# alevar/tiebrush

Hardware: AMD Instinct MI355X
Metric: input alignment records/sec collapsed (tiebrush) + bases/sec covered (tiecov) (higher is better)
Workload: dtype int64; 1 GPU; c3: 64 synthetic sorted BAMs x 5000000 100bp reads per GPU, --clip collapse + tiecov -c -j of the result; records_per_gpu=320000000, groups_out=25086541, parallelism=files-per-rank x1, ranks_seen=1, resident=SoA in HBM before the timed region, contexts=3

## Files before the change

### include/tbk.h

```cpp
#ifndef TBK_H_
#define TBK_H_

#include <stddef.h>
#include <stdint.h>

#ifdef __cplusplus
extern "C" {
#endif

#define TBK_ABI_VERSION 9

typedef struct tbk_ctx tbk_ctx;

typedef enum tbk_status {
  TBK_OK = 0,
  TBK_EINVAL = -1,
  TBK_ENOMEM = -2,
  TBK_EHIP = -3,
  TBK_E2BIG = -4,
  TBK_EUNSUPPORTED = -5,
  TBK_EUNSORTED = -6,
  TBK_EFATALOP = -7,
  TBK_ECOLLISION = -8,
  TBK_ENODEVICE = -9
// ... 7 lines not shown
} tbk_strategy;

typedef enum tbk_mem {
  TBK_MEM_HOST = 0,
  TBK_MEM_DEVICE = 1,
  TBK_MEM_KEPT = 2
} tbk_mem;

#define TBK_NH_ABSENT INT32_MIN

typedef struct tbk_collapse_opts {
  int32_t strategy;
  int32_t max_nh;
  int32_t min_qual;
  uint32_t flags_mask;
  uint8_t keep_supplementary;
  uint8_t keep_secondary;
  uint8_t keep_unmapped;
  uint8_t collapse_same;
  uint8_t store_frac;
  uint8_t defer_yd;
  uint8_t keep_results;
  uint8_t reserved[1];
} tbk_collapse_opts;

typedef struct tbk_soa_in {
  int32_t mem;
  uint32_t n_files;
  uint32_t n_records;
  uint32_t n_cigar_ops;
  const uint32_t* file_off;
  const uint8_t* tbmerged;
  const int32_t* tid;
  const int32_t* pos;
  const uint16_t* flag;
  const uint8_t* mapq;
  const uint8_t* strand;
  const int32_t* nh;
  const uint32_t* cig_off;
  const uint32_t* cig;
  const double* yc_in;
  const int64_t* yx_in;
  const int64_t* yd_in;
  const uint32_t* md_off;
  const uint8_t* md;
  const uint8_t* md_has;
  const uint64_t* qname_hash;
  const uint64_t* prio_hi;
  const uint64_t* prio_lo;
  const uint32_t* qname_off;
  const uint8_t* qname;
} tbk_soa_in;

typedef struct tbk_groups_out {
  int32_t mem;
  uint32_t cap_groups;
  uint32_t* rep;
  double* yc;
  int64_t* yx;
  int32_t* yd;
  int32_t* g_start;
  int32_t* g_end;
  int32_t* rec_group;
  int32_t* rep_effend;
  uint64_t* g_key;
  uint32_t n_groups;
  uint32_t n_passed;
} tbk_groups_out;

typedef struct tbk_cov_in {
  int32_t mem;
  uint32_t n_records;
  uint32_t n_cigar_ops;
  const int32_t* tid;
  const int32_t* pos;
  const uint16_t* flag;
  const uint32_t* cig_off;
  const uint32_t* cig;
  const double* yc;
  const uint8_t* strand;
  const int64_t* yx;
} tbk_cov_in;

typedef struct tbk_cov_out {
  int32_t mem;
  uint32_t cap_intervals;
  int32_t* iv_tid;
  int32_t* iv_start;
  int32_t* iv_end;
  double* iv_val;
  uint32_t cap_junctions;
  int32_t* j_tid;
  int32_t* j_start;
  int32_t* j_end;
  uint8_t* j_strand;
  double* j_val;
  uint32_t n_intervals;
  uint32_t n_junctions;
  uint64_t n_bases;
  uint64_t span_bases;
} tbk_cov_out;

typedef struct tbk_sample_out {
  int32_t mem;
  uint32_t cap_intervals;
  int32_t* iv_tid;
  int32_t* iv_start;
  int32_t* iv_end;
  int64_t* iv_count;
  float* iv_heat;
  uint32_t n_intervals;
} tbk_sample_out;

typedef struct tbk_kernel_time {
  const char* name;
  float ms;
  uint32_t launches;
} tbk_kernel_time;

int tbk_abi_version(void);
int tbk_create(int device_ordinal, tbk_ctx** out);
void tbk_destroy(tbk_ctx* ctx);
const char* tbk_strerror(int status);
const char* tbk_last_error(const tbk_ctx* ctx);

#define TBK_STREAM_DEFAULT ((void*)1)
int tbk_set_stream(tbk_ctx* ctx, void* hip_stream);
void* tbk_get_stream(tbk_ctx* ctx);
int tbk_set_profiling(tbk_ctx* ctx, int enabled);
int tbk_set_debug(tbk_ctx* ctx, const char* spec);
int tbk_kernel_times(tbk_ctx* ctx, tbk_kernel_time* out, int cap);

int tbk_host_alloc(size_t bytes, void** out);
void tbk_host_free(void* p);

void tbk_collapse_opts_default(tbk_collapse_opts* o);
int tbk_collapse_tile(tbk_ctx* ctx, const tbk_collapse_opts* opts, const tbk_soa_in* in, tbk_groups_out* out);
int tbk_collapse_finish_yd(tbk_ctx* ctx);
int tbk_warmup(tbk_ctx* ctx);
enum { TBK_ROUTE_NONE = 0, TBK_ROUTE_RAW_WINDOW = 1, TBK_ROUTE_COMPACTED_WINDOW = 2, TBK_ROUTE_SORT = 3 };
typedef struct tbk_collapse_route {
  int32_t form;
  int32_t reseeds;
  uint8_t raw_handed_back;
  uint8_t big_bucket;
  uint8_t wg_stats;
  uint8_t reserved;
  uint32_t nw, nw_live;
  uint32_t ovf1, ovf2;
} tbk_collapse_route;
int tbk_last_route(const tbk_ctx* ctx, tbk_collapse_route* out);
int tbk_coverage_tile(tbk_ctx* ctx, const tbk_cov_in* in, tbk_cov_out* out);
int tbk_sample_tile(tbk_ctx* ctx, const tbk_cov_in* in, int32_t num_samples, tbk_sample_out* out);

int tbk_groups_to_cov_in(tbk_ctx* ctx, const tbk_soa_in* in, const tbk_groups_out* groups, tbk_cov_in* view);


int tbk_bgzf_inflate(tbk_ctx* ctx, const uint8_t* comp, uint64_t comp_bytes, uint8_t* out, uint64_t out_cap, uint64_t* out_bytes, int mem);

int tbk_bam_decode(tbk_ctx* ctx, uint32_t n_files, const uint8_t* const* comp, const uint64_t* comp_bytes, const uint8_t* tbmerged,
                   int want_md, int want_names, tbk_soa_in* tile, uint32_t* file_off_out);
int tbk_bam_records(tbk_ctx* ctx, const uint32_t* idx, uint32_t n, int idx_mem, uint8_t* out, uint64_t out_cap, uint64_t* out_off);
void tbk_bam_release(tbk_ctx* ctx);
int tbk_tile_join(tbk_ctx* ctx, const tbk_soa_in* dev_part, const tbk_soa_in* host_part, tbk_soa_in* out, uint32_t* file_off_out,
                  uint8_t* tbmerged_out);
int tbk_reserve_tile(tbk_ctx* ctx, uint64_t n_records, uint64_t n_cigar_ops);


int tbk_bgzf_deflate(tbk_ctx* ctx, const uint8_t* src, uint64_t n, int src_mem, const uint64_t* cuts, uint32_t n_members, uint8_t* out,
                     uint64_t out_cap, uint64_t* out_bytes);

typedef struct tbk_enc_in {
  int32_t mem;
  uint32_t n;
  const uint32_t* rep;
  const double* yc;
  const int64_t* yx;
  const int32_t* yd;
  uint32_t n_dev;
  uint32_t n_host;
  const uint8_t* host_blob;
  const uint64_t* host_off;
  const uint32_t* host_slot;
  uint32_t first;
  tbk_ctx* from;
} tbk_enc_in;
int tbk_bam_encode(tbk_ctx* ctx, const tbk_enc_in* in, uint8_t* out, uint64_t out_cap, uint64_t* out_bytes, uint64_t* payload_bytes);
typedef struct tbk_ix_opts {
  uint32_t n_ref;
  uint32_t reserved;
  const uint32_t* ref_len;
  uint64_t* rec_vbeg;
} tbk_ix_opts;
typedef struct tbk_ix_chunk {
  int32_t tid;
  uint32_t bin;
  uint64_t beg, end;
} tbk_ix_chunk;
typedef struct tbk_ix_ref {
  int32_t tid;
  uint32_t reserved;
  uint64_t n_records;
  uint64_t first, last;
} tbk_ix_ref;
typedef struct tbk_ix_part {
  uint32_t n_chunks;
  uint32_t n_refs;
  uint64_t n_lin;
  uint64_t lin_first;
  const tbk_ix_chunk* chunks;
  const uint64_t* lin;
  const tbk_ix_ref* refs;
} tbk_ix_part;
int tbk_bam_encode_indexed(tbk_ctx* ctx, const tbk_enc_in* in, uint8_t* out, uint64_t out_cap, uint64_t* out_bytes, uint64_t* payload_bytes,
                           const tbk_ix_opts* ix, tbk_ix_part* part);
int tbk_kept_results(tbk_ctx* ctx, uint32_t first, uint32_t n, uint32_t* rep, double* yc, int64_t* yx, int32_t* yd);

typedef struct tbk_packed_in {
  uint32_t n_files;
  uint32_t n_records;
  uint32_t n_cigar_ops;
  uint32_t n_tid_runs;
  const uint32_t* file_off;
  const uint32_t* tid_run_end;
  const int32_t* tid_run_tid;
  const int32_t* pos;
  const uint32_t* meta;
  const uint8_t* ncig;
  const uint32_t* cig;
  uint32_t n_nh_esc, n_ncig_esc;
  const uint32_t* nh_esc_idx;
  const int32_t* nh_esc_val;
  const uint32_t* ncig_esc_idx;
  const uint32_t* ncig_esc_val;
} tbk_packed_in;
int tbk_unpack_tile(tbk_ctx* ctx, const tbk_packed_in* in, tbk_soa_in* tile);


int tbk_shard_prepare(tbk_ctx* ctx, const tbk_collapse_opts* opts, const tbk_soa_in* in, int64_t* key, int64_t* emax, int32_t* effend,
                      uint8_t* pass);
int tbk_shard_probe_max(tbk_ctx* ctx, const uint32_t* file_off, uint32_t n_files, const int64_t* key, const int64_t* emax,
                        const int64_t* cuts, uint32_t n_cuts, int64_t* m_out);
int tbk_shard_probe_next(tbk_ctx* ctx, const uint32_t* file_off, uint32_t n_files, const int64_t* key, const int64_t* m, uint32_t n_cuts,
                         int64_t* nxt_out);
#define TBK_SHARD_ROW 6
int tbk_shard_pack(tbk_ctx* ctx, const tbk_soa_in* in, const int64_t* key, const uint8_t* pass, const int32_t* effend, const int64_t* cuts,
                   uint32_t world, int32_t* rows, uint32_t* cig_out, int64_t* src_idx, int64_t* tab);
int tbk_shard_unpack(tbk_ctx* ctx, const int32_t* rows, uint32_t n2, const uint32_t* file_off2, uint32_t K, int32_t* tid, int32_t* pos,
                     uint16_t* flag, uint8_t* mapq, uint8_t* strand, int32_t* nh, uint32_t* cig_off, int64_t* prio_hi, int64_t* prio_lo);


int tbk_partial_keys(tbk_ctx* ctx, const tbk_soa_in* in, const tbk_groups_out* g, int64_t* key, int64_t* emax, uint32_t* not_packable);
#define TBK_PARTIAL_ROW 12
int tbk_partial_pack(tbk_ctx* ctx, const tbk_collapse_opts* opts, const tbk_soa_in* in, const tbk_groups_out* g, const int64_t* key,
                     const int64_t* cuts, uint32_t world, uint32_t first_fidx, int32_t* rows, uint32_t* cig_out, int64_t* tab);
#define TBK_PARTIAL_BUNDLES 15
#define TBK_PARTIAL_CAND (2 + 2 * TBK_PARTIAL_BUNDLES)
#define TBK_PARTIAL_META (64 + 4)
int tbk_partial_stage_keys(tbk_ctx* ctx, const tbk_soa_in* in, const tbk_groups_out* g, int64_t* key, int64_t* emax, uint32_t first_fidx, int64_t carry,
                           int64_t* meta);
int tbk_partial_stage_cands(tbk_ctx* ctx, const int64_t* key, const int64_t* emax, uint32_t n_groups, const int64_t* allmeta, uint32_t world,
                            int64_t* targets, int64_t* cands);
int tbk_partial_stage_pack(tbk_ctx* ctx, const tbk_collapse_opts* opts, const tbk_soa_in* in, const tbk_groups_out* g, const int64_t* key,
                           const int64_t* mymeta, const int64_t* allcands, const int64_t* targets, uint32_t world, uint32_t first_fidx, int64_t* cuts,
                           int32_t* rows, uint32_t* cig_out, int64_t* tabx);
int tbk_partial_pack_md(tbk_ctx* ctx, const tbk_soa_in* in, const tbk_groups_out* g, const int64_t* tab, uint32_t world, int32_t* rows, uint8_t* md_out,
                        int64_t* md_tab);
int tbk_partial_unpack_md(tbk_ctx* ctx, const int32_t* rows, uint32_t n2, uint32_t* md_off, uint8_t* md_has);
int tbk_partial_unpack(tbk_ctx* ctx, const int32_t* rows, uint32_t n2, int32_t* tid, int32_t* pos, uint16_t* flag, uint8_t* mapq,
                       uint8_t* strand, int32_t* nh, uint32_t* cig_off, double* yc_in, int64_t* yx_in, int64_t* yd_in, int64_t* prio_hi,
                       int64_t* prio_lo);
int tbk_partial_reduce(tbk_ctx* ctx, const tbk_collapse_opts* opts, const int32_t* rows, uint32_t n2, const uint32_t* run_off,
                       uint32_t n_runs, const uint32_t* cig, tbk_groups_out* out, tbk_cov_in* view);
int tbk_partial_reduce_md(tbk_ctx* ctx, const tbk_collapse_opts* opts, const int32_t* rows, uint32_t n2, const uint32_t* run_off, uint32_t n_runs,
                          const uint32_t* cig, const uint8_t* md, tbk_groups_out* out, tbk_cov_in* view);

typedef enum tbk_track_kind { TBK_TRACK_COV = 0, TBK_TRACK_JUNC = 1, TBK_TRACK_SAMPLE = 2 } tbk_track_kind;
typedef struct tbk_track_rows {
  int32_t mem;
  int32_t kind;
  uint32_t n;
  uint32_t reserved;
  const int32_t* tid;
  const int32_t* start;
  const int32_t* end;
  const double* val;
  const uint8_t* strand;
  const int64_t* count;
  const float* heat;
  int64_t first_junc;
} tbk_track_rows;
typedef int (*tbk_track_sink)(void* user, const char* bytes, uint64_t n);
int tbk_track_names(tbk_ctx* ctx, uint32_t n_names, const uint64_t* off, const char* bytes);
int tbk_format_track(tbk_ctx* ctx, const tbk_track_rows* rows, tbk_track_sink sink, void* user, uint64_t* out_bytes);


int tbk_bam_decode_spans(tbk_ctx* ctx, uint32_t n_spans, const uint8_t* const* comp, const uint64_t* comp_bytes, const uint32_t* first_uoff,
                         const uint32_t* last_uoff, int32_t n_ref, tbk_soa_in* tile, uint32_t* span_off_out, const uint8_t** tag_seen_out);

int tbk_region_view(tbk_ctx* ctx, const tbk_soa_in* tile, const uint8_t* tag_seen, int32_t tid, int64_t beg, int64_t end, tbk_cov_in* view,
                    uint32_t* n_kept);

int tbk_cov_clip(tbk_ctx* ctx, tbk_cov_out* rows, int32_t tid, int64_t beg, int64_t end);
int tbk_sample_clip(tbk_ctx* ctx, tbk_sample_out* rows, int32_t tid, int64_t beg, int64_t end);


// ... 26 lines not shown
```

### tiebrush_amd/_lib.py

```python
from __future__ import annotations

import ctypes as C
import os

_HERE = os.path.dirname(os.path.abspath(__file__))
LIB_PATH = os.path.join(_HERE, "_build", "libtbk.so")

_P = C.c_void_p

TBK_MEM_HOST, TBK_MEM_DEVICE, TBK_MEM_KEPT = 0, 1, 2
PARTIAL_BUNDLES = 15
PARTIAL_CAND = 2 + 2 * PARTIAL_BUNDLES
PARTIAL_META = 64 + 4
STRAT = {"cigar": 0, "full": 1, "clip": 2, "exon": 3}
STATUS = {0: "TBK_OK", -1: "TBK_EINVAL", -2: "TBK_ENOMEM", -3: "TBK_EHIP", -4: "TBK_E2BIG", -5: "TBK_EUNSUPPORTED",
          -6: "TBK_EUNSORTED", -7: "TBK_EFATALOP", -8: "TBK_ECOLLISION", -9: "TBK_ENODEVICE"}

SYMBOLS = ["tbk_abi_version", "tbk_create", "tbk_destroy", "tbk_strerror", "tbk_last_error", "tbk_set_stream",
           "tbk_get_stream", "tbk_set_profiling", "tbk_set_debug", "tbk_kernel_times", "tbk_host_alloc", "tbk_host_free",
           "tbk_collapse_opts_default", "tbk_collapse_tile", "tbk_collapse_finish_yd", "tbk_coverage_tile", "tbk_sample_tile",
           "tbk_groups_to_cov_in", "tbk_bgzf_inflate", "tbk_bam_decode", "tbk_bam_records", "tbk_bam_release", "tbk_shard_prepare", "tbk_shard_probe_max", "tbk_shard_probe_next",
           "tbk_shard_pack", "tbk_shard_unpack", "tbk_partial_keys", "tbk_partial_pack", "tbk_partial_unpack", "tbk_partial_reduce", "tbk_unpack_tile", "tbk_tile_join", "tbk_reserve_tile", "tbk_bgzf_deflate", "tbk_bam_encode", "tbk_kept_results", "tbk_warmup", "tbk_partial_stage_keys", "tbk_partial_stage_cands", "tbk_partial_stage_pack",
           "tbk_partial_pack_md", "tbk_partial_unpack_md", "tbk_partial_reduce_md", "tbk_track_names", "tbk_format_track", "tbk_bam_encode_indexed",
           "tbk_bam_decode_spans", "tbk_region_view", "tbk_cov_clip", "tbk_sample_clip", "tbk_bam_decode_file_spans", "tbk_tile_region", "tbk_last_route",
           "tbk_regions_view", "tbk_cov_clip_regions", "tbk_sample_clip_regions", "tbk_tile_regions"]


class CollapseOpts(C.Structure):
    _fields_ = [("strategy", C.c_int32), ("max_nh", C.c_int32), ("min_qual", C.c_int32), ("flags_mask", C.c_uint32),
                ("keep_supplementary", C.c_uint8), ("keep_secondary", C.c_uint8), ("keep_unmapped", C.c_uint8),
                ("collapse_same", C.c_uint8), ("store_frac", C.c_uint8), ("defer_yd", C.c_uint8), ("keep_results", C.c_uint8), ("reserved", C.c_uint8 * 1)]


class CollapseRoute(C.Structure):
    _fields_ = [("form", C.c_int32), ("reseeds", C.c_int32), ("raw_handed_back", C.c_uint8), ("big_bucket", C.c_uint8),
                ("wg_stats", C.c_uint8), ("reserved", C.c_uint8), ("nw", C.c_uint32), ("nw_live", C.c_uint32), ("ovf1", C.c_uint32),
                ("ovf2", C.c_uint32)]


ROUTE_FORMS = {0: "none", 1: "raw", 2: "compacted", 3: "sort"}


class SoaIn(C.Structure):
    _fields_ = [("mem", C.c_int32), ("n_files", C.c_uint32), ("n_records", C.c_uint32), ("n_cigar_ops", C.c_uint32),
                ("file_off", _P), ("tbmerged", _P), ("tid", _P), ("pos", _P), ("flag", _P), ("mapq", _P),
                ("strand", _P), ("nh", _P), ("cig_off", _P), ("cig", _P), ("yc_in", _P), ("yx_in", _P), ("yd_in", _P),
                ("md_off", _P), ("md", _P), ("md_has", _P), ("qname_hash", _P), ("prio_hi", _P), ("prio_lo", _P),
                ("qname_off", _P), ("qname", _P)]


class PackedIn(C.Structure):
    _fields_ = [("n_files", C.c_uint32), ("n_records", C.c_uint32), ("n_cigar_ops", C.c_uint32), ("n_tid_runs", C.c_uint32), ("file_off", _P),
                ("tid_run_end", _P), ("tid_run_tid", _P), ("pos", _P), ("meta", _P), ("ncig", _P), ("cig", _P), ("n_nh_esc", C.c_uint32),
                ("n_ncig_esc", C.c_uint32), ("nh_esc_idx", _P), ("nh_esc_val", _P), ("ncig_esc_idx", _P), ("ncig_esc_val", _P)]


class GroupsOut(C.Structure):
    _fields_ = [("mem", C.c_int32), ("cap_groups", C.c_uint32), ("rep", _P), ("yc", _P), ("yx", _P), ("yd", _P),
                ("g_start", _P), ("g_end", _P), ("rec_group", _P), ("rep_effend", _P), ("g_key", _P), ("n_groups", C.c_uint32),
                ("n_passed", C.c_uint32)]


class CovIn(C.Structure):
    _fields_ = [("mem", C.c_int32), ("n_records", C.c_uint32), ("n_cigar_ops", C.c_uint32), ("tid", _P), ("pos", _P),
                ("flag", _P), ("cig_off", _P), ("cig", _P), ("yc", _P), ("strand", _P), ("yx", _P)]


class CovOut(C.Structure):
    _fields_ = [("mem", C.c_int32), ("cap_intervals", C.c_uint32), ("iv_tid", _P), ("iv_start", _P), ("iv_end", _P),
                ("iv_val", _P), ("cap_junctions", C.c_uint32), ("j_tid", _P), ("j_start", _P), ("j_end", _P),
                ("j_strand", _P), ("j_val", _P), ("n_intervals", C.c_uint32), ("n_junctions", C.c_uint32),
                ("n_bases", C.c_uint64), ("span_bases", C.c_uint64)]


class SampleOut(C.Structure):
    _fields_ = [("mem", C.c_int32), ("cap_intervals", C.c_uint32), ("iv_tid", _P), ("iv_start", _P), ("iv_end", _P),
                ("iv_count", _P), ("iv_heat", _P), ("n_intervals", C.c_uint32)]


class EncIn(C.Structure):
    _fields_ = [("mem", C.c_int32), ("n", C.c_uint32), ("rep", _P), ("yc", _P), ("yx", _P), ("yd", _P), ("n_dev", C.c_uint32), ("n_host", C.c_uint32),
                ("host_blob", _P), ("host_off", _P), ("host_slot", _P), ("first", C.c_uint32), ("from_ctx", _P)]


class IxOpts(C.Structure):
    _fields_ = [("n_ref", C.c_uint32), ("reserved", C.c_uint32), ("ref_len", _P), ("rec_vbeg", _P)]


class IxChunk(C.Structure):
    _fields_ = [("tid", C.c_int32), ("bin", C.c_uint32), ("beg", C.c_uint64), ("end", C.c_uint64)]


class IxRef(C.Structure):
    _fields_ = [("tid", C.c_int32), ("reserved", C.c_uint32), ("n_records", C.c_uint64), ("first", C.c_uint64), ("last", C.c_uint64)]


class IxPart(C.Structure):
    _fields_ = [("n_chunks", C.c_uint32), ("n_refs", C.c_uint32), ("n_lin", C.c_uint64), ("lin_first", C.c_uint64), ("chunks", _P), ("lin", _P), ("refs", _P)]


class Regions(C.Structure):
    _fields_ = [("n", C.c_uint32), ("tid", _P), ("beg", _P), ("end", _P)]


TRACK = {"cov": 0, "junc": 1, "sample": 2}


class TrackRows(C.Structure):
    _fields_ = [("mem", C.c_int32), ("kind", C.c_int32), ("n", C.c_uint32), ("reserved", C.c_uint32), ("tid", _P), ("start", _P), ("end", _P),
                ("val", _P), ("strand", _P), ("count", _P), ("heat", _P), ("first_junc", C.c_int64)]


TRACK_SINK = C.CFUNCTYPE(C.c_int, _P, _P, C.c_uint64)


class KernelTime(C.Structure):
    _fields_ = [("name", C.c_char_p), ("ms", C.c_float), ("launches", C.c_uint32)]


_lib = None


def load():
    global _lib
    if _lib is not None:
        return _lib
    if not os.path.exists(LIB_PATH):
        raise ImportError("%s not found: build it with `python -c 'import __graft_entry__ as g; g.build()'` "
                          "(hipcc --offload-arch=gfx950); there is no CPU fallback" % LIB_PATH)
    try:
        import torch
    except ImportError:
        pass
    L = C.CDLL(LIB_PATH)
    L.tbk_abi_version.restype = C.c_int
    L.tbk_create.argtypes = [C.c_int, C.POINTER(_P)]
    L.tbk_create.restype = C.c_int
    L.tbk_destroy.argtypes = [_P]
    L.tbk_destroy.restype = None
    L.tbk_strerror.argtypes = [C.c_int]
    L.tbk_strerror.restype = C.c_char_p
    L.tbk_last_error.argtypes = [_P]
    L.tbk_last_error.restype = C.c_char_p
    L.tbk_set_stream.argtypes = [_P, _P]
    L.tbk_get_stream.argtypes = [_P]
    L.tbk_get_stream.restype = _P
    L.tbk_set_profiling.argtypes = [_P, C.c_int]
    L.tbk_set_debug.argtypes = [_P, C.c_char_p]
    L.tbk_last_route.argtypes = [_P, C.POINTER(CollapseRoute)]
    L.tbk_last_route.restype = C.c_int
    L.tbk_kernel_times.argtypes = [_P, C.POINTER(KernelTime), C.c_int]
    L.tbk_host_alloc.argtypes = [C.c_size_t, C.POINTER(_P)]
    L.tbk_host_free.argtypes = [_P]
    L.tbk_host_free.restype = None
    L.tbk_collapse_opts_default.argtypes = [C.POINTER(CollapseOpts)]
    L.tbk_collapse_opts_default.restype = None
    L.tbk_collapse_tile.argtypes = [_P, C.POINTER(CollapseOpts), C.POINTER(SoaIn), C.POINTER(GroupsOut)]
    L.tbk_collapse_finish_yd.argtypes = [_P]
    L.tbk_coverage_tile.argtypes = [_P, C.POINTER(CovIn), C.POINTER(CovOut)]
    L.tbk_sample_tile.argtypes = [_P, C.POINTER(CovIn), C.c_int32, C.POINTER(SampleOut)]
    L.tbk_groups_to_cov_in.argtypes = [_P, C.POINTER(SoaIn), C.POINTER(GroupsOut), C.POINTER(CovIn)]
    L.tbk_bgzf_inflate.argtypes = [_P, _P, C.c_uint64, _P, C.c_uint64, C.POINTER(C.c_uint64), C.c_int]
    L.tbk_bam_decode.argtypes = [_P, C.c_uint32, _P, _P, _P, C.c_int, C.c_int, C.POINTER(SoaIn), _P]
    L.tbk_bam_records.argtypes = [_P, _P, C.c_uint32, C.c_int, _P, C.c_uint64, _P]
    L.tbk_bam_release.argtypes = [_P]
    L.tbk_bam_release.restype = None
    L.tbk_shard_prepare.argtypes = [_P, C.POINTER(CollapseOpts), C.POINTER(SoaIn), _P, _P, _P, _P]
    L.tbk_shard_probe_max.argtypes = [_P, _P, C.c_uint32, _P, _P, _P, C.c_uint32, _P]
    L.tbk_shard_probe_next.argtypes = [_P, _P, C.c_uint32, _P, _P, C.c_uint32, _P]
    L.tbk_shard_pack.argtypes = [_P, C.POINTER(SoaIn), _P, _P, _P, _P, C.c_uint32, _P, _P, _P, _P]
    L.tbk_shard_unpack.argtypes = [_P, _P, C.c_uint32, _P, C.c_uint32, _P, _P, _P, _P, _P, _P, _P, _P, _P]
    L.tbk_partial_keys.argtypes = [_P, C.POINTER(SoaIn), C.POINTER(GroupsOut), _P, _P, C.POINTER(C.c_uint32)]
    L.tbk_partial_pack.argtypes = [_P, C.POINTER(CollapseOpts), C.POINTER(SoaIn), C.POINTER(GroupsOut), _P, _P, C.c_uint32, C.c_uint32, _P, _P, _P]
    L.tbk_partial_reduce.argtypes = [_P, C.POINTER(CollapseOpts), _P, C.c_uint32, _P, C.c_uint32, _P, C.POINTER(GroupsOut), C.POINTER(CovIn)]
    L.tbk_partial_unpack.argtypes = [_P, _P, C.c_uint32] + [_P] * 12
    L.tbk_tile_join.argtypes = [_P, C.POINTER(SoaIn), C.POINTER(SoaIn), C.POINTER(SoaIn), C.POINTER(C.c_uint32), C.POINTER(C.c_uint8)]
    L.tbk_tile_join.restype = C.c_int
    L.tbk_reserve_tile.argtypes = [_P, C.c_uint64, C.c_uint64]
    L.tbk_reserve_tile.restype = C.c_int
    L.tbk_unpack_tile.argtypes = [_P, C.POINTER(PackedIn), C.POINTER(SoaIn)]
    L.tbk_partial_stage_keys.argtypes = [_P, C.POINTER(SoaIn), C.POINTER(GroupsOut), _P, _P, C.c_uint32, C.c_int64, _P]
    L.tbk_partial_stage_cands.argtypes = [_P, _P, _P, C.c_uint32, _P, C.c_uint32, _P, _P]
    L.tbk_partial_stage_pack.argtypes = [_P, C.POINTER(CollapseOpts), C.POINTER(SoaIn), C.POINTER(GroupsOut), _P, _P, _P, _P, C.c_uint32, C.c_uint32, _P, _P, _P, _P]
    L.tbk_partial_pack_md.argtypes = [_P, C.POINTER(SoaIn), C.POINTER(GroupsOut), _P, C.c_uint32, _P, _P, _P]
    L.tbk_partial_unpack_md.argtypes = [_P, _P, C.c_uint32, _P, _P]
    L.tbk_partial_reduce_md.argtypes = [_P, C.POINTER(CollapseOpts), _P, C.c_uint32, _P, C.c_uint32, _P, _P, C.POINTER(GroupsOut), C.POINTER(CovIn)]
    L.tbk_bgzf_deflate.argtypes = [_P, _P, C.c_uint64, C.c_int, _P, C.c_uint32, _P, C.c_uint64, C.POINTER(C.c_uint64)]
    L.tbk_bgzf_deflate.restype = C.c_int
    L.tbk_bam_encode.argtypes = [_P, C.POINTER(EncIn), _P, C.c_uint64, C.POINTER(C.c_uint64), C.POINTER(C.c_uint64)]
    L.tbk_bam_encode.restype = C.c_int
    L.tbk_bam_encode_indexed.argtypes = [_P, C.POINTER(EncIn), _P, C.c_uint64, C.POINTER(C.c_uint64), C.POINTER(C.c_uint64), C.POINTER(IxOpts), C.POINTER(IxPart)]
    L.tbk_bam_encode_indexed.restype = C.c_int
    L.tbk_kept_results.argtypes = [_P, C.c_uint32, C.c_uint32, _P, _P, _P, _P]
    L.tbk_kept_results.restype = C.c_int
    L.tbk_warmup.argtypes = [_P]
    L.tbk_warmup.restype = C.c_int
    L.tbk_track_names.argtypes = [_P, C.c_uint32, _P, _P]
    L.tbk_track_names.restype = C.c_int
    L.tbk_format_track.argtypes = [_P, C.POINTER(TrackRows), TRACK_SINK, _P, C.POINTER(C.c_uint64)]
    L.tbk_format_track.restype = C.c_int
    L.tbk_bam_decode_spans.argtypes = [_P, C.c_uint32, _P, _P, _P, _P, C.c_int32, C.POINTER(SoaIn), _P, C.POINTER(_P)]
    L.tbk_bam_decode_spans.restype = C.c_int
    L.tbk_region_view.argtypes = [_P, C.POINTER(SoaIn), _P, C.c_int32, C.c_int64, C.c_int64, C.POINTER(CovIn), C.POINTER(C.c_uint32)]
    L.tbk_region_view.restype = C.c_int
    L.tbk_cov_clip.argtypes = [_P, C.POINTER(CovOut), C.c_int32, C.c_int64, C.c_int64]
    L.tbk_cov_clip.restype = C.c_int
    L.tbk_sample_clip.argtypes = [_P, C.POINTER(SampleOut), C.c_int32, C.c_int64, C.c_int64]
    L.tbk_sample_clip.restype = C.c_int
    L.tbk_bam_decode_file_spans.argtypes = [_P, C.c_uint32, _P, _P, _P, _P, _P, C.c_int32, _P, C.c_int, C.c_int, C.POINTER(SoaIn), _P]
    L.tbk_bam_decode_file_spans.restype = C.c_int
    L.tbk_tile_region.argtypes = [_P, C.POINTER(SoaIn), C.c_int32, C.c_int64, C.c_int64, C.POINTER(SoaIn), _P, C.POINTER(C.c_uint32)]
    L.tbk_tile_region.restype = C.c_int
    L.tbk_regions_view.argtypes = [_P, C.POINTER(SoaIn), _P, C.POINTER(Regions), C.POINTER(CovIn), C.POINTER(C.c_uint32)]
    L.tbk_regions_view.restype = C.c_int
    L.tbk_cov_clip_regions.argtypes = [_P, C.POINTER(CovOut), C.POINTER(Regions)]
    L.tbk_cov_clip_regions.restype = C.c_int
    L.tbk_sample_clip_regions.argtypes = [_P, C.POINTER(SampleOut), C.POINTER(Regions)]
    L.tbk_sample_clip_regions.restype = C.c_int
    L.tbk_tile_regions.argtypes = [_P, C.POINTER(SoaIn), C.POINTER(Regions), C.POINTER(SoaIn), _P, C.POINTER(C.c_uint32)]
    L.tbk_tile_regions.restype = C.c_int
    _lib = L
    return L


HOST_LIB_PATH = os.environ.get("TBK_HOST_LIB") or os.path.join(_HERE, "_build", "libtbh.so")
HOST_SYMBOLS = ["tbh_abi_version", "tbh_last_error", "tbh_tag_deflate_part", "tbh_write_bam_parts", "tbh_is_tiebrush", "tbh_bai_index_file", "tbh_bai_reg2bin",
                "tbh_csi_index_file", "tbh_csi_depth", "tbh_csi_reg2bin", "tbh_index_query",
                "tbh_regions_from_bed", "tbh_index_query_regions"]
_host = None


def load_host():
    global _host
    if _host is not None:
        return _host
    if not os.path.exists(HOST_LIB_PATH):
        raise ImportError("%s not found: build it with `python -c 'import __graft_entry__ as g; g.build()'`" % HOST_LIB_PATH)
    H = C.CDLL(HOST_LIB_PATH)
    H.tbh_abi_version.restype = C.c_int
    H.tbh_last_error.restype = C.c_char_p
    H.tbh_tag_deflate_part.argtypes = [_P, _P, _P, C.c_uint32, _P, _P, _P, C.c_int, C.c_int, C.c_char_p]
    H.tbh_tag_deflate_part.restype = C.c_int
    H.tbh_write_bam_parts.argtypes = [C.c_char_p, C.c_char_p, C.c_int, C.POINTER(C.c_char_p), C.c_int, C.POINTER(C.c_char_p), C.c_int,
                                      C.POINTER(C.c_char_p), C.c_int]
    H.tbh_write_bam_parts.restype = C.c_int
    H.tbh_is_tiebrush.argtypes = [C.c_char_p]
    H.tbh_is_tiebrush.restype = C.c_int
    H.tbh_bai_index_file.argtypes = [C.c_char_p, C.c_char_p]
    H.tbh_bai_index_file.restype = C.c_int
    H.tbh_bai_reg2bin.argtypes = [C.c_int64, C.c_int64]
    H.tbh_bai_reg2bin.restype = C.c_uint32
    H.tbh_csi_index_file.argtypes = [C.c_char_p, C.c_char_p]
    H.tbh_csi_index_file.restype = C.c_int
    H.tbh_csi_depth.argtypes = [C.c_uint64]
    H.tbh_csi_depth.restype = C.c_int
    H.tbh_csi_reg2bin.argtypes = [C.c_int64, C.c_int64, C.c_int]
    H.tbh_csi_reg2bin.restype = C.c_uint32
    H.tbh_index_query.argtypes = [C.c_char_p, C.c_char_p, C.c_int32, C.c_int64, C.c_int64, _P, _P, C.c_uint64]
    H.tbh_index_query.restype = C.c_int64
    H.tbh_regions_from_bed.argtypes = [C.c_char_p, C.c_char_p, _P, _P, _P, C.c_uint64]
    H.tbh_regions_from_bed.restype = C.c_int64
    H.tbh_index_query_regions.argtypes = [C.c_char_p, C.c_char_p, C.c_uint32, _P, _P, _P, _P, _P, C.c_uint64]
    H.tbh_index_query_regions.restype = C.c_int64
    _host = H
    return H


class TbkError(RuntimeError):
    def __init__(self, status, detail=""):
        self.status = status
        super().__init__("%s (%d) %s" % (STATUS.get(status, "?"), status, detail))
```

### tiebrush_amd/api.py

```python
from __future__ import annotations

import contextlib
import os
import ctypes as C
from dataclasses import replace

import numpy as np

from . import _lib
from ._lib import TbkError
from .soa import CovInput, SoATile


def _torch():
    import torch
    return torch


def _is_torch(a):
    return a is not None and type(a).__module__.startswith("torch")


def _addr(a, dtype, keep, n=None):
    if a is None:
        return None
    if _is_torch(a):
        torch = _torch()
        want = {np.int32: torch.int32, np.uint32: torch.int32, np.uint16: torch.int16, np.uint8: torch.uint8,
                np.float64: torch.float64, np.int64: torch.int64, np.uint64: torch.int64, np.float32: torch.float32}[dtype]
        if a.dtype != want and a.element_size() != np.dtype(dtype).itemsize:
            raise TypeError("tensor dtype %s does not match %s" % (a.dtype, dtype))
        if not a.is_contiguous():
            raise ValueError("tensor must be contiguous")
        if n is not None and a.numel() < n:
            raise ValueError("tensor too small: %d < %d" % (a.numel(), n))
        keep.append(a)
        return a.data_ptr()
    b = np.ascontiguousarray(a, dtype=dtype)
    if n is not None and b.size < n:
        raise ValueError("array too small: %d < %d" % (b.size, n))
    keep.append(b)
    return b.ctypes.data


def to_device(obj, device="cuda:0"):
    torch = _torch()

    def mv(a, dt):
        if a is None:
            return None
        b = np.ascontiguousarray(a, dtype=dt)
        sd = {np.uint32: np.int32, np.uint16: np.int16, np.uint64: np.int64}.get(dt, dt)
        return torch.from_numpy(b.view(sd)).to(device)

    if isinstance(obj, SoATile):
        r = replace(obj, tid=mv(obj.tid, np.int32), pos=mv(obj.pos, np.int32), flag=mv(obj.flag, np.uint16),
                       mapq=mv(obj.mapq, np.uint8), strand=mv(obj.strand, np.uint8), nh=mv(obj.nh, np.int32),
                       cig_off=mv(obj.cig_off, np.uint32), cig=mv(obj.cig, np.uint32), yc_in=mv(obj.yc_in, np.float64),
                       yx_in=mv(obj.yx_in, np.int64), yd_in=mv(obj.yd_in, np.int64), md_off=mv(obj.md_off, np.uint32),
                       md=mv(obj.md, np.uint8), md_has=mv(obj.md_has, np.uint8),
                       qname_hash=mv(obj.qname_hash, np.uint64), qn_off=mv(obj.qn_off, np.uint32), qn=mv(obj.qn, np.uint8),
                       prio_hi=mv(obj.prio_hi, np.uint64), prio_lo=mv(obj.prio_lo, np.uint64))
        torch.cuda.synchronize()
        return r
    if isinstance(obj, CovInput):
        r = replace(obj, tid=mv(obj.tid, np.int32), pos=mv(obj.pos, np.int32), flag=mv(obj.flag, np.uint16),
                       cig_off=mv(obj.cig_off, np.uint32), cig=mv(obj.cig, np.uint32), yc=mv(obj.yc, np.float64),
                       strand=mv(obj.strand, np.uint8), yx=mv(obj.yx, np.int64))
        torch.cuda.synchronize()
        return r
    raise TypeError(type(obj))


def _numel(a):
    return int(a.numel()) if _is_torch(a) else int(np.asarray(a).size)


class DeviceTile:

    def __init__(self, struct, n_files, keep):
        self.struct, self.n_files, self._keep = struct, n_files, keep
        self.n_records = int(struct.n_records)


class DeviceCovView:

    def __init__(self, struct, n_records, n_cigar_ops):
        self.struct = struct
        self.n_records = n_records
        self.n_cigar_ops = n_cigar_ops


class _FollowDebug:

    def __init__(self, lib, ctx):
        self._lib, self._ctx = lib, ctx

    def __getattr__(self, name):
        self._ctx._follow_debug()
        return getattr(self._lib, name)


class Context:
    def __init__(self, device: int = 0):
        lib = _lib.load()
        h = C.c_void_p()
        self._debug_spec = os.environ.get("TBK_DEBUG", "")
        rc = lib.tbk_create(int(device), C.byref(h))
        if rc != 0:
            raise TbkError(rc, "tbk_create(device=%d)" % device)
        self._lib = lib
        self.L = _FollowDebug(lib, self)
        self.h = h
        self.device = device
        self._on_torch_stream = False

    def _follow_debug(self):
        spec = os.environ.get("TBK_DEBUG", "")
        if spec != self._debug_spec and getattr(self, "h", None):
            self._debug_spec = spec
            self._lib.tbk_set_debug(self.h, spec.encode())

    def set_debug(self, spec: str):
        self._debug_spec = os.environ.get("TBK_DEBUG", "")
        self._check(self._lib.tbk_set_debug(self.h, spec.encode()), "tbk_set_debug")

    def close(self):
        if getattr(self, "h", None):
            self._lib.tbk_destroy(self.h)
            self.h = None

    def __del__(self):
        try:
            self.close()
        except Exception:
            pass

    def _check(self, rc, what):
        if rc != 0:
            raise TbkError(rc, "%s: %s" % (what, (self.L.tbk_last_error(self.h) or b"").decode()))

    def use_torch_stream(self):
        s = _torch().cuda.current_stream(self.device).cuda_stream
        self._check(self.L.tbk_set_stream(self.h, C.c_void_p(s if s else 1)), "tbk_set_stream")
        self._on_torch_stream = True

    def _order_after_torch(self, dev):
        if dev and not self._on_torch_stream:
            _torch().cuda.current_stream(self.device).synchronize()

    def last_message(self) -> str:
        return (self.L.tbk_last_error(self.h) or b"").decode()

    def collapse_route(self) -> dict:
        r = _lib.CollapseRoute()
        self._check(self._lib.tbk_last_route(self.h, C.byref(r)), "tbk_last_route")
        d = dict(form=_lib.ROUTE_FORMS[int(r.form)], reseeds=int(r.reseeds), raw_handed_back=bool(r.raw_handed_back),
                 big_bucket=bool(r.big_bucket))
        if r.wg_stats:
            d.update(nw=int(r.nw), nw_live=int(r.nw_live), ovf1=int(r.ovf1), ovf2=int(r.ovf2))
        return d

    def stream_ptr(self):
        return self.L.tbk_get_stream(self.h)

    def set_profiling(self, on: bool):
        self._check(self.L.tbk_set_profiling(self.h, 1 if on else 0), "tbk_set_profiling")

    def kernel_times(self):
        arr = (_lib.KernelTime * 128)()
        n = self.L.tbk_kernel_times(self.h, arr, 128)
        return {arr[i].name.decode(): (float(arr[i].ms), int(arr[i].launches)) for i in range(min(n, 128))}

    def _alloc(self, device_mode, n, dtype):
        n = max(int(n), 1)
        if device_mode:
            torch = _torch()
            td = {np.int32: torch.int32, np.uint32: torch.int32, np.uint8: torch.uint8, np.float64: torch.float64,
                  np.int64: torch.int64, np.uint64: torch.int64, np.float32: torch.float32}[dtype]
            return torch.empty(n, dtype=td, device="cuda:%d" % self.device)
        return np.empty(n, dtype=dtype)

    @staticmethod
    def _trim(a, n, dtype):
        if _is_torch(a):
            return a[:n]
        return a[:n].view(dtype) if a.dtype != dtype else a[:n]

    def make_opts(self, strategy="cigar", max_nh=2**31 - 1, min_qual=-1, keep_supplementary=False,
                  keep_secondary=False, keep_unmapped=False, collapse_same=False, store_frac=False, flags_mask=0,
                  defer_yd=False, keep_results=False):
        o = _lib.CollapseOpts()
        self.L.tbk_collapse_opts_default(C.byref(o))
        o.strategy = _lib.STRAT[strategy] if isinstance(strategy, str) else int(strategy)
        o.max_nh, o.min_qual, o.flags_mask = int(max_nh), int(min_qual), int(flags_mask)
        o.keep_supplementary, o.keep_secondary = int(keep_supplementary), int(keep_secondary)
        o.keep_unmapped, o.collapse_same, o.store_frac = int(keep_unmapped), int(collapse_same), int(store_frac)
        o.defer_yd = int(defer_yd)
        o.keep_results = int(keep_results)
        return o

    def finish_yd(self):
        self._check(self.L.tbk_collapse_finish_yd(self.h), "tbk_collapse_finish_yd")

    def unpack_tile(self, pt) -> DeviceTile:
        keep = []

        def addr(a, dt):
            if _is_torch(a):
                keep.append(a)
                return a.data_ptr() if a.numel() else None
            b = np.ascontiguousarray(a, dtype=dt)
            keep.append(b)
            return b.ctypes.data if b.size else None

        fo = np.ascontiguousarray(pt.file_off, dtype=np.uint32)
        re_, rt = np.ascontiguousarray(pt.tid_run_end, np.uint32), np.ascontiguousarray(pt.tid_run_tid, np.int32)
        keep += [fo, re_, rt]
        p = _lib.PackedIn(pt.n_files, _numel(pt.pos), _numel(pt.cig), len(re_), fo.ctypes.data, re_.ctypes.data, rt.ctypes.data, addr(pt.pos, np.int32),
                          addr(pt.meta, np.uint32), addr(pt.ncig, np.uint8), addr(pt.cig, np.uint32), _numel(pt.nh_esc_idx), _numel(pt.ncig_esc_idx),
                          addr(pt.nh_esc_idx, np.uint32), addr(pt.nh_esc_val, np.int32), addr(pt.ncig_esc_idx, np.uint32),
                          addr(pt.ncig_esc_val, np.uint32))
        s = _lib.SoaIn()
        self._check(self.L.tbk_unpack_tile(self.h, C.byref(p), C.byref(s)), "tbk_unpack_tile")
        return DeviceTile(s, pt.n_files, keep)

    def _soa_struct(self, tile: SoATile, keep):
        if isinstance(tile, DeviceTile):
            keep.append(tile)
            return tile.struct, True, tile.n_records
        dev = _is_torch(tile.tid)
        n = _numel(tile.tid)
        nc = _numel(tile.cig)
        fo = np.ascontiguousarray(tile.file_off, dtype=np.uint32)
        tb = np.ascontiguousarray(tile.tbmerged, dtype=np.uint8)
        keep += [fo, tb]
        s = _lib.SoaIn(
            _lib.TBK_MEM_DEVICE if dev else _lib.TBK_MEM_HOST, tile.n_files, n, nc, fo.ctypes.data, tb.ctypes.data,
            _addr(tile.tid, np.int32, keep, n), _addr(tile.pos, np.int32, keep, n), _addr(tile.flag, np.uint16, keep, n),
            _addr(tile.mapq, np.uint8, keep, n), _addr(tile.strand, np.uint8, keep, n), _addr(tile.nh, np.int32, keep, n),
            _addr(tile.cig_off, np.uint32, keep, n + 1), _addr(tile.cig, np.uint32, keep, nc),
            _addr(tile.yc_in, np.float64, keep, n), _addr(tile.yx_in, np.int64, keep, n),
            _addr(tile.yd_in, np.int64, keep, n), _addr(tile.md_off, np.uint32, keep, n + 1),
            _addr(tile.md, np.uint8, keep), _addr(tile.md_has, np.uint8, keep, n),
            _addr(tile.qname_hash, np.uint64, keep, n), _addr(tile.prio_hi, np.uint64, keep, n),
            _addr(tile.prio_lo, np.uint64, keep, n), _addr(tile.qn_off, np.uint32, keep, n + 1), _addr(tile.qn, np.uint8, keep))
        return s, dev, n

    def collapse(self, tile: SoATile, opts=None, want_coords=True, want_rec_group=False, want_effend=False, out=None,
                 raw=False, want_key=None, cap_groups=None, **kw):
        o = opts if opts is not None else self.make_opts(**kw)
        keep = []
        s, dev, n = self._soa_struct(tile, keep)
        self._order_after_torch(dev)
        cap = max(n if cap_groups is None else min(int(cap_groups), n), 1)
        bufs = out if out is not None else {}
        if bufs.get("_cap_groups", 0) > cap:
            cap = bufs["_cap_groups"]
        res = self._collapse_once(o, s, dev, n, cap, bufs, keep, want_coords, want_rec_group, want_effend, want_key, raw)
        if isinstance(res, int):
            bufs["_cap_groups"] = cap = min(n, res + res // 16 + 1)
            res = self._collapse_once(o, s, dev, n, cap, bufs, keep, want_coords, want_rec_group, want_effend, want_key, raw)
            assert not isinstance(res, int)
        return res

    def _collapse_once(self, o, s, dev, n, cap, bufs, keep, want_coords, want_rec_group, want_effend, want_key, raw):

        def buf(name, count, dt, wanted=True):
            if not wanted:
                return None
            if name not in bufs or _numel(bufs[name]) < count:
                bufs[name] = self._alloc(dev, count, dt)
            return bufs[name]

        rep, yc = buf("rep", cap, np.uint32), buf("yc", cap, np.float64)
        yx, yd = buf("yx", cap, np.int64), buf("yd", cap, np.int32)
        gs, ge = buf("g_start", cap, np.int32, want_coords), buf("g_end", cap, np.int32, want_coords)
        rg = buf("rec_group", max(n, 1), np.int32, want_rec_group)
        re_ = buf("rep_effend", cap, np.int32, want_effend)
        want_key = bool(dev) if want_key is None else want_key
        gk = buf("g_key", 2 * cap, np.uint64, want_key)
        g = _lib.GroupsOut(s.mem, cap, _addr(rep, np.uint32, keep), _addr(yc, np.float64, keep),
                           _addr(yx, np.int64, keep), _addr(yd, np.int32, keep), _addr(gs, np.int32, keep),
                           _addr(ge, np.int32, keep), _addr(rg, np.int32, keep), _addr(re_, np.int32, keep),
                           _addr(gk, np.uint64, keep), 0, 0)
        rc = self.L.tbk_collapse_tile(self.h, C.byref(o), C.byref(s), C.byref(g))
        if rc == -4 and int(g.n_groups) > cap:
            return int(g.n_groups)
        self._check(rc, "tbk_collapse_tile")
        m = int(g.n_groups)
        res = dict(n_groups=m, n_passed=int(g.n_passed), _bufs=bufs, _struct=g, _soa=s, _keep=keep)
        if raw:
            return res
        res.update(rep=self._trim(rep, m, np.uint32), yc=yc[:m], yx=yx[:m], yd=yd[:m])
        if want_coords:
            res.update(g_start=gs[:m], g_end=ge[:m])
        if want_rec_group:
            res["rec_group"] = rg[:n]
        if want_effend:
            res["rep_effend"] = re_[:m]
        if want_key:
            res["g_key"] = gk[:2 * m]
        return res

    def groups_to_cov_in(self, collapse_result) -> DeviceCovView:
        v = _lib.CovIn()
        self._order_after_torch(True)
        self._check(self.L.tbk_groups_to_cov_in(self.h, C.byref(collapse_result["_soa"]),
                                                C.byref(collapse_result["_struct"]), C.byref(v)),
                    "tbk_groups_to_cov_in")
        return DeviceCovView(v, int(v.n_records), int(v.n_cigar_ops))

    def bgzf_inflate(self, comp: bytes) -> bytes:
        src = np.frombuffer(comp, dtype=np.uint8)
        need = C.c_uint64(0)
        out = np.empty(max(1, 4 * len(src) + 65536), dtype=np.uint8)
        rc = self.L.tbk_bgzf_inflate(self.h, src.ctypes.data, len(src), out.ctypes.data, out.size, C.byref(need), _lib.TBK_MEM_HOST)
        if rc == -4:
            out = np.empty(int(need.value), dtype=np.uint8)
            rc = self.L.tbk_bgzf_inflate(self.h, src.ctypes.data, len(src), out.ctypes.data, out.size, C.byref(need), _lib.TBK_MEM_HOST)
        self._check(rc, "tbk_bgzf_inflate")
        return out[:int(need.value)].tobytes()

    def bgzf_deflate(self, payload: bytes, cuts=None) -> bytes:
        src = np.frombuffer(payload, dtype=np.uint8)
# ... 698 lines not shown
```

### tiebrush_amd/csrc/cb_tiles.hpp

```cpp
#pragma once
#include "dev_common.hpp"
#include "scan_op.hpp"

struct CbAgg {
  int32_t first_tid, last_tid;
  int32_t mx;
  uint32_t whole;
};
struct CbOp {
  __device__ __forceinline__ CbAgg operator()(const CbAgg& a, const CbAgg& b) const {
    if (b.last_tid == INT32_MIN) return a;
    if (a.last_tid == INT32_MIN) return b;
    CbAgg r;
    r.first_tid = a.first_tid;
    r.last_tid = b.last_tid;
    const bool joins = b.whole && b.first_tid == a.last_tid;
    r.mx = joins ? (a.mx > b.mx ? a.mx : b.mx) : b.mx;
    r.whole = joins ? a.whole : 0u;
    return r;
  }
};
constexpr uint32_t CB_NT = 256, CB_ROWS = 4, CB_TILE = CB_NT * 4 * CB_ROWS;
template <class T, class Op>
__device__ __forceinline__ T wave_incl_scan_op(T v, Op op) {
#pragma unroll
  for (int d = 1; d < 64; d <<= 1) {
    const T o = shfl_up_t(v, d);
    if ((int)lane_id() >= d) v = op(o, v);
  }
  return v;
}
__device__ __forceinline__ void cb_put(uint64_t* p, uint64_t v) { __hip_atomic_store(p, v, __ATOMIC_RELAXED, __HIP_MEMORY_SCOPE_AGENT); }
__device__ __forceinline__ uint64_t cb_get(const uint64_t* p) { return __hip_atomic_load(p, __ATOMIC_RELAXED, __HIP_MEMORY_SCOPE_AGENT); }
__device__ __forceinline__ uint4 cb_get4(const uint4* p) {
  const uint64_t a = cb_get(reinterpret_cast<const uint64_t*>(p)), b = cb_get(reinterpret_cast<const uint64_t*>(p) + 1);
  return make_uint4((uint32_t)a, (uint32_t)(a >> 32), (uint32_t)b, (uint32_t)(b >> 32));
}
__device__ __forceinline__ bool cb_last_block(uint32_t* __restrict__ done) {
  __shared__ uint32_t s_last;
  if (threadIdx.x == 0) {
    __builtin_amdgcn_s_waitcnt(TBK_WAIT_VMCNT0);
    __asm__ volatile("" ::: "memory");
    s_last = atomicAdd(done, 1u) == gridDim.x - 1u ? 1u : 0u;
  }
  __syncthreads();
  return s_last != 0u;
}
template <uint32_t NT>
__device__ __forceinline__ void cb_spine_block(uint4* __restrict__ part, uint32_t ntiles, CbAgg* wl ) {
  const CbOp op{};
  const CbAgg none{0, INT32_MIN, INT32_MIN, 1u};
  auto un = [](const uint4& v) { return CbAgg{(int32_t)v.x, (int32_t)v.y, (int32_t)v.z, v.w}; };
  auto pk = [](const CbAgg& a) { return make_uint4((uint32_t)a.first_tid, (uint32_t)a.last_tid, (uint32_t)a.mx, a.whole); };
  const uint4 none4 = pk(none);
  const uint32_t per = (ntiles + NT - 1u) / NT, i0 = threadIdx.x * per, i1 = i0 + per < ntiles ? i0 + per : ntiles;
  CbAgg a = none;
  for (uint32_t q0 = i0; q0 < i1; q0 += 8u) {
    uint4 v8[8];
#pragma unroll
    for (uint32_t u = 0; u < 8u; ++u) v8[u] = q0 + u < i1 ? cb_get4(part + q0 + u) : none4;
#pragma unroll
    for (uint32_t u = 0; u < 8u; ++u) a = op(a, un(v8[u]));
  }
  const CbAgg inc = wave_incl_scan_op(a, op);
  if (lane_id() == 63) wl[threadIdx.x >> 6] = inc;
  CbAgg run = shfl_up_t(inc, 1);
  __syncthreads();
  {
    CbAgg acc = none;
    const uint32_t wv = threadIdx.x >> 6;
    for (uint32_t q = 0; q < wv; ++q) acc = op(acc, wl[q]);
    run = lane_id() == 0 ? acc : op(acc, run);
  }
  for (uint32_t q0 = i0; q0 < i1; q0 += 8u) {
    uint4 v8[8];
#pragma unroll
    for (uint32_t u = 0; u < 8u; ++u) v8[u] = q0 + u < i1 ? cb_get4(part + q0 + u) : none4;
#pragma unroll
    for (uint32_t u = 0; u < 8u; ++u) {
      if (q0 + u < i1) part[q0 + u] = pk(run);
      run = op(run, un(v8[u]));
    }
  }
}
```

### tiebrush_amd/csrc/collapse.hip

```cpp
#include <stdlib.h>

#include <chrono>

#include "cb_tiles.hpp"
#include "dev_common.hpp"
#include "rx_w64.hpp"
#include "scan_op.hpp"
#include "strategy.hpp"
#include "tbk_internal.h"
#include "wgroup.h"

namespace {

struct EffKey {
  uint32_t khi_h, khi_l;
  int32_t kend;
  uint32_t flag_cnt;
};
struct EffOp {
  __device__ __forceinline__ EffKey operator()(const EffKey& a, const EffKey& b) const {
    uint64_t ak = ((uint64_t)a.khi_h << 32) | a.khi_l, bk = ((uint64_t)b.khi_h << 32) | b.khi_l;
    bool take_b = (b.flag_cnt >> 31) || bk > ak || (bk == ak && b.kend > a.kend);
    EffKey r;
    r.khi_h = take_b ? b.khi_h : a.khi_h;
// ... 2301 lines not shown
      out->n_passed = m;
      if (m == 0) return 0;
      m_hi = m;
    }
    bool runs_now = use_runs && (lean || m >= runs_min);
    for (;;) {
      if (runs_now)
        TBK_TRY(tbk_sort_runs(ctx, &s2, m_hi, run_off, I.k, ctx->d_err, (uint32_t*)(sc + 12)));
      else
        TBK_TRY(tbk_radix_sort128(ctx, &s2, m));
      TBK_LAUNCH(ctx, "col_heads", col_heads_k, cdiv(m_hi, B), B, 0, I, O.strategy, sc + 0, m_hi, s2.hi, s2.lo, s2.val, fidx, flags,
                 ghead, ctx->d_err);
      TBK_TRY(tbk_exscan_u32(ctx, ghead, gex, m_hi, sc + 1));
      if (lean) break;
      TBK_TRY(tbk_sync_err(ctx, &eb));
      if (runs_now && (eb & TBK_DERR_BIGBUCKET)) {
        std::swap(s2.hi, s2.hi2);
        std::swap(s2.lo, s2.lo2);
        std::swap(s2.val, s2.val2);
        TBK_HIP(hipMemsetAsync(ctx->d_err, 0, sizeof(uint32_t), ctx->stream));
        runs_now = false;
        continue;
      }
      break;
    }
    if (!lean) {
      if (eb & TBK_DERR_COLLISION) {
        ++attempt;
        continue;
      }
      if (eb) return tbk_derr_to_status(ctx, eb);
      ng = (uint32_t)ctx->h_scalars[1];
      if (ng > out->cap_groups) {
        out->n_groups = ng;
        return TBK_E2BIG;
      }
      ng_hi = ng;
    }
    const uint64_t *pm = sc + 0, *png = sc + 1;
    G.yc = ws_alloc<double>(ctx, ng_hi);
    G.ns = ws_alloc<uint32_t>(ctx, ng_hi);
    G.yxin = ws_alloc<long long>(ctx, ng_hi);
    G.ydin = ws_alloc<long long>(ctx, ng_hi);
    G.rep = ws_alloc<unsigned long long>(ctx, ng_hi);
    G.first = ws_alloc<uint32_t>(ctx, ng_hi);
    G.tie = ws_alloc<uint8_t>(ctx, ng_hi);
    g_yd = ws_alloc<int32_t>(ctx, ng_hi);
    gperm = ws_alloc<uint32_t>(ctx, ng_hi);
    ginv = ws_alloc<uint32_t>(ctx, ng_hi);
    if (!ginv) return TBK_ENOMEM;
    TBK_LAUNCH(ctx, "col_init_groups", col_init_groups_k, cdiv(ng_hi, B), B, 0, png, G, g_yd);
    TBK_LAUNCH(ctx, "col_reduce", col_reduce_k, cdiv(m_hi, B), B, 0, I, O, pm, s2.val, flags, gex, fidx, effend, G, sgid, ctx->d_err);
    if (I.prio_hi && I.prio_lo) TBK_LAUNCH(ctx, "col_rep_prio", col_rep_prio_k, cdiv(ng_hi, B), B, 0, I, png, pm, s2.val, G);
    if (O.collapse_same) TBK_LAUNCH(ctx, "col_same", col_same_k, cdiv(m_hi, B), B, 0, I, O, pm, s2.val, flags, sgid, fidx, G);
    TBK_LAUNCH(ctx, "col_tie_sort", col_tie_sort_k, cdiv(ng_hi, B), B, 0, I, O.strategy, png, s2.val, G, gperm, ginv);

    if (O.store_frac || any_tbm) {
      TBK_TRY(tbk_sync_err(ctx, &eb));
      const bool need_ordered = O.store_frac || (eb & TBK_DERR_FRACTIONAL);
      eb &= ~TBK_DERR_FRACTIONAL;
      if (eb) return tbk_derr_to_status(ctx, eb);
      if (need_ordered) {
        TBK_HIP(hipMemsetAsync(ctx->d_err, 0, sizeof(uint32_t), ctx->stream));
        SortBufs ob;
        ob.hi = ws_alloc<uint64_t>(ctx, m);
        ob.lo = ws_alloc<uint64_t>(ctx, m);
        ob.val = ws_alloc<uint32_t>(ctx, m);
        ob.hi2 = ws_alloc<uint64_t>(ctx, m);
        ob.lo2 = ws_alloc<uint64_t>(ctx, m);
        ob.val2 = ws_alloc<uint32_t>(ctx, m);
        uint8_t* fh_by_rec = ws_alloc<uint8_t>(ctx, n);
        if (!ob.val2 || !fh_by_rec) return TBK_ENOMEM;
        TBK_LAUNCH(ctx, "ord_fill", ord_fill_k, cdiv(m, B), B, 0, m, s2.val, sgid, effend, I.prio_hi, flags, ob.hi, ob.lo, ob.val, fh_by_rec);
        TBK_TRY(tbk_radix_sort128(ctx, &ob, m));
        TBK_LAUNCH(ctx, "ord_sum", ord_sum_k, cdiv(ng, 64), 64, 0, I, O, ng, m, ob.val, fidx, fh_by_rec, G);
      }
    }
    TBK_LAUNCH(ctx, "col_write", col_write_k<false>, cdiv(ng_hi, B), B, 0, png, gperm, G, s2.hi, s2.lo, out->cap_groups, out->rep, out->yc,
               out->yx, out->g_start, out->g_end, effend, out->rep_effend, out->g_key, O.strategy);
    if (out->rec_group) TBK_LAUNCH(ctx, "col_recgroup", col_recgroup_k, cdiv(m_hi, B), B, 0, pm, s2.val, sgid, ginv, out->rec_group);
    TBK_TRY(tbk_sync_err(ctx, &eb));
    if (lean) {
      if (eb & TBK_DERR_BIGBUCKET) {
        use_runs = false;
        lean = false;
        continue;
      }
      if (eb & TBK_DERR_COLLISION) {
        ++attempt;
        continue;
      }
      m = (uint32_t)ctx->h_scalars[0];
      ng = (uint32_t)ctx->h_scalars[1];
      out->n_passed = m;
    }
    if (eb & ~TBK_DERR_FRACTIONAL) return tbk_derr_to_status(ctx, eb);
    sb = s2;
    route.form = TBK_ROUTE_SORT;
    if (attempt > 0) {
      char b[96];
      snprintf(b, sizeof(b), "info: key-hash collision, reseeded %d time(s)", attempt);
      ctx->last_error = b;
    }
    break;
  }
  out->n_groups = ng;
  if (m == 0) return 0;
  if (ng > out->cap_groups) return TBK_E2BIG;
  TBK_TRY(tbk_check_launch(ctx, "collapse"));
  YdJob* job = new YdJob();
  job->I = I;
  job->m = m;
  job->ng = ng;
  job->cap = out->cap_groups;
  if (win_done) {
    job->win = true;
    job->np = win_out.np;
    job->pfile = win_out.pfile;
    job->pgrp = win_out.pgrp;
    job->gpoff = win_out.gpoff;
    job->gfmask = win_out.gfmask;
  }
  job->val = sb.val;
  job->flags = flags;
  job->fidx = fidx;
  job->sgid = sgid;
  job->ginv = ginv;
  job->gperm = gperm;
  job->G = G;
  job->shi = win_done ? win_out.ghi : sb.hi;
  job->slo = win_done ? win_out.glo : sb.lo;
  job->g_yd = g_yd;
  job->out_yd = out->yd;
  ctx->yd_job = job;
  return 0;
}

namespace {
__global__ void g2c_count_k(uint32_t ng, const uint32_t* __restrict__ rep, const uint32_t* __restrict__ cig_off, uint32_t* __restrict__ cnt,
                            uint32_t* __restrict__ cfirst) {
  uint32_t o = blockIdx.x * blockDim.x + threadIdx.x;
  if (o >= ng) return;
  const uint32_t c0 = cig_off[rep[o]];
  cnt[o] = cig_off[rep[o] + 1] - c0;
  cfirst[o] = c0;
}
__device__ __forceinline__ uint32_t g2c_key_ops(uint64_t k1) {
  const uint32_t shape = (uint32_t)k1;
  return shape == 0x80000000u ? 1u : ((shape >> 30) == 3u ? 3u : 0u);
}
__global__ __launch_bounds__(CB_NT) void g2c_count_key_k(uint32_t ng, const uint64_t* __restrict__ key, const uint32_t* __restrict__ rep,
                                                         const uint32_t* __restrict__ cig_off, const uint32_t* __restrict__ cig,
                                                         uint32_t* __restrict__ cnt, uint32_t* __restrict__ cfirst, uint4* __restrict__ part,
                                                         unsigned long long* __restrict__ tsum, uint32_t* __restrict__ done,
                                                         unsigned long long* __restrict__ total) {
  constexpr uint32_t NWV = CB_NT / 64;
  __shared__ CbAgg wl[CB_ROWS * NWV];
  __shared__ unsigned long long wsum[CB_ROWS * NWV];
  const CbOp op{};
  const CbAgg none{0, INT32_MIN, INT32_MIN, 1u};
  for (uint32_t r = 0; r < CB_ROWS; ++r) {
    const uint64_t i = (uint64_t)blockIdx.x * CB_TILE + ((uint64_t)r * CB_NT + threadIdx.x) * 4u;
    CbAgg a = none;
    uint32_t n4[4] = {0u, 0u, 0u, 0u};
#pragma unroll
    for (int e = 0; e < 4; ++e) {
      if (i + e < ng) {
        const uint32_t o = (uint32_t)(i + e);
        const uint64_t k0 = key[2 * (size_t)o], k1 = key[2 * (size_t)o + 1];
        const int32_t tidv = (int32_t)(uint32_t)(k0 >> 33) - 1, posv = (int32_t)(uint32_t)((k0 >> 2) & 0x7FFFFFFFull) - 1;
        uint32_t n = g2c_key_ops(k1);
        int l = (int)(uint32_t)(k1 >> 32);
        if (n == 0) {
          const uint32_t rp = rep[o];
          const uint32_t c0 = cig_off[rp];
          n = cig_off[rp + 1] - c0;
          cfirst[o] = c0;
          int nex = 0;
          l = walk_exons(posv, cig + c0, n, [](int, int) {}, &nex);
        }
        n4[e] = n;
        a = op(a, CbAgg{tidv, tidv, posv + l, 1u});
      }
    }
    if (i + 3 < ng) {
      *reinterpret_cast<uint4*>(cnt + i) = make_uint4(n4[0], n4[1], n4[2], n4[3]);
    } else {
#pragma unroll
      for (int e = 0; e < 4; ++e)
        if (i + e < ng) cnt[i + e] = n4[e];
    }
    a = wave_incl_scan_op(a, op);
    const unsigned long long sum = wave_sum((unsigned long long)n4[0] + n4[1] + n4[2] + n4[3]);
    if (lane_id() == 63) {
      wl[r * NWV + (threadIdx.x >> 6)] = a;
      wsum[r * NWV + (threadIdx.x >> 6)] = sum;
    }
  }
  __syncthreads();
  if (threadIdx.x == 0) {
    CbAgg run = none;
    unsigned long long sum = 0;
#pragma unroll
    for (uint32_t q = 0; q < CB_ROWS * NWV; ++q) {
      run = op(run, wl[q]);
      sum += wsum[q];
    }
    uint64_t* o = reinterpret_cast<uint64_t*>(part + blockIdx.x);
    cb_put(o, (uint64_t)(uint32_t)run.first_tid | ((uint64_t)(uint32_t)run.last_tid << 32));
    cb_put(o + 1, (uint64_t)(uint32_t)run.mx | ((uint64_t)run.whole << 32));
    cb_put(reinterpret_cast<uint64_t*>(tsum + blockIdx.x), sum);
  }
  if (!cb_last_block(done)) return;
  const uint32_t ntiles = gridDim.x;
  cb_spine_block<CB_NT>(part, ntiles, wl);
  const uint32_t per = (ntiles + CB_NT - 1u) / CB_NT;
  const uint32_t i0 = threadIdx.x * per < ntiles ? threadIdx.x * per : ntiles, i1 = i0 + per < ntiles ? i0 + per : ntiles;
  unsigned long long mine = 0;
  for (uint32_t q = i0; q < i1; ++q) mine += cb_get(reinterpret_cast<const uint64_t*>(tsum + q));
  unsigned long long tot;
  unsigned long long run = block_excl_sum<unsigned long long, CB_NT>(mine, wsum, &tot);
  for (uint32_t q = i0; q < i1; ++q) {
    const unsigned long long v = cb_get(reinterpret_cast<const uint64_t*>(tsum + q));
    tsum[q] = run;
    run += v;
  }
  if (threadIdx.x == 0) *total = tot;
}
struct G2cPrep {
  int32_t *start, *end, *yi;
  uint32_t *jcnt, *ridx;
  unsigned long long* sums;
};
__global__ __launch_bounds__(256) void g2c_gather_key_k(uint32_t ng, const uint64_t* __restrict__ key, const double* __restrict__ yc,
                                                        const int64_t* __restrict__ yx, const uint32_t* __restrict__ cfirst,
                                                        const uint32_t* __restrict__ cnt, const uint32_t* __restrict__ cig,
                                                        const unsigned long long* __restrict__ tbase, const uint4* __restrict__ part,
                                                        uint32_t ntiles, uint32_t total, int32_t* __restrict__ o_tid,
                                                        int32_t* __restrict__ o_pos, uint8_t* __restrict__ o_strand, double* __restrict__ o_yc,
                                                        int64_t* __restrict__ o_yx, uint32_t* __restrict__ o_cig_off, uint32_t* __restrict__ o_cig,
                                                        uint4* __restrict__ o_part, G2cPrep P) {
  constexpr uint32_t NROW = CB_TILE / 256u;
  __shared__ uint32_t s_w[NROW * 4u];
  for (uint32_t q = blockIdx.x * 256u + threadIdx.x; q < ntiles; q += gridDim.x * 256u) o_part[q] = part[q];
  unsigned long long mb = 0, ay = 0, nji = 0;
  uint32_t eb = 0;
  for (uint32_t tile = blockIdx.x; tile < ntiles; tile += gridDim.x) {
  const uint32_t o0 = tile * CB_TILE;
  for (uint32_t j = 0; j < NROW; ++j) {
    const uint32_t o = o0 + j * 256u + threadIdx.x;
    const uint32_t s = wave_sum(o < ng ? cnt[o] : 0u);
    if (lane_id() == 0) s_w[j * 4u + (threadIdx.x >> 6)] = s;
  }
  __syncthreads();
  if (threadIdx.x < 64u) {
    const uint32_t v = s_w[threadIdx.x];
    s_w[threadIdx.x] = wave_incl_sum(v) - v;
  }
  __syncthreads();
  const uint32_t base = (uint32_t)tbase[tile];
  for (uint32_t j = 0; j < NROW; ++j) {
    const uint32_t o = o0 + j * 256u + threadIdx.x;
    const uint32_t cn = o < ng ? cnt[o] : 0u;
    const uint32_t d = base + s_w[j * 4u + (threadIdx.x >> 6)] + wave_incl_sum(cn) - cn;
    if (o >= ng) continue;
    const uint64_t k0 = key[2 * (size_t)o], k1 = key[2 * (size_t)o + 1];
    const int32_t tidv = (int32_t)(uint32_t)(k0 >> 33) - 1, posv = (int32_t)(uint32_t)((k0 >> 2) & 0x7FFFFFFFull) - 1;
    o_tid[o] = tidv;
    o_pos[o] = posv;
    const uint32_t sc = (uint32_t)k0 & 3u;
    o_strand[o] = sc == 0u ? (uint8_t)'+' : (sc == 1u ? (uint8_t)'-' : (uint8_t)'.');
    const double y0 = (double)(float)yc[o];
    o_yc[o] = y0;
    o_yx[o] = yx[o];
    o_cig_off[o] = d;
    if (o + 1 == ng) o_cig_off[ng] = total;
    const uint32_t shape = (uint32_t)k1, span = (uint32_t)(k1 >> 32);
    int l, nex = 0;
    if (shape == 0x80000000u) {
      o_cig[d] = (span << 4) | C_M;
      l = (int)span;
      nex = 1;
      mb += span;
    } else if ((shape >> 30) == 3u) {
      const uint32_t a = (shape >> 20) & 0x3FFu, g = shape & 0xFFFFFu;
      o_cig[d] = (a << 4) | C_M;
      o_cig[d + 1] = (g << 4) | C_N;
      o_cig[d + 2] = ((span - a - g) << 4) | C_M;
      l = (int)span;
      nex = 2;
      mb += span - g;
    } else {
      const uint32_t c0 = cfirst[o], n = cn;
      l = walk_exons(posv, cig + c0, n, [](int, int) {}, &nex);
      for (uint32_t k = 0; k < n; ++k) {
        const uint32_t w = cig[c0 + k];
        o_cig[d + k] = w;
        const uint32_t op = cig_op(w);
        if (op == C_M)
          mb += cig_len(w);
        else if (op != C_I && op != C_D && op != C_N && op != C_S)
          eb |= TBK_DERR_FATALOP;
      }
      if (n >= 256) eb |= TBK_DERR_NCIGAR;
    }
    double y = y0;
    if (!(y == rint(y)) || !(fabs(y) < 1073741824.0)) {
      eb |= TBK_DERR_FRACTIONAL;
      y = 0.0;
    } else {
      ay += (unsigned long long)fabs(y);
    }
    P.ridx[o] = o;
    P.yi[o] = (int32_t)y;
    P.start[o] = posv + 1;
    P.end[o] = posv + l;
    P.jcnt[o] = (uint32_t)(nex - 1);
    nji += (unsigned long long)(nex - 1);
  }
  __syncthreads();
  }
  __shared__ unsigned long long red_mb[4], red_ay[4], red_nj[4];
  __shared__ uint32_t red_e[4];
  mb = wave_sum(mb);
  ay = wave_sum(ay);
  nji = wave_sum(nji);
#pragma unroll
  for (int dd = 32; dd >= 1; dd >>= 1) eb |= __shfl_xor(eb, dd, 64);
  if (lane_id() == 0) {
    red_mb[threadIdx.x >> 6] = mb;
    red_ay[threadIdx.x >> 6] = ay;
    red_nj[threadIdx.x >> 6] = nji;
    red_e[threadIdx.x >> 6] = eb;
  }
  __syncthreads();
  if (threadIdx.x == 0) {
    for (int q = 1; q < 4; ++q) {
      mb += red_mb[q];
      ay += red_ay[q];
      nji += red_nj[q];
      eb |= red_e[q];
    }
    if (mb) atomicAdd(&P.sums[0], mb);
    if (ay) atomicAdd(&P.sums[1], ay);
    if (eb) atomicOr(&P.sums[2], (unsigned long long)eb);
    if (nji) atomicAdd(&P.sums[3], nji);
  }
}
__global__ void g2c_gather_k(uint32_t ng, const uint32_t* __restrict__ rep, const double* __restrict__ yc, const int64_t* __restrict__ yx,
                             const int32_t* __restrict__ tid, const int32_t* __restrict__ pos, const uint8_t* __restrict__ strand,
                             const uint32_t* __restrict__ cfirst, const uint32_t* __restrict__ cnt, const uint32_t* __restrict__ cig,
                             const uint32_t* __restrict__ ooff, uint32_t total, int32_t* __restrict__ o_tid, int32_t* __restrict__ o_pos,
                             uint8_t* __restrict__ o_strand, double* __restrict__ o_yc, int64_t* __restrict__ o_yx,
                             uint32_t* __restrict__ o_cig_off, uint32_t* __restrict__ o_cig) {
  uint32_t o = blockIdx.x * blockDim.x + threadIdx.x;
  if (o >= ng) return;
  uint32_t r = rep[o];
  o_tid[o] = tid[r];
  o_pos[o] = pos[r];
  o_strand[o] = strand[r];
  o_yc[o] = (double)(float)yc[o];
  o_yx[o] = yx[o];
  uint32_t d = ooff[o];
  o_cig_off[o] = d;
  if (o + 1 == ng) o_cig_off[ng] = total;
  const uint32_t c0 = cfirst[o], n = cnt[o];
  for (uint32_t k = 0; k < n; ++k) o_cig[d + k] = cig[c0 + k];
}
}

extern "C" int tbk_groups_to_cov_in(tbk_ctx* ctx, const tbk_soa_in* in, const tbk_groups_out* g, tbk_cov_in* view) {
  if (!ctx || !in || !g || !view) return TBK_EINVAL;
  if (in->mem != TBK_MEM_DEVICE || g->mem != TBK_MEM_DEVICE) return TBK_EINVAL;
  TBK_HIP(hipSetDevice(ctx->device));
  const uint32_t ng = g->n_groups;
  memset(view, 0, sizeof(*view));
  view->mem = TBK_MEM_DEVICE;
  tbk_prof_begin_call(ctx);
  struct ProfEnd {
    tbk_ctx* c;
    ~ProfEnd() { tbk_prof_end_call(c); }
  } prof_end{ctx};
  if (ng == 0) return 0;
  TBK_TRY(tbk_ws_reserve(ctx, (size_t)ng * 24 + ((size_t)1 << 20)));
  return tbk_cov_view_build(ctx, in->tid, in->pos, in->strand, in->cig_off, in->cig, g->rep, g->yc, g->yx, ng, view, g->g_key);
}

int tbk_cov_view_build(tbk_ctx* ctx, const int32_t* r_tid, const int32_t* r_pos, const uint8_t* r_strand, const uint32_t* r_cig_off,
                       const uint32_t* r_cig, const uint32_t* g_rep, const double* g_yc, const int64_t* g_yx, uint32_t ng, tbk_cov_in* view,
                       const uint64_t* g_key) {
  memset(view, 0, sizeof(*view));
  view->mem = TBK_MEM_DEVICE;
  ctx->view_prep.valid = false;
  if (ng == 0) return 0;
  uint32_t* cnt = ws_alloc<uint32_t>(ctx, ng);
  uint32_t* cfirst = ws_alloc<uint32_t>(ctx, ng);
  if (!cnt || !cfirst) return TBK_ENOMEM;
  const uint32_t B = 256;
  static_assert(CB_NT == 256 && CB_TILE % 256 == 0 && CB_TILE / 256 * 4 == 64, "g2c_gather_key_k: rows of 256 groups, 64 wave sums per tile");
  const uint32_t ntiles = cdiv(ng, CB_TILE);
  uint32_t* ooff = nullptr;
  uint4* part = nullptr;
  unsigned long long* tbase = nullptr;
  if (g_key) {
    part = ws_alloc<uint4>(ctx, ntiles);
    tbase = ws_alloc<unsigned long long>(ctx, ntiles);
    if (!part || !tbase) return TBK_ENOMEM;
    uint32_t* done = (uint32_t*)(ctx->d_scalars + 21);
    TBK_HIP(hipMemsetAsync(done, 0, sizeof(uint64_t), ctx->stream));
    TBK_LAUNCH(ctx, "g2c_count", g2c_count_key_k, ntiles, CB_NT, 0, ng, g_key, g_rep, r_cig_off, r_cig, cnt, cfirst, part, tbase, done,
               (unsigned long long*)(ctx->d_scalars + 20));
  } else {
    ooff = ws_alloc<uint32_t>(ctx, ng);
    if (!ooff) return TBK_ENOMEM;
    TBK_LAUNCH(ctx, "g2c_count", g2c_count_k, cdiv(ng, B), B, 0, ng, g_rep, r_cig_off, cnt, cfirst);
    TBK_TRY(tbk_exscan_u32(ctx, cnt, ooff, ng, ctx->d_scalars + 20));
  }
  TBK_HIP(hipMemcpyAsync(ctx->h_scalars + 20, ctx->d_scalars + 20, sizeof(uint64_t), hipMemcpyDeviceToHost, ctx->stream));
  TBK_HIP(hipStreamSynchronize(ctx->stream));
  const uint64_t total = ctx->h_scalars[20];
  if (total >= (1ull << 32)) return TBK_E2BIG;
  auto al = [](size_t x) { return (x + 255) & ~(size_t)255; };
  size_t need = al((size_t)ng * 4) * 2 + al(ng) + al((size_t)ng * 8) * 2 + al((size_t)(ng + 1) * 4) + al((size_t)total * 4 + 4) +
                (g_key ? al((size_t)ng * 4) * 5 + al((size_t)ntiles * sizeof(uint4)) : 0);
  if (need > ctx->d_view_cap) {
    if (ctx->d_view) (void)hipFree(ctx->d_view);
    ctx->d_view = nullptr;
    ctx->d_view_cap = 0;
    size_t cap = need + need / 4;
    TBK_HIP(hipMalloc((void**)&ctx->d_view, cap));
    ctx->d_view_cap = cap;
  }
  char* p = ctx->d_view;
  auto take = [&](size_t bytes) {
    char* r = p;
    p += al(bytes);
    return r;
  };
  int32_t* o_tid = (int32_t*)take((size_t)ng * 4);
  int32_t* o_pos = (int32_t*)take((size_t)ng * 4);
  uint8_t* o_strand = (uint8_t*)take(ng);
  double* o_yc = (double*)take((size_t)ng * 8);
  int64_t* o_yx = (int64_t*)take((size_t)ng * 8);
  uint32_t* o_cig_off = (uint32_t*)take((size_t)(ng + 1) * 4);
  uint32_t* o_cig = (uint32_t*)take((size_t)total * 4 + 4);
  G2cPrep P{};
  uint4* o_part = nullptr;
  if (g_key) {
    P.start = (int32_t*)take((size_t)ng * 4);
    P.end = (int32_t*)take((size_t)ng * 4);
    P.yi = (int32_t*)take((size_t)ng * 4);
    P.jcnt = (uint32_t*)take((size_t)ng * 4);
    P.ridx = (uint32_t*)take((size_t)ng * 4);
    o_part = (uint4*)take((size_t)ntiles * sizeof(uint4));
    P.sums = (unsigned long long*)(ctx->d_scalars + 24);
    TBK_HIP(hipMemsetAsync(P.sums, 0, 4 * sizeof(uint64_t), ctx->stream));
    TBK_LAUNCH(ctx, "g2c_gather", g2c_gather_key_k, ntiles, B, 0, ng, g_key, g_yc, g_yx, cfirst, cnt, r_cig, tbase, part, ntiles, (uint32_t)total,
               o_tid, o_pos, o_strand, o_yc, o_yx, o_cig_off, o_cig, o_part, P);
    TBK_HIP(hipMemcpyAsync(ctx->h_scalars + 24, ctx->d_scalars + 24, 4 * sizeof(uint64_t), hipMemcpyDeviceToHost, ctx->stream));
  } else
    TBK_LAUNCH(ctx, "g2c_gather", g2c_gather_k, cdiv(ng, B), B, 0, ng, g_rep, g_yc, g_yx, r_tid, r_pos, r_strand, cfirst, cnt, r_cig, ooff,
               (uint32_t)total, o_tid, o_pos, o_strand, o_yc, o_yx, o_cig_off, o_cig);
  TBK_HIP(hipStreamSynchronize(ctx->stream));
  TBK_TRY(tbk_check_launch(ctx, "groups_to_cov_in"));
  view->n_records = ng;
  view->n_cigar_ops = (uint32_t)total;
  view->tid = o_tid;
  view->pos = o_pos;
  view->flag = nullptr;
  view->cig_off = o_cig_off;
  view->cig = o_cig;
  view->yc = o_yc;
  view->strand = o_strand;
  view->yx = o_yx;
  if (g_key) {
    auto& V = ctx->view_prep;
    V.cig = o_cig;
    V.n = ng;
    V.start = P.start;
    V.end = P.end;
    V.yi = P.yi;
    V.jcnt = P.jcnt;
    V.ridx = P.ridx;
    V.agg = o_part;
    V.agg_tiles = ntiles;
    V.n_bases = ctx->h_scalars[24];
    V.sum_abs = ctx->h_scalars[25];
    V.err = (uint32_t)ctx->h_scalars[26];
    V.n_junc = ctx->h_scalars[27];
    V.valid = true;
  }
  return 0;
}
```

### tiebrush_amd/csrc/cov.hip

```cpp
#include <thread>

#include "cb_tiles.hpp"
#include "dev_common.hpp"
#include "scan_op.hpp"
#include "tbk_internal.h"

namespace {

constexpr int COV_W = 8192;
constexpr int COV_NT = 256;
constexpr int COV_PER = COV_W / COV_NT;

struct SegMax {
  int32_t mx;
  uint32_t flag;
};
struct SegMaxOp {
  __device__ __forceinline__ SegMax operator()(const SegMax& a, const SegMax& b) const {
    SegMax r;
    r.mx = b.flag ? b.mx : (a.mx > b.mx ? a.mx : b.mx);
    r.flag = a.flag | b.flag;
    return r;
  }
};
// ... 549 lines not shown
}

__device__ __forceinline__ bool cp_kept(const uint64_t* sp, const double* sv, uint32_t q) {
  if (!(sp[q] >> 63)) return true;
  return q > 0 && sv[q] != sv[q - 1];
}


constexpr uint32_t IV_NT = 256, IV_ROWS = 8, IV_TILE = IV_NT * IV_ROWS;
__device__ __forceinline__ bool iv_emits(const uint64_t* __restrict__ sp, const double* __restrict__ sv, uint32_t q) {
  return cp_kept(sp, sv, q) && sv[q] != 0.0;
}
__global__ __launch_bounds__(IV_NT) void iv_count_k(uint32_t ncp, const uint64_t* __restrict__ sp, const double* __restrict__ sv, uint32_t* __restrict__ cnt) {
  __shared__ uint32_t sm[IV_NT / 64];
  uint32_t n = 0;
#pragma unroll
  for (uint32_t r = 0; r < IV_ROWS; ++r) {
    const uint64_t q = (uint64_t)blockIdx.x * IV_TILE + (uint64_t)r * IV_NT + threadIdx.x;
    n += q < ncp && iv_emits(sp, sv, (uint32_t)q) ? 1u : 0u;
  }
  n = wave_sum(n);
  if (lane_id() == 0) sm[threadIdx.x >> 6] = n;
  __syncthreads();
  if (threadIdx.x == 0) cnt[blockIdx.x] = sm[0] + sm[1] + sm[2] + sm[3];
}
__global__ __launch_bounds__(IV_NT) void iv_emit_k(uint32_t ncp, uint64_t S, uint32_t nb, CovArrays A, const uint64_t* __restrict__ sp,
                                                   const double* __restrict__ sv, const uint32_t* __restrict__ off, const uint32_t* __restrict__ tile_b,
                                                   uint32_t cap, int32_t* __restrict__ iv_tid, int32_t* __restrict__ iv_start, int32_t* __restrict__ iv_end,
                                                   double* __restrict__ iv_val) {
  __shared__ uint32_t sm[8];
  uint32_t run = off[blockIdx.x];
#pragma unroll 1
  for (uint32_t r = 0; r < IV_ROWS; ++r) {
    const uint64_t q64 = (uint64_t)blockIdx.x * IV_TILE + (uint64_t)r * IV_NT + threadIdx.x;
    const uint32_t q = (uint32_t)q64;
    const bool e = q64 < ncp && iv_emits(sp, sv, q);
    uint32_t tot;
    const uint32_t o = run + block_excl_sum<uint32_t, IV_NT>(e ? 1u : 0u, sm, &tot);
    run += tot;
    if (!e || o >= cap) continue;
    uint32_t nx = q + 1;
    while (nx < ncp && !cp_kept(sp, sv, nx)) ++nx;
    const uint64_t endp = nx < ncp ? (sp[nx] & ~(1ull << 63)) : S;
    const uint64_t p = sp[q] & ~(1ull << 63);
    const uint32_t tl = (uint32_t)(p / COV_W);
    uint32_t lo = tile_b[tl], hi = tile_b[tl + 1] + 1u;
    if (hi > nb) hi = nb;
    while (hi - lo > 1) {
      const uint32_t mid = lo + ((hi - lo) >> 1);
      if (A.b_off[mid] <= p)
        lo = mid;
      else
        hi = mid;
    }
    const int32_t s0 = A.b_start[lo] - 1 + (int32_t)(p - A.b_off[lo]);
    iv_tid[o] = A.b_tid[lo];
    iv_start[o] = s0;
    iv_end[o] = s0 + (int32_t)(endp - p);
    iv_val[o] = sv[q];
  }
}

__global__ void cov_tile_bundle_k(uint32_t ntiles, uint32_t nb, const uint64_t* __restrict__ b_off, uint32_t* __restrict__ tile_b) {
  const uint32_t t = blockIdx.x * blockDim.x + threadIdx.x;
  if (t > ntiles) return;
  const uint64_t p = (uint64_t)t * COV_W;
  uint32_t lo = 0, hi = nb;
  while (hi - lo > 1) {
    const uint32_t mid = lo + ((hi - lo) >> 1);
    if (b_off[mid] <= p)
      lo = mid;
    else
      hi = mid;
  }
  tile_b[t] = lo;
}

struct ClTiles {
  uint32_t* first;
  uint32_t* tb;
  uint32_t* cnt;
  uint32_t cap;
};
constexpr uint32_t CL_SC_NB = 3, CL_SC_S = 4, CL_SC_NSPILL = 5, CL_SC_NSL = 12, CL_SC_REFUSED = 13;

struct ClChunks {
  uint32_t *base, *cnt, *tbase;
  uint32_t* j;
  uint64_t* cs;
};
template <uint32_t NT>
__device__ __forceinline__ void cl_scan_block(uint32_t nt, const uint32_t* __restrict__ hcnt, const long long* __restrict__ xsum,
                                              uint32_t* __restrict__ hbase, long long* __restrict__ xbase, uint32_t* sh ,
                                              long long* sx ) {
  const uint32_t per = (nt + NT - 1u) / NT, i0 = threadIdx.x * per, i1 = i0 + per < nt ? i0 + per : nt;
  uint32_t h = 0;
  long long x = 0;
  for (uint32_t q0 = i0; q0 < i1; q0 += 8u) {
    uint32_t h8[8];
    long long x8[8];
#pragma unroll
    for (uint32_t u = 0; u < 8u; ++u) {
      h8[u] = q0 + u < i1 ? __hip_atomic_load(hcnt + q0 + u, __ATOMIC_RELAXED, __HIP_MEMORY_SCOPE_AGENT) : 0u;
      x8[u] = q0 + u < i1 ? __hip_atomic_load(xsum + q0 + u, __ATOMIC_RELAXED, __HIP_MEMORY_SCOPE_AGENT) : 0ll;
    }
#pragma unroll
    for (uint32_t u = 0; u < 8u; ++u) {
      h += h8[u];
      x += x8[u];
    }
  }
  uint32_t hi_ = h;
  long long xi_ = x;
#pragma unroll
  for (int d = 1; d < 64; d <<= 1) {
    const uint32_t oh = __shfl_up(hi_, d, 64);
    const long long ox = __shfl_up(xi_, d, 64);
    if ((int)lane_id() >= d) {
      hi_ += oh;
      xi_ += ox;
    }
  }
  if (lane_id() == 63) {
    sh[threadIdx.x >> 6] = hi_;
    sx[threadIdx.x >> 6] = xi_;
  }
  __syncthreads();
  uint32_t rh = hi_ - h;
  long long rx = xi_ - x;
  for (uint32_t q = 0; q < (threadIdx.x >> 6); ++q) {
    rh += sh[q];
    rx += sx[q];
  }
  for (uint32_t q0 = i0; q0 < i1; q0 += 8u) {
    uint32_t h8[8];
    long long x8[8];
#pragma unroll
    for (uint32_t u = 0; u < 8u; ++u) {
      h8[u] = q0 + u < i1 ? __hip_atomic_load(hcnt + q0 + u, __ATOMIC_RELAXED, __HIP_MEMORY_SCOPE_AGENT) : 0u;
      x8[u] = q0 + u < i1 ? __hip_atomic_load(xsum + q0 + u, __ATOMIC_RELAXED, __HIP_MEMORY_SCOPE_AGENT) : 0ll;
    }
#pragma unroll
    for (uint32_t u = 0; u < 8u; ++u) {
      if (q0 + u < i1) {
        hbase[q0 + u] = rh;
        xbase[q0 + u] = rx;
      }
      rh += h8[u];
      rx += x8[u];
    }
  }
}

template <bool EMIT>
__global__ __launch_bounds__(CB_NT) void cl_heads_k(uint32_t m, CovArrays A, const uint4* __restrict__ part ,
                                                    uint32_t* __restrict__ hcnt, long long* __restrict__ xsum, const uint32_t* __restrict__ hbase,
                                                    const long long* __restrict__ xbase, const uint32_t* __restrict__ cig_off,
                                                    const uint32_t* __restrict__ cig, ClTiles T, ClChunks L, uint64_t* __restrict__ sc,
                                                    uint32_t* __restrict__ err, uint32_t* __restrict__ done, uint32_t* __restrict__ hbase_out,
                                                    long long* __restrict__ xbase_out) {
  constexpr uint32_t NWV = CB_NT / 64;
  __shared__ CbAgg wl[CB_ROWS * NWV];
  __shared__ uint32_t smu[CB_ROWS * NWV];
  __shared__ long long smx[CB_ROWS * NWV];
  __shared__ uint32_t lcnt[EMIT ? COV_SW : 1];
  __shared__ uint16_t l_j[EMIT ? CB_TILE : 1];
  __shared__ uint32_t l_cs[EMIT ? CB_TILE : 1];
  __shared__ uint32_t s_tbase, s_nsl, s_np, s_slbase;
  __shared__ uint64_t s_cs0, s_cs1;
  const CbOp op{};
  const CbAgg none{0, INT32_MIN, INT32_MIN, 1u};
  auto un = [](const uint4& v) { return CbAgg{(int32_t)v.x, (int32_t)v.y, (int32_t)v.z, v.w}; };
  const uint32_t wv = threadIdx.x >> 6;
  uint32_t heads_tile = 0;
  long long x_tile = 0;
  bool bad = false, refused = false;
  if (EMIT) {
    if (threadIdx.x < COV_SW) lcnt[threadIdx.x] = 0;
    if (threadIdx.x == 0) s_nsl = s_np = 0;
  }
  int32_t t4[CB_ROWS][4], s4[CB_ROWS][4], e4[CB_ROWS][4];
#pragma unroll
  for (uint32_t r = 0; r < CB_ROWS; ++r) {
    const uint64_t i = (uint64_t)blockIdx.x * CB_TILE + ((uint64_t)r * CB_NT + threadIdx.x) * 4u;
    cb_load4(A.tid, i, m, 0, t4[r]);
    cb_load4(A.start, i, m, 0, s4[r]);
    cb_load4(A.end, i, m, 0, e4[r]);
  }
  const CbAgg run0 = un(part[blockIdx.x]);
  const uint32_t hrun0 = EMIT ? hbase[blockIdx.x] : 0u;
  const long long xrun0 = EMIT ? xbase[blockIdx.x] : 0ll;
  CbAgg ex[CB_ROWS];
#pragma unroll
  for (uint32_t r = 0; r < CB_ROWS; ++r) {
    const uint64_t i = (uint64_t)blockIdx.x * CB_TILE + ((uint64_t)r * CB_NT + threadIdx.x) * 4u;
    CbAgg a = none;
#pragma unroll
    for (int e = 0; e < 4; ++e)
      if (i + e < m) a = op(a, CbAgg{t4[r][e], t4[r][e], e4[r][e], 1u});
    const CbAgg inc = wave_incl_scan_op(a, op);
    if (lane_id() == 63) wl[r * NWV + wv] = inc;
    ex[r] = shfl_up_t(inc, 1);
  }
  __syncthreads();
  {
    CbAgg acc = run0;
#pragma unroll
    for (uint32_t q = 0; q < CB_ROWS * NWV; ++q) {
      if (q % NWV == wv) ex[q / NWV] = lane_id() == 0 ? acc : op(acc, ex[q / NWV]);
      acc = op(acc, wl[q]);
    }
  }
  uint32_t hdn[CB_ROWS];
  uint32_t hinc[CB_ROWS];
  long long xs[CB_ROWS], xinc[CB_ROWS];
#pragma unroll
  for (uint32_t r = 0; r < CB_ROWS; ++r) {
    const uint64_t i = (uint64_t)blockIdx.x * CB_TILE + ((uint64_t)r * CB_NT + threadIdx.x) * 4u;
    uint32_t hd = 0, nh = 0;
    xs[r] = 0;
    CbAgg w = ex[r];
#pragma unroll
    for (int e = 0; e < 4; ++e) {
      if (i + e < m) {
        const bool first = w.last_tid == INT32_MIN;
        const bool head = first || t4[r][e] != w.last_tid || s4[r][e] > w.mx;
        if (head) {
          xs[r] += (long long)s4[r][e] - 1ll - (first ? 0ll : (long long)w.mx);
          hd |= 1u << e;
          ++nh;
        }
        w = op(w, CbAgg{t4[r][e], t4[r][e], e4[r][e], 1u});
      }
    }
    hdn[r] = hd | (nh << 4);
    uint32_t hi_ = nh;
    long long xi_ = xs[r];
#pragma unroll
    for (int d = 1; d < 64; d <<= 1) {
      const uint32_t oh = __shfl_up(hi_, d, 64);
      const long long ox = __shfl_up(xi_, d, 64);
      if ((int)lane_id() >= d) {
        hi_ += oh;
        xi_ += ox;
      }
    }
    if (lane_id() == 63) {
      smu[r * NWV + wv] = hi_;
      smx[r * NWV + wv] = xi_;
    }
    hinc[r] = hi_;
    xinc[r] = xi_;
  }
  __syncthreads();
  uint32_t bf[CB_ROWS];
  long long cf[CB_ROWS];
  {
    uint32_t ah = 0;
    long long ax = 0;
#pragma unroll
    for (uint32_t q = 0; q < CB_ROWS * NWV; ++q) {
      if (q % NWV == wv) {
        bf[q / NWV] = hrun0 + ah + hinc[q / NWV] - (hdn[q / NWV] >> 4);
        cf[q / NWV] = xrun0 + ax + xinc[q / NWV] - xs[q / NWV];
      }
      ah += smu[q];
      ax += smx[q];
    }
    heads_tile = ah;
    x_tile = ax;
  }
  if (EMIT) {
    const uint32_t hd_all = (hdn[0] & 15u) | ((hdn[1] & 15u) << 4) | ((hdn[2] & 15u) << 8) | ((hdn[3] & 15u) << 12);
    static_assert(CB_ROWS == 4, "the row selects below");
#define CL_ROW(a, r) ((r) == 0 ? a[0] : (r) == 1 ? a[1] : (r) == 2 ? a[2] : a[3])
    const int32_t vt[CB_ROWS] = {ex[0].last_tid, ex[1].last_tid, ex[2].last_tid, ex[3].last_tid};
    const int32_t vm[CB_ROWS] = {ex[0].mx, ex[1].mx, ex[2].mx, ex[3].mx};
#pragma unroll 1
    for (uint32_t r = 0; r < CB_ROWS; ++r) {
      const uint64_t i = (uint64_t)blockIdx.x * CB_TILE + ((uint64_t)r * CB_NT + threadIdx.x) * 4u;
      int32_t rt[4], rs[4], re[4];
      cb_load4(A.tid, i, m, 0, rt);
      cb_load4(A.start, i, m, 0, rs);
      cb_load4(A.end, i, m, 0, re);
      const int32_t pst = i > 0 && i < m ? A.start[i - 1] : 0;
      const uint32_t hd = (hd_all >> (4u * r)) & 15u;
      long long C = CL_ROW(cf, r);
      uint32_t b = CL_ROW(bf, r);
      int32_t v_tid = CL_ROW(vt, r), v_mx = CL_ROW(vm, r);
      uint64_t prev_cs = i > 0 && i < m ? (uint64_t)((long long)pst - 1ll - C) : 0ull;
      uint64_t pk4 = 0;
#pragma unroll
      for (int e = 0; e < 4; ++e) {
        const uint64_t j = i + e;
        if (j < m) {
          const bool head = (hd >> e) & 1u;
          const bool run_head = v_tid == INT32_MIN || rt[e] != v_tid;
          const int32_t prev_start = e == 0 ? pst : rs[e - 1];
          if (!run_head && rs[e] < prev_start) bad = true;
          b += head ? 1u : 0u;
          if (head) C += (long long)rs[e] - 1ll - (v_tid == INT32_MIN ? 0ll : (long long)v_mx);
          const uint32_t bundle = b - 1u;
          const uint64_t cs = (uint64_t)((long long)rs[e] - 1ll - C);
          pk4 |= (uint64_t)((uint32_t)(cs % COV_W) | (head ? 0x8000u : 0u)) << (16 * e);
          if (head) {
            A.b_tid[bundle] = rt[e];
            A.b_start[bundle] = rs[e];
            A.b_off[bundle] = cs;
          }
          const uint64_t tl = cs / COV_W;
          if (r == 0 && threadIdx.x == 0 && e == 0) {
            s_tbase = (uint32_t)tl;
            s_cs0 = cs;
          }
          if (j + 1 == m || j + 1 == ((uint64_t)blockIdx.x + 1u) * CB_TILE) s_cs1 = cs;
          for (uint64_t tp = j ? prev_cs / COV_W + 1u : 0u; tp <= tl; ++tp) {
            if (tp >= T.cap) {
              refused = true;
              break;
            }
            T.first[tp] = (uint32_t)j;
            T.tb[tp] = bundle - ((head && cs > tp * COV_W) ? 1u : 0u);
          }
          v_mx = (!run_head && v_mx > re[e]) ? v_mx : re[e];
          v_tid = rt[e];
          if (j + 1 == m) {
            const uint64_t S = (uint64_t)((long long)v_mx - C);
            const uint64_t nt = (S + COV_W - 1) / COV_W;
            sc[CL_SC_NB] = (uint64_t)bundle + 1u;
            sc[CL_SC_S] = S;
            if (nt >= T.cap) {
              refused = true;
            } else {
              for (uint64_t u = tl + 1; u <= nt; ++u) {
                T.first[u] = m;
                T.tb[u] = bundle;
              }
            }
          }
          if ((uint32_t)(cs % COV_W) + (uint32_t)(re[e] - rs[e] + 1) > (uint32_t)COV_W) {
            const uint32_t k = atomicAdd(&s_nsl, 1u);
            l_j[k] = (uint16_t)(j - (uint64_t)blockIdx.x * CB_TILE);
            l_cs[k] = (uint32_t)cs;
          }
          prev_cs = cs;
        }
      }
      if (i + 3 < m) {
        *reinterpret_cast<uint64_t*>(A.pk + i) = pk4;
      } else {
        for (int e = 0; e < 4; ++e)
          if (i + e < m) A.pk[i + e] = (uint16_t)(pk4 >> (16 * e));
      }
    }
#undef CL_ROW
    __syncthreads();
  }
  if (!EMIT) {
    if (threadIdx.x == 0) {
      __hip_atomic_store(hcnt + blockIdx.x, heads_tile, __ATOMIC_RELAXED, __HIP_MEMORY_SCOPE_AGENT);
      __hip_atomic_store(xsum + blockIdx.x, x_tile, __ATOMIC_RELAXED, __HIP_MEMORY_SCOPE_AGENT);
    }
    if (cb_last_block(done)) cl_scan_block<CB_NT>(gridDim.x, hcnt, xsum, hbase_out, xbase_out, smu, smx);
  }
  if (EMIT) {
    const uint32_t nsl = s_nsl, tbase = s_tbase;
    const uint64_t cs0 = s_cs0;
    if (s_cs1 - cs0 >= (1ull << 32)) refused = true;
    auto full_cs = [&](uint32_t k) { return cs0 + (uint64_t)(uint32_t)(l_cs[k] - (uint32_t)cs0); };
    if (nsl) {
      if (threadIdx.x == 0) s_slbase = (uint32_t)atomicAdd((unsigned long long*)&sc[CL_SC_NSL], (unsigned long long)nsl);
      uint32_t np = 0;
      for (uint32_t k = threadIdx.x; k < nsl; k += CB_NT) {
        const uint32_t ri = A.ridx[(uint64_t)blockIdx.x * CB_TILE + l_j[k]];
        const uint32_t c0 = cig_off[ri];
        for_each_spill_piece(full_cs(k), cig + c0, cig_off[ri + 1] - c0, [&](uint32_t t, uint32_t, uint32_t) {
          ++np;
          if (t >= T.cap)
            refused = true;
          else if (t - tbase < COV_SW)
            atomicAdd(&lcnt[t - tbase], 1u);
// ... 596 lines not shown
  if (threadIdx.x == 0) ucnt[h] = run;
  __syncthreads();
  }
}
__global__ void jh_write_k(uint32_t nblk, const uint32_t* __restrict__ ucnt, const uint32_t* __restrict__ uoff, const uint32_t* __restrict__ off,
                           const uint64_t* __restrict__ hi2, const uint64_t* __restrict__ lo2, const double* __restrict__ pv2, uint32_t cap,
                           int32_t* __restrict__ j_tid, int32_t* __restrict__ j_start, int32_t* __restrict__ j_end, uint8_t* __restrict__ j_strand,
                           double* __restrict__ j_val) {
  const uint32_t h = (blockIdx.x * blockDim.x + threadIdx.x) >> 6;
  if (h >= nblk) return;
  const uint32_t n = ucnt[h], o0 = uoff[h], b0 = off[h];
  for (uint32_t u = lane_id(); u < n; u += 64) {
    const uint32_t o = o0 + u;
    if (o >= cap) break;
    const uint64_t kh = hi2[b0 + u], kl = lo2[b0 + u];
    const int32_t start = (int32_t)(uint32_t)(kh & 0xFFFFFFFFu);
    j_tid[o] = (int32_t)(uint32_t)(kh >> 32);
    j_start[o] = start - 1;
    j_end[o] = start + (int32_t)(uint32_t)(kl >> 8) - 1;
    j_strand[o] = (uint8_t)(kl & 0xFFu);
    j_val[o] = pv2[b0 + u];
  }
}

}

namespace {
__global__ void sample_convert_k(uint32_t n, const double* __restrict__ v, float denom, int64_t* __restrict__ cnt, float* __restrict__ heat) {
  uint32_t i = blockIdx.x * blockDim.x + threadIdx.x;
  if (i >= n) return;
  unsigned long long c = (unsigned long long)v[i];
  cnt[i] = (int64_t)c;
  const float mint = 0.1f, maxt = 1.5f;
  const float mult = (maxt - mint);
  heat[i] = ((float)c / denom) * mult + mint;
}
}

constexpr uint32_t COV_SIDE_MIN = 1u << 16;
static int junc_branch(tbk_ctx* ctx, uint32_t m, const CovArrays& A, const tbk_cov_in* in, const uint32_t* jcnt, tbk_cov_out* out,
                       bool integral, uint64_t nj_known, uint32_t* nj_out, uint32_t* nju_out) {
  const uint32_t B = 256;
  uint64_t* sc = ctx->d_scalars;
  *nj_out = *nju_out = 0;
  const bool agg = integral && !ctx->dbg.no_junc_agg;
  uint32_t* joff = nullptr;
  uint32_t nj;
  if (agg && nj_known != ~0ull) {
    if (nj_known >= (1ull << 32)) return TBK_E2BIG;
    nj = (uint32_t)nj_known;
  } else {
    joff = ws_alloc<uint32_t>(ctx, m);
    if (!joff) return TBK_ENOMEM;
    TBK_TRY(tbk_exscan_u32(ctx, jcnt, joff, m, sc + 7));
    TBK_HIP(hipMemcpyAsync(ctx->h_scalars + 7, sc + 7, sizeof(uint64_t), hipMemcpyDeviceToHost, ctx->stream));
    TBK_HIP(hipStreamSynchronize(ctx->stream));
    nj = (uint32_t)ctx->h_scalars[7];
  }
  *nj_out = nj;
  if (!nj) return 0;
  SortBufs sb;
  sb.hi = ws_alloc<uint64_t>(ctx, nj);
  sb.lo = ws_alloc<uint64_t>(ctx, nj);
  sb.val = ws_alloc<uint32_t>(ctx, nj);
  sb.hi2 = ws_alloc<uint64_t>(ctx, nj);
  sb.lo2 = ws_alloc<uint64_t>(ctx, nj);
  sb.val2 = ws_alloc<uint32_t>(ctx, nj);
  uint32_t* head = ws_alloc<uint32_t>(ctx, nj);
  uint32_t* hoff = ws_alloc<uint32_t>(ctx, nj);
  if (!hoff) return TBK_ENOMEM;
  uint32_t ns = nj;
  double* pv = nullptr;
  if (agg) {
    pv = ws_alloc<double>(ctx, nj);
    if (!pv) return TBK_ENOMEM;
    TBK_HIP(hipMemsetAsync(sc + 11, 0, 3 * sizeof(uint64_t), ctx->stream));
    TBK_LAUNCH(ctx, "junc_agg", junc_agg_k, cdiv(m, JA_REC), 256, 0, m, A, in->tid, in->pos, in->cig_off, in->cig, in->strand, in->yc, jcnt, sb.hi, sb.lo,
               pv, (unsigned long long*)(sc + 11));
    if (!ctx->dbg.junc_radix) {
      const uint32_t nblk = cdiv(m, JH_REC);
      uint64_t* bkey = ws_alloc<uint64_t>(ctx, nblk);
      uint32_t* hcnt = ws_alloc<uint32_t>(ctx, (size_t)nblk * 2);
      uint32_t* hoff2 = ws_alloc<uint32_t>(ctx, nblk);
      uint32_t* ucnt = ws_alloc<uint32_t>(ctx, nblk);
      uint32_t* uoff = ws_alloc<uint32_t>(ctx, nblk);
      double* pv2 = ws_alloc<double>(ctx, nj);
      if (!bkey || !hcnt || !hoff2 || !ucnt || !uoff || !pv2) return TBK_ENOMEM;
      uint32_t* hfill = hcnt + nblk;
      TBK_HIP(hipMemsetAsync(hcnt, 0, (size_t)nblk * 2 * 4, ctx->stream));
      TBK_LAUNCH(ctx, "junc_home", jh_blockkey_k, cdiv(nblk, B), B, 0, nblk, A, in->tid, in->pos, bkey);
      TBK_LAUNCH(ctx, "junc_home", jh_home_k, cdiv(nj, B), B, 0, (const unsigned long long*)(sc + 11), nj, sb.hi, nblk, bkey, head , hcnt);
      TBK_TRY(tbk_exscan_u32(ctx, hcnt, hoff2, nblk, nullptr));
      TBK_LAUNCH(ctx, "junc_home", jh_scatter_k, cdiv(nj, B), B, 0, (const unsigned long long*)(sc + 11), nj, sb.hi, sb.lo, pv, head, hoff2, hfill, sb.hi2,
                 sb.lo2, pv2);
      uint32_t jh_cap = JH_CAP;
      if (ctx->dbg.jh_cap && ctx->dbg.jh_cap < JH_CAP) jh_cap = ctx->dbg.jh_cap;
      uint32_t* big = hoff;
      TBK_LAUNCH(ctx, "junc_sort", jh_sort_k, cdiv((uint64_t)nblk * 64, B), B, 0, nblk, hcnt, hoff2, sb.hi2, sb.lo2, pv2, ucnt, big, sc + 13);
      TBK_LAUNCH(ctx, "junc_sort", jh_sort_big_k, 512, 256, 0, big, sc + 13, hcnt, hoff2, sb.hi2, sb.lo2, pv2, ucnt, sc + 12, jh_cap);
      TBK_TRY(tbk_exscan_u32(ctx, ucnt, uoff, nblk, sc + 9));
      TBK_LAUNCH(ctx, "junc_write", jh_write_k, cdiv((uint64_t)nblk * 64, B), B, 0, nblk, ucnt, uoff, hoff2, sb.hi2, sb.lo2, pv2, out->cap_junctions, out->j_tid,
                 out->j_start, out->j_end, out->j_strand, out->j_val);
      TBK_HIP(hipMemcpyAsync(ctx->h_scalars + 9, sc + 9, 4 * sizeof(uint64_t), hipMemcpyDeviceToHost, ctx->stream));
      TBK_HIP(hipStreamSynchronize(ctx->stream));
      if (!ctx->h_scalars[12]) {
        *nju_out = (uint32_t)ctx->h_scalars[9];
        return tbk_check_launch(ctx, "junctions");
      }
      ns = (uint32_t)ctx->h_scalars[11];
    } else {
      TBK_HIP(hipMemcpyAsync(ctx->h_scalars + 11, sc + 11, sizeof(uint64_t), hipMemcpyDeviceToHost, ctx->stream));
      TBK_HIP(hipStreamSynchronize(ctx->stream));
      ns = (uint32_t)ctx->h_scalars[11];
    }
    TBK_LAUNCH(ctx, "junc_iota", junc_iota_k, cdiv(ns, B), B, 0, ns, sb.val);
  } else {
    TBK_LAUNCH(ctx, "junc_fill", junc_fill_k, cdiv(m, B), B, 0, m, A, in->tid, in->pos, in->cig_off, in->cig, in->strand, joff, sb.hi, sb.lo, sb.val);
  }
  TBK_TRY(tbk_radix_sort128(ctx, &sb, ns));
  TBK_LAUNCH(ctx, "junc_head", junc_head_k, cdiv(ns, B), B, 0, ns, sb.hi, sb.lo, head);
  TBK_TRY(tbk_exscan_u32(ctx, head, hoff, ns, sc + 9));
  if (integral) {
    TBK_LAUNCH(ctx, "junc_head_write", junc_head_write_k, cdiv(ns, B), B, 0, ns, sb.hi, sb.lo, head, hoff, out->cap_junctions, out->j_tid,
               out->j_start, out->j_end, out->j_strand, out->j_val);
    if (agg)
      TBK_LAUNCH(ctx, "junc_sum", junc_sum_k<true>, cdiv(ns, B), B, 0, ns, A, sb.val, head, hoff, pv, out->cap_junctions, out->j_val);
    else
      TBK_LAUNCH(ctx, "junc_sum", junc_sum_k<false>, cdiv(ns, B), B, 0, ns, A, sb.val, head, hoff, in->yc, out->cap_junctions, out->j_val);
  } else {
    TBK_LAUNCH(ctx, "junc_write", junc_write_k, cdiv(nj, B), B, 0, nj, A, sb.hi, sb.lo, sb.val, head, hoff, in->yc, out->cap_junctions,
               out->j_tid, out->j_start, out->j_end, out->j_strand, out->j_val);
  }
  TBK_HIP(hipMemcpyAsync(ctx->h_scalars + 9, sc + 9, sizeof(uint64_t), hipMemcpyDeviceToHost, ctx->stream));
  TBK_HIP(hipStreamSynchronize(ctx->stream));
  *nju_out = (uint32_t)ctx->h_scalars[9];
  return tbk_check_launch(ctx, "junctions");
}

struct JuncSide {
  TbkWorker* w = nullptr;
  bool th = false;
  int rc = 0;
  int join() {
    if (th) {
      w->wait();
      th = false;
    }
    return rc;
  }
  ~JuncSide() { (void)join(); }
};

static int cov_intervals_lean(tbk_ctx* ctx, const tbk_cov_in* in, tbk_cov_out* out, CovArrays A, uint32_t m, bool all_valid, uint64_t sum_abs,
                              const uint4* pre_part) {
  const uint32_t B = 256;
  uint64_t* sc = ctx->d_scalars;
  const uint32_t cbt = cdiv(m, CB_TILE);
  uint4* own_part = pre_part ? nullptr : ws_alloc<uint4>(ctx, cbt);
  const uint4* cpart = pre_part ? pre_part : own_part;
  uint32_t* hcnt = ws_alloc<uint32_t>(ctx, cbt);
  uint32_t* hbase = ws_alloc<uint32_t>(ctx, cbt);
  long long* xsum = ws_alloc<long long>(ctx, cbt);
  long long* xbase = ws_alloc<long long>(ctx, cbt);
  ClChunks L;
  L.base = ws_alloc<uint32_t>(ctx, cbt);
  L.cnt = ws_alloc<uint32_t>(ctx, cbt);
  L.tbase = ws_alloc<uint32_t>(ctx, cbt);
  L.j = ws_alloc<uint32_t>(ctx, m);
  L.cs = ws_alloc<uint64_t>(ctx, m);
  ClTiles T;
  uint64_t cap64 = (uint64_t)m / 8u > (1ull << 20) ? (uint64_t)m / 8u : (1ull << 20);
  if (ctx->dbg.cov_tile_cap) cap64 = ctx->dbg.cov_tile_cap;
  T.cap = (uint32_t)cap64;
  T.first = ws_alloc<uint32_t>(ctx, (size_t)T.cap + 1);
  T.tb = ws_alloc<uint32_t>(ctx, (size_t)T.cap + 1);
  T.cnt = ws_alloc<uint32_t>(ctx, (size_t)T.cap + 1);
  if (!cpart || !hcnt || !hbase || !xsum || !xbase || !L.base || !L.cnt || !L.tbase || !L.j || !L.cs || !T.first || !T.tb || !T.cnt) return TBK_ENOMEM;
  TBK_HIP(hipMemsetAsync(T.cnt, 0, ((size_t)T.cap + 1) * 4, ctx->stream));
  uint32_t* done = (uint32_t*)(sc + 16);
  TBK_HIP(hipMemsetAsync(done, 0, sizeof(uint64_t), ctx->stream));
  if (!pre_part) TBK_LAUNCH(ctx, "cov_bundles", cb_agg_k, cbt, CB_NT, 0, m, A.tid, A.end, own_part, done);
  TBK_LAUNCH(ctx, "cov_bundles", cl_heads_k<false>, cbt, CB_NT, 0, m, A, cpart, hcnt, xsum, (const uint32_t*)nullptr, (const long long*)nullptr, in->cig_off,
             in->cig, T, L, sc, ctx->d_err, done + 1, hbase, xbase);
  TBK_LAUNCH(ctx, "cov_place", cl_heads_k<true>, cbt, CB_NT, 0, m, A, cpart, hcnt, xsum, hbase, xbase, in->cig_off, in->cig, T, L, sc, ctx->d_err,
             (uint32_t*)nullptr, (uint32_t*)nullptr, (long long*)nullptr);
  uint32_t eb = 0;
  TBK_TRY(tbk_sync_err(ctx, &eb));
  if (eb) return tbk_derr_to_status(ctx, eb);
  if (ctx->h_scalars[CL_SC_REFUSED]) return 1;
  const uint32_t nb = (uint32_t)ctx->h_scalars[CL_SC_NB];
  const uint64_t S = ctx->h_scalars[CL_SC_S], nspill = ctx->h_scalars[CL_SC_NSPILL];
  const uint32_t nsl = (uint32_t)ctx->h_scalars[CL_SC_NSL];
  out->span_bases = S;
  const uint32_t ntiles = (uint32_t)((S + COV_W - 1) / COV_W);
  if (nspill >= (1ull << 32)) return TBK_E2BIG;
  const uint64_t cp_cap64 = 2ull * ((uint64_t)in->n_cigar_ops + nspill) + nb + ntiles + 16;
  if (cp_cap64 >= (1ull << 32)) return TBK_E2BIG;
  const uint32_t cp_cap = (uint32_t)cp_cap64;
  uint32_t* tile_off = ws_alloc<uint32_t>(ctx, (size_t)ntiles + 1);
  uint32_t* tile_fill = ws_alloc<uint32_t>(ctx, (size_t)ntiles + 1);
  uint32_t* sp_seg = ws_alloc<uint32_t>(ctx, nspill + 1);
  uint32_t* sp_rec = ws_alloc<uint32_t>(ctx, nspill + 1);
  uint64_t* cp_pos = ws_alloc<uint64_t>(ctx, cp_cap);
  double* cp_val = ws_alloc<double>(ctx, cp_cap);
  uint32_t* tile_cp_base = ws_alloc<uint32_t>(ctx, ntiles);
  uint32_t* tile_cp_cnt = ws_alloc<uint32_t>(ctx, ntiles);
  uint32_t* icnt = ws_alloc<uint32_t>(ctx, ntiles);
  uint32_t* ioff = ws_alloc<uint32_t>(ctx, ntiles);
  ClTileOut O;
  O.ecnt = ws_alloc<uint32_t>(ctx, ntiles);
  O.fv = ws_alloc<double>(ctx, ntiles);
  O.lv = ws_alloc<double>(ctx, ntiles);
  uint32_t* cp_alloc = (uint32_t*)(sc + 10);
  if (!tile_off || !tile_fill || !sp_seg || !sp_rec || !cp_pos || !cp_val || !tile_cp_base || !tile_cp_cnt || !icnt || !ioff || !O.ecnt || !O.fv || !O.lv)
    return TBK_ENOMEM;
  TBK_TRY(tbk_exscan_u32(ctx, T.cnt, tile_off, ntiles + 1, nullptr));
  if (nsl) {
    TBK_HIP(hipMemsetAsync(tile_fill, 0, ((size_t)ntiles + 1) * 4, ctx->stream));
    TBK_LAUNCH(ctx, "cov_spill_fill", cl_spill_fill_k, cbt, B, 0, L, A, in->cig_off, in->cig, tile_off, tile_fill, sp_seg, sp_rec);
  }
#define COV_TILE_LAUNCH(ACC, ID)                                                                                                  \
  TBK_LAUNCH(ctx, "cov_tile", (cov_tile_k<ACC, ID, true>), ntiles, COVT_NT, 0, m, S, A, in->cig_off, in->cig, in->yc, T.first, tile_off, \
             sp_seg, sp_rec, cp_pos, cp_val, tile_cp_base, tile_cp_cnt, cp_alloc, cp_cap, ctx->d_err, O)
  const bool small = sum_abs < (1ull << 31);
  if (!ntiles) {
  } else if (small && all_valid)
    COV_TILE_LAUNCH(int32_t, true);
  else if (small)
    COV_TILE_LAUNCH(int32_t, false);
  else if (all_valid)
    COV_TILE_LAUNCH(long long, true);
  else
    COV_TILE_LAUNCH(long long, false);
#undef COV_TILE_LAUNCH
  if (ntiles) TBK_LAUNCH(ctx, "cov_iv_count", cl_iv_count_k, cdiv(ntiles, B), B, 0, ntiles, O, icnt);
  TBK_TRY(tbk_exscan_u32(ctx, icnt, ioff, ntiles, sc + 8));
  if (ntiles)
    TBK_LAUNCH(ctx, "cov_iv_write", cl_iv_emit_k, ntiles, 256, 0, ntiles, S, nb, A, cp_pos, cp_val, tile_cp_base, tile_cp_cnt, O, ioff, T.tb, out->cap_intervals,
               out->iv_tid, out->iv_start, out->iv_end, out->iv_val);
  return 0;
}

static int cov_run(tbk_ctx* ctx, const tbk_cov_in* in, tbk_cov_out* out, bool sample_mode) {
  const uint32_t n = in->n_records;
  const bool want_cov = out->cap_intervals > 0, want_j = out->cap_junctions > 0;
  out->n_intervals = out->n_junctions = 0;
  out->n_bases = 0;
  out->span_bases = 0;
  if (n == 0) return 0;
  const uint32_t B = 256;
  uint64_t* sc = ctx->d_scalars;
  TBK_HIP(hipMemsetAsync(sc, 0, 16 * sizeof(uint64_t), ctx->stream));

  uint32_t* valid = ws_alloc<uint32_t>(ctx, n);
  uint32_t* vpos = ws_alloc<uint32_t>(ctx, n);
  CovArrays A;
  A.ridx = ws_alloc<uint32_t>(ctx, n);
  A.start = ws_alloc<int32_t>(ctx, n);
  A.end = ws_alloc<int32_t>(ctx, n);
  A.tid = ws_alloc<int32_t>(ctx, n);
  A.bhead = ws_alloc<uint32_t>(ctx, n);
  A.bid = ws_alloc<uint32_t>(ctx, n);
  A.cs = ws_alloc<uint64_t>(ctx, n);
  A.pk = ws_alloc<uint16_t>(ctx, n);
  A.yi = ws_alloc<int32_t>(ctx, n);
  A.b_tid = ws_alloc<int32_t>(ctx, n);
  A.b_start = ws_alloc<int32_t>(ctx, n);
  A.b_end = ws_alloc<int32_t>(ctx, n);
  A.b_span = ws_alloc<uint32_t>(ctx, n);
  A.b_off = ws_alloc<uint64_t>(ctx, n + 1);
  uint32_t* jcnt = want_j ? ws_alloc<uint32_t>(ctx, n) : nullptr;
  if (!A.b_off || (want_j && !jcnt)) return TBK_ENOMEM;
  uint32_t nj = 0, nju = 0;
  JuncSide side;

  const bool all_valid = in->flag == nullptr;
  if (!all_valid) {
    TBK_LAUNCH(ctx, "cov_valid", cov_valid_k, cdiv(n, B), B, 0, in->flag, n, valid);
    TBK_TRY(tbk_exscan_u32(ctx, valid, vpos, n, sc + 2));
  }
  const auto& V = ctx->view_prep;
  const bool prepared = V.valid && all_valid && !sample_mode && in->mem == TBK_MEM_DEVICE && in->cig == V.cig && n == V.n &&
                        !ctx->dbg.cov_prep;
  uint32_t eb = 0;
  if (prepared) {
    A.ridx = V.ridx;
    A.start = V.start;
    A.end = V.end;
    A.tid = const_cast<int32_t*>(in->tid);
    A.yi = V.yi;
    if (want_j) jcnt = V.jcnt;
    eb = V.err;
    if (!want_cov) eb &= ~(uint32_t)(TBK_DERR_FATALOP | TBK_DERR_NCIGAR);
    ctx->h_scalars[0] = V.n_bases;
    ctx->h_scalars[1] = V.sum_abs;
  } else {
    TBK_LAUNCH(ctx, "cov_prep", cov_prep_k, (cdiv(n, B) < 4096u ? cdiv(n, B) : 4096u), B, 0, n, all_valid ? (const uint32_t*)nullptr : valid, vpos, in->tid, in->pos, in->cig_off, in->cig,
               sample_mode ? (const double*)nullptr : in->yc, want_cov ? 1 : 0, A, jcnt, sc, ctx->d_err);
    TBK_TRY(tbk_sync_err(ctx, &eb));
  }
  const bool fractional = (eb & TBK_DERR_FRACTIONAL) != 0;
  eb &= ~TBK_DERR_FRACTIONAL;
  if (eb) return tbk_derr_to_status(ctx, eb);
  if (fractional && !prepared) TBK_HIP(hipMemsetAsync(ctx->d_err, 0, sizeof(uint32_t), ctx->stream));
  const uint32_t m = all_valid ? n : (uint32_t)ctx->h_scalars[2];
  out->n_bases = ctx->h_scalars[0];
  const uint64_t sum_abs = ctx->h_scalars[1];
  const bool integral = !fractional && !sample_mode && sum_abs < (1ull << 52);
  const uint64_t nj_known = prepared ? V.n_junc : (want_j ? ctx->h_scalars[14] : ~0ull);
  if (m == 0) return 0;
  if (want_j && want_cov && m >= COV_SIDE_MIN) {
    tbk_ctx* jc = tbk_side_ctx(ctx);
    if (jc) {
      const size_t hint = (size_t)m * 8 + (size_t)in->n_cigar_ops * 64 + ((size_t)4 << 20);
      if (!ctx->side_worker) ctx->side_worker = new TbkWorker();
      side.w = ctx->side_worker;
      side.th = true;
      side.w->post([&side, jc, hint, m, &A, in, jcnt, out, integral, nj_known, &nj, &nju]() {
        side.rc = tbk_side_begin(jc, hint);
        if (side.rc == 0) side.rc = junc_branch(jc, m, A, in, jcnt, out, integral, nj_known, &nj, &nju);
        tbk_side_end(jc);
      });
    }
  }

  bool lean_done = false;
  if (want_cov && !fractional && !sample_mode && !ctx->dbg.cov_legacy && !ctx->dbg.cov_bundle_scan) {
    const size_t ws_mark = ctx->ws_off;
    const uint4* pre_part = (prepared && V.agg && V.agg_tiles == cdiv(m, CB_TILE)) ? (const uint4*)V.agg : nullptr;
    const int lrc = cov_intervals_lean(ctx, in, out, A, m, all_valid, sum_abs, pre_part);
    if (lrc < 0) return lrc;
    lean_done = lrc == 0;
    if (!lean_done) {
      if (ctx->ws_overflow.empty()) ctx->ws_off = ws_mark;
      TBK_HIP(hipMemsetAsync(sc + 3, 0, 11 * sizeof(uint64_t), ctx->stream));
    }
  }
  if (!lean_done) {
  {
    if (ctx->dbg.cov_bundle_scan) {
      BundleLoad ld{A.tid, A.end};
      BundleAux ax{A.tid, A.start};
      BundleHead hd{};
      BundleStore st{A, m, sc + 3, ctx->d_err};
      SegMax ident{INT32_MIN, 0u};
      TBK_TRY((scan_two_run<4, SegMax, SegMaxOp, uint32_t, SoPlusU32, BundleLoad, BundleAux, BundleHead, BundleStore>(ctx, "cov_bundles", m, ld, ax, hd, st, SegMaxOp{}, ident,
                                                                                                          SoPlusU32{}, 0u)));
    } else {
      const uint32_t cbt = cdiv(m, CB_TILE);
      uint4* cpart = ws_alloc<uint4>(ctx, cbt);
      uint32_t* hcnt = ws_alloc<uint32_t>(ctx, cbt);
      uint32_t* hbase = ws_alloc<uint32_t>(ctx, cbt);
      if (!cpart || !hcnt || !hbase) return TBK_ENOMEM;
      uint32_t* done = (uint32_t*)(sc + 16);
      TBK_HIP(hipMemsetAsync(done, 0, sizeof(uint64_t), ctx->stream));
      TBK_LAUNCH(ctx, "cov_bundles", cb_agg_k, cbt, CB_NT, 0, m, A.tid, A.end, cpart, done);
      TBK_LAUNCH(ctx, "cov_bundles", cb_heads_k<false>, cbt, CB_NT, 0, m, A, cpart, hcnt, (const uint32_t*)nullptr, sc + 3, ctx->d_err);
      TBK_TRY(tbk_exscan_u32(ctx, hcnt, hbase, cbt, nullptr));
      TBK_LAUNCH(ctx, "cov_bundles", cb_heads_k<true>, cbt, CB_NT, 0, m, A, cpart, hcnt, hbase, sc + 3, ctx->d_err);
    }
  }
  TBK_TRY(tbk_sync_err(ctx, &eb));
  if (eb) return tbk_derr_to_status(ctx, eb);
  const uint32_t nb = (uint32_t)ctx->h_scalars[3];
  TBK_LAUNCH(ctx, "cov_bundle_span", cov_bundle_span_k, cdiv(nb, B), B, 0, nb, A);
  TBK_TRY(tbk_exscan_u32_u64(ctx, A.b_span, A.b_off, nb, sc + 4));
  TBK_HIP(hipMemcpyAsync(A.b_off + nb, sc + 4, sizeof(uint64_t), hipMemcpyDeviceToDevice, ctx->stream));
  TBK_HIP(hipMemcpyAsync(ctx->h_scalars, sc, 16 * sizeof(uint64_t), hipMemcpyDeviceToHost, ctx->stream));
  TBK_HIP(hipStreamSynchronize(ctx->stream));
  const uint64_t S = ctx->h_scalars[4];
  out->span_bases = S;
  const uint64_t ntiles64 = (S + COV_W - 1) / COV_W;
  if (ntiles64 >= (1ull << 31)) return TBK_E2BIG;
  const uint32_t ntiles = (uint32_t)ntiles64;

  if (want_cov) {
    uint32_t* tile_cnt = ws_alloc<uint32_t>(ctx, ntiles + 1);
    uint32_t* tile_off = ws_alloc<uint32_t>(ctx, ntiles + 1);
    uint32_t* tile_fill = ws_alloc<uint32_t>(ctx, ntiles + 1);
    uint32_t* tile_first = ws_alloc<uint32_t>(ctx, ntiles + 1);
    if (!tile_fill || !tile_first) return TBK_ENOMEM;
    TBK_HIP(hipMemsetAsync(tile_cnt, 0, (size_t)(ntiles + 1) * 4, ctx->stream));
    TBK_HIP(hipMemsetAsync(tile_fill, 0, (size_t)(ntiles + 1) * 4, ctx->stream));
    TBK_LAUNCH(ctx, "cov_cs_count", cov_cs_count_k, cdiv(m, B), B, 0, m, A, in->cig_off, in->cig, tile_cnt, tile_first, ntiles);
    TBK_TRY(tbk_exscan_u32(ctx, tile_cnt, tile_off, ntiles + 1, sc + 5));
    TBK_HIP(hipMemcpyAsync(ctx->h_scalars, sc, 16 * sizeof(uint64_t), hipMemcpyDeviceToHost, ctx->stream));
    TBK_HIP(hipStreamSynchronize(ctx->stream));
    const uint64_t nspill = ctx->h_scalars[5];
    if (nspill >= (1ull << 32)) return TBK_E2BIG;
    uint32_t* sp_seg = ws_alloc<uint32_t>(ctx, nspill + 1);
    uint32_t* sp_rec = ws_alloc<uint32_t>(ctx, nspill + 1);
    const uint64_t cp_cap64 = 2ull * ((uint64_t)in->n_cigar_ops + nspill) + nb + ntiles + 16;
    if (cp_cap64 >= (1ull << 32)) return TBK_E2BIG;
    const uint32_t cp_cap = (uint32_t)cp_cap64;
    uint64_t* cp_pos = ws_alloc<uint64_t>(ctx, cp_cap);
    double* cp_val = ws_alloc<double>(ctx, cp_cap);
    uint64_t* sp = ws_alloc<uint64_t>(ctx, cp_cap);
    double* sv = ws_alloc<double>(ctx, cp_cap);
    uint32_t* tile_cp_base = ws_alloc<uint32_t>(ctx, ntiles);
    uint32_t* tile_cp_cnt = ws_alloc<uint32_t>(ctx, ntiles);
    uint32_t* tile_cp_off = ws_alloc<uint32_t>(ctx, ntiles);
    uint32_t* cp_alloc = (uint32_t*)(sc + 10);
    if (!cp_pos || !cp_val || !sp || !sv || !tile_cp_off) return TBK_ENOMEM;
    if (nspill)
      TBK_LAUNCH(ctx, "cov_spill_fill", cov_spill_fill_k, cdiv(m, B), B, 0, m, A, in->cig_off, in->cig, tile_off, tile_fill,
                 sp_seg, sp_rec);
    if (!ntiles) {
    } else if (sample_mode) {
      TBK_LAUNCH(ctx, "sample_tile", (cov_tile_ordered_k<true>), ntiles, COV_NT, 0, m, S, A, in->cig_off, in->cig, in->yc, in->yx,
                 tile_first, tile_off, sp_seg, sp_rec, cp_pos, cp_val, tile_cp_base, tile_cp_cnt, cp_alloc, cp_cap, ctx->d_err);
    } else if (fractional) {
      TBK_LAUNCH(ctx, "cov_tile_ordered", (cov_tile_ordered_k<false>), ntiles, COV_NT, 0, m, S, A, in->cig_off, in->cig, in->yc,
                 in->yx, tile_first, tile_off, sp_seg, sp_rec, cp_pos, cp_val, tile_cp_base, tile_cp_cnt, cp_alloc, cp_cap, ctx->d_err);
    } else {
#define COV_TILE_LAUNCH(ACC, ID)                                                                                                   \
  TBK_LAUNCH(ctx, "cov_tile", (cov_tile_k<ACC, ID, false>), ntiles, COVT_NT, 0, m, S, A, in->cig_off, in->cig, in->yc, tile_first, tile_off, \
             sp_seg, sp_rec, cp_pos, cp_val, tile_cp_base, tile_cp_cnt, cp_alloc, cp_cap, ctx->d_err, ClTileOut{nullptr, nullptr, nullptr})
      const bool small = sum_abs < (1ull << 31);
      if (small && all_valid)
        COV_TILE_LAUNCH(int32_t, true);
      else if (small)
        COV_TILE_LAUNCH(int32_t, false);
      else if (all_valid)
        COV_TILE_LAUNCH(long long, true);
      else
        COV_TILE_LAUNCH(long long, false);
#undef COV_TILE_LAUNCH
    }
    TBK_TRY(tbk_exscan_u32(ctx, tile_cp_cnt, tile_cp_off, ntiles, sc + 6));
    if (ntiles)
      TBK_LAUNCH(ctx, "cov_cp_gather", cov_cp_gather_k, ntiles, 64, 0, ntiles, tile_cp_base, tile_cp_cnt, tile_cp_off, cp_pos, cp_val,
                 sp, sv);
    TBK_TRY(tbk_sync_err(ctx, &eb));
    if (eb) return tbk_derr_to_status(ctx, eb);
    const uint32_t ncp = (uint32_t)ctx->h_scalars[6];
    if (ncp) {
      const uint32_t ivt = cdiv(ncp, IV_TILE);
      uint32_t* icnt = ws_alloc<uint32_t>(ctx, ivt);
      uint32_t* ioff = ws_alloc<uint32_t>(ctx, ivt);
      uint32_t* tile_b = ws_alloc<uint32_t>(ctx, (size_t)ntiles + 2);
      if (!icnt || !ioff || !tile_b) return TBK_ENOMEM;
      TBK_LAUNCH(ctx, "cov_iv_write", cov_tile_bundle_k, cdiv(ntiles + 1, B), B, 0, ntiles, nb, A.b_off, tile_b);
      TBK_LAUNCH(ctx, "cov_iv_count", iv_count_k, ivt, IV_NT, 0, ncp, sp, sv, icnt);
      TBK_TRY(tbk_exscan_u32(ctx, icnt, ioff, ivt, sc + 8));
      TBK_LAUNCH(ctx, "cov_iv_write", iv_emit_k, ivt, IV_NT, 0, ncp, S, nb, A, sp, sv, ioff, tile_b, out->cap_intervals, out->iv_tid, out->iv_start,
                 out->iv_end, out->iv_val);
    }
  }

  }

  if (want_j && !side.th) TBK_TRY(junc_branch(ctx, m, A, in, jcnt, out, integral, nj_known, &nj, &nju));
  TBK_TRY(tbk_sync_err(ctx, &eb));
  if (eb) return tbk_derr_to_status(ctx, eb);
  TBK_TRY(tbk_check_launch(ctx, "coverage"));
  if (side.th) {
    const int jrc = side.join();
    ctx->side_times_pending = true;
    if (jrc != 0) {
      ctx->last_error = ctx->side_ctx->last_error;
      return jrc;
    }
  }
  if (want_cov) {
    out->n_intervals = (uint32_t)ctx->h_scalars[8];
    if (out->n_intervals > out->cap_intervals) return TBK_E2BIG;
  }
  if (want_j && nj) {
    out->n_junctions = nju;
    if (out->n_junctions > out->cap_junctions) return TBK_E2BIG;
  }
  return 0;
}

int tbk_coverage_device(tbk_ctx* ctx, const tbk_cov_in* in, tbk_cov_out* out) { return cov_run(ctx, in, out, false); }

int tbk_sample_device(tbk_ctx* ctx, const tbk_cov_in* in, int32_t num_samples, tbk_sample_out* out) {
  out->n_intervals = 0;
  if (out->cap_intervals == 0 || !out->iv_tid || !out->iv_start || !out->iv_end || !out->iv_count || !out->iv_heat) return TBK_EINVAL;
  tbk_cov_out co;
  memset(&co, 0, sizeof(co));
  co.mem = TBK_MEM_DEVICE;
  co.cap_intervals = out->cap_intervals;
// ... 15 lines not shown
```

### tiebrush_amd/csrc/tbk_api.hip

```cpp
#include <sys/mman.h>

#include <algorithm>
#include <chrono>
#include <mutex>
#include <vector>
#include <new>

#include "tbk_internal.h"

namespace {
std::mutex g_reg_m;
struct RegEntry {
  void* p;
  int users;
};
std::vector<RegEntry> g_reg;
}

static void release_registered(tbk_ctx* ctx) {
  if (ctx->registered.empty()) return;
  (void)hipStreamSynchronize(ctx->stream);
  const auto r0 = std::chrono::steady_clock::now();
  struct RP {
    tbk_ctx* c;
// ... 302 lines not shown
}
static int out_dalloc(tbk_ctx* ctx, const tbk_groups_out* out, size_t cap, size_t n, bool keep, tbk_groups_out* dout) {
  dout->mem = TBK_MEM_DEVICE;
  TBK_TRY(dalloc_if(ctx, keep || out->rep, cap, &dout->rep));
  TBK_TRY(dalloc_if(ctx, keep || out->yc, cap, &dout->yc));
  TBK_TRY(dalloc_if(ctx, keep || out->yx, cap, &dout->yx));
  TBK_TRY(dalloc_if(ctx, keep || out->yd, cap, &dout->yd));
  TBK_TRY(dalloc(ctx, out->g_start, cap, &dout->g_start));
  TBK_TRY(dalloc(ctx, out->g_end, cap, &dout->g_end));
  TBK_TRY(dalloc(ctx, out->rec_group, n, &dout->rec_group));
  TBK_TRY(dalloc(ctx, out->rep_effend, cap, &dout->rep_effend));
  TBK_TRY(dalloc(ctx, out->g_key, 2 * cap, &dout->g_key));
  return 0;
}
static int out_d2h(tbk_ctx* ctx, tbk_groups_out* out, const tbk_groups_out* dout, size_t n) {
  const size_t g = dout->n_groups;

  TBK_TRY(d2h(ctx, out->rep, dout->rep, g));
  TBK_TRY(d2h(ctx, out->yc, dout->yc, g));
  TBK_TRY(d2h(ctx, out->yx, dout->yx, g));
  TBK_TRY(d2h(ctx, out->yd, dout->yd, g));
  TBK_TRY(d2h(ctx, out->g_start, dout->g_start, g));
  TBK_TRY(d2h(ctx, out->g_end, dout->g_end, g));
  TBK_TRY(d2h(ctx, out->rec_group, dout->rec_group, n));
  TBK_TRY(d2h(ctx, out->rep_effend, dout->rep_effend, g));
  TBK_TRY(d2h(ctx, out->g_key, dout->g_key, 2 * g));
  TBK_HIP(hipStreamSynchronize(ctx->stream));
  return 0;
}
static int keep_results(tbk_ctx* ctx, const tbk_groups_out* d) {
  const size_t g = d->n_groups;
  auto al = [](size_t x) { return (x + 255) & ~(size_t)255; };
  const size_t need = 2 * al(g * 8) + 2 * al(g * 4) + 256;
  if (need > ctx->kept_cap) {
    if (ctx->kept) (void)hipFree(ctx->kept);
    ctx->kept = nullptr;
    ctx->kept_cap = 0;
    if (hipMalloc((void**)&ctx->kept, need + need / 8) != hipSuccess) {
      (void)hipGetLastError();
      ctx->last_error = "keep_results: hipMalloc failed";
      return TBK_ENOMEM;
    }
    ctx->kept_cap = need + need / 8;
  }
  char* p = ctx->kept;
  ctx->kept_yc = (double*)p, p += al(g * 8);
  ctx->kept_yx = (int64_t*)p, p += al(g * 8);
  ctx->kept_rep = (uint32_t*)p, p += al(g * 4);
  ctx->kept_yd = (int32_t*)p;
  if (g) {
    TBK_HIP(hipMemcpyAsync(ctx->kept_yc, d->yc, g * 8, hipMemcpyDeviceToDevice, ctx->stream));
    TBK_HIP(hipMemcpyAsync(ctx->kept_yx, d->yx, g * 8, hipMemcpyDeviceToDevice, ctx->stream));
    TBK_HIP(hipMemcpyAsync(ctx->kept_rep, d->rep, g * 4, hipMemcpyDeviceToDevice, ctx->stream));
    TBK_HIP(hipMemcpyAsync(ctx->kept_yd, d->yd, g * 4, hipMemcpyDeviceToDevice, ctx->stream));
  }
  ctx->kept_n = (uint32_t)g;
  return 0;
}

hipStream_t tbk_aux_stream(tbk_ctx* ctx) {
  if (!ctx->aux) {
    if (hipStreamCreateWithFlags(&ctx->aux, hipStreamNonBlocking) != hipSuccess) ctx->aux = nullptr;
    if (ctx->aux && hipEventCreateWithFlags(&ctx->aux_done, hipEventDisableTiming) != hipSuccess) {
      (void)hipStreamDestroy(ctx->aux);
      ctx->aux = nullptr;
    }
  }
  return ctx->aux;
}

tbk_ctx* tbk_side_ctx(tbk_ctx* ctx) {
  if (!ctx->side_ctx && tbk_create(ctx->device, &ctx->side_ctx) != 0) ctx->side_ctx = nullptr;
  if (ctx->side_ctx) {
    ctx->side_ctx->profiling = ctx->profiling;
    ctx->side_ctx->dbg = ctx->dbg;
  }
  return ctx->side_ctx;
}
int tbk_side_begin(tbk_ctx* side, size_t arena_hint) {
  if (hipSetDevice(side->device) != hipSuccess) return TBK_EHIP;
  tbk_prof_begin_call(side);
  return ws_begin_call(side, arena_hint);
}
void tbk_side_end(tbk_ctx* side) { tbk_prof_end_call(side); }

static void merge_side_times(tbk_ctx* ctx) {
  if (!ctx->side_times_pending || !ctx->side_ctx) return;
  ctx->side_times_pending = false;
  for (auto& t : ctx->side_ctx->last_times) {
    bool found = false;
    for (auto& u : ctx->last_times)
      if (strcmp(u.name, t.name) == 0) {
        u.ms += t.ms;
        u.launches += t.launches;
        found = true;
        break;
      }
    if (!found) ctx->last_times.push_back(t);
  }
}

static int yd_stage_on(tbk_ctx* run_on, void* job, size_t hint) {
  if (hipSetDevice(run_on->device) != hipSuccess) return TBK_EHIP;
  tbk_prof_begin_call(run_on);
  int rc = ws_begin_call(run_on, hint);
  if (rc == 0) rc = tbk_collapse_yd_run(run_on, job);
  tbk_prof_end_call(run_on);
  return rc;
}

static int finish_yd(tbk_ctx* ctx) {
  if (!ctx->yd_pending) return 0;
  ctx->yd_worker->wait();
  ctx->yd_pending = false;
  ctx->ws_base_off = 0;
  if (ctx->yd_ctx) {
    ctx->last_times = ctx->yd_ctx->last_times;
    if (ctx->yd_rc != 0) ctx->last_error = ctx->yd_ctx->last_error;
  }
  return ctx->yd_rc;
}

void tbk_debug_parse(const char* spec, TbkDebug* out) {
  *out = TbkDebug();
  if (!spec) return;
  std::string s(spec);
  size_t at = 0;
  while (at < s.size()) {
    size_t end = s.find(',', at);
    if (end == std::string::npos) end = s.size();
    const std::string kv = s.substr(at, end - at);
    at = end + 1;
    const size_t eq = kv.find('=');
    const std::string k = kv.substr(0, eq), v = eq == std::string::npos ? std::string("1") : kv.substr(eq + 1);
    const unsigned long long u = strtoull(v.c_str(), nullptr, 0);
    const bool on = v != "0";
    if (k == "path") out->path = v == "sort" ? 1 : (v == "window" ? 2 : 0);
    else if (k == "raw") out->raw = on ? 1 : 0;
    else if (k == "sort") out->sort = v == "radix" ? 1 : (v == "runs" ? 2 : 0);
    else if (k == "scan") out->scan = v == "lookback" ? 1 : (v == "3pass" ? 2 : 0);
    else if (k == "hash_mask") out->hash_mask = (uint32_t)u;
    else if (k == "qhash_mask") out->qhash_mask = u;
    else if (k == "yd_wave_min") out->yd_wave_min = (uint32_t)u;
    else if (k == "yd_bgrid") out->yd_bgrid = (uint32_t)u;
    else if (k == "yd_radix") out->yd_radix = on;
    else if (k == "yd_literal") out->yd_literal = on;
    else if (k == "yd_front") out->yd_front_split = v == "split";
    else if (k == "yd_own_arena") out->yd_own_arena = on;
    else if (k == "wg_stats") out->wg_stats = on;
    else if (k == "wg_og") out->wg_og = (uint32_t)u;
    else if (k == "wg_dense_verify") out->wg_dense_verify = on;
    else if (k == "wg_rank_merge") out->wg_rank_merge = on;
    else if (k == "wg_back") out->wg_back_split = v == "split";
    else if (k == "cov_legacy") out->cov_legacy = on;
    else if (k == "cov_bundle_scan") out->cov_bundle_scan = on;
    else if (k == "cov_prep") out->cov_prep = on;
    else if (k == "cov_tile_cap") out->cov_tile_cap = u;
    else if (k == "junc_radix") out->junc_radix = on;
    else if (k == "no_junc_agg") out->no_junc_agg = on;
    else if (k == "jh_cap") out->jh_cap = (uint32_t)u;
    else if (k == "index_chain") out->index_chain = on;
    else if (k == "no_register") out->no_register = on;
    else if (k == "phases") out->phases = on;
    else if (k == "no_bounce") out->no_bounce = on;
    else if (k == "fmt_slice") out->fmt_slice = u;
  }
}

extern "C" {

int tbk_abi_version(void) { return TBK_ABI_VERSION; }

int tbk_set_debug(tbk_ctx* ctx, const char* spec) {
  if (!ctx) return TBK_EINVAL;
  tbk_debug_parse(spec, &ctx->dbg);
  if (ctx->yd_ctx) ctx->yd_ctx->dbg = ctx->dbg;
  if (ctx->side_ctx) ctx->side_ctx->dbg = ctx->dbg;
  return 0;
}

const char* tbk_strerror(int s) {
  switch (s) {
    case TBK_OK: return "ok";
    case TBK_EINVAL: return "invalid argument";
    case TBK_ENOMEM: return "out of memory";
    case TBK_EHIP: return "HIP runtime error";
    case TBK_E2BIG: return "output capacity too small";
    case TBK_EUNSUPPORTED: return "option or input outside the supported/pinned semantics";
    case TBK_EUNSORTED: return "input not coordinate-sorted";
    case TBK_EFATALOP: return "unknown opcode (tiecov accepts only M/I/D/N/S)";
    case TBK_ECOLLISION: return "key hash collision survived all reseeds";
    case TBK_ENODEVICE: return "no usable gfx950 device";
  }
  return "unknown status";
}

int tbk_create(int device_ordinal, tbk_ctx** out) {
  if (!out) return TBK_EINVAL;
  *out = nullptr;
  int ndev = 0;
  if (hipGetDeviceCount(&ndev) != hipSuccess || ndev <= 0 || device_ordinal < 0 || device_ordinal >= ndev) return TBK_ENODEVICE;
  tbk_ctx* ctx = new (std::nothrow) tbk_ctx();
  if (!ctx) return TBK_ENOMEM;
  ctx->device = device_ordinal;
  tbk_debug_parse(getenv("TBK_DEBUG"), &ctx->dbg);
  bool ok = hipSetDevice(device_ordinal) == hipSuccess;
  hipDeviceProp_t prop;
  if (ok && hipGetDeviceProperties(&prop, device_ordinal) == hipSuccess) ctx->num_cu = prop.multiProcessorCount;
  ok = ok && hipStreamCreateWithFlags(&ctx->own_stream, hipStreamNonBlocking) == hipSuccess;
  ctx->stream = ctx->own_stream;
  ok = ok && hipMalloc((void**)&ctx->d_scalars, 64 * sizeof(uint64_t)) == hipSuccess;
  if (ok) ctx->d_err = (uint32_t*)(ctx->d_scalars + 15);
  ok = ok && hipHostMalloc((void**)&ctx->h_scalars, (64 + 4096) * sizeof(uint64_t), hipHostMallocDefault) == hipSuccess;
  if (!ok) {
    tbk_destroy(ctx);
    return TBK_EHIP;
  }
  *out = ctx;
  return 0;
}

int tbk_collapse_finish_yd(tbk_ctx* ctx) {
  if (!ctx) return TBK_EINVAL;
  return finish_yd(ctx);
}

void tbk_destroy(tbk_ctx* ctx) {
  if (!ctx) return;
  (void)finish_yd(ctx);
  tbk_bam_release(ctx);
  delete ctx->yd_worker;
  ctx->yd_worker = nullptr;
  delete ctx->side_worker;
  ctx->side_worker = nullptr;
  if (ctx->yd_ctx) {
    tbk_destroy(ctx->yd_ctx);
    ctx->yd_ctx = nullptr;
  }
  if (ctx->side_ctx) {
    tbk_destroy(ctx->side_ctx);
    ctx->side_ctx = nullptr;
  }
  (void)hipSetDevice(ctx->device);
  if (ctx->stream) (void)hipStreamSynchronize(ctx->stream);
  release_registered(ctx);
  for (auto& c : ctx->ws_overflow) (void)hipFree(c.first);
  for (auto e : ctx->ev_pool) (void)hipEventDestroy(e);
  if (ctx->ws && !ctx->ws_borrowed) (void)hipFree(ctx->ws);
  if (ctx->d_view) (void)hipFree(ctx->d_view);
  if (ctx->d_unpack) (void)hipFree(ctx->d_unpack);
  if (ctx->kept) (void)hipFree(ctx->kept);
  if (ctx->d_names) (void)hipFree(ctx->d_names);
  if (ctx->d_name_off) (void)hipFree(ctx->d_name_off);
  for (void* p : ctx->fmt_pin)
    if (p) (void)hipHostFree(p);
  if (ctx->bounce) (void)hipHostFree(ctx->bounce);
  tbk_enc_free(ctx);
  tbk_ix_free(ctx);
  tbk_stager_free(ctx);
  if (ctx->d_scalars) (void)hipFree(ctx->d_scalars);
  if (ctx->h_scalars) (void)hipHostFree(ctx->h_scalars);
  if (ctx->aux_done) (void)hipEventDestroy(ctx->aux_done);
  if (ctx->stage_ev) (void)hipEventDestroy(ctx->stage_ev);
  if (ctx->aux) (void)hipStreamDestroy(ctx->aux);
  if (ctx->own_stream) (void)hipStreamDestroy(ctx->own_stream);
  delete ctx;
}

int tbk_last_route(const tbk_ctx* ctx, tbk_collapse_route* out) {
  if (!ctx || !out) return TBK_EINVAL;
  *out = ctx->route;
  return 0;
}
const char* tbk_last_error(const tbk_ctx* ctx) { return ctx ? ctx->last_error.c_str() : ""; }

int tbk_set_stream(tbk_ctx* ctx, void* s) {
  if (!ctx) return TBK_EINVAL;
  ctx->stream = s == TBK_STREAM_DEFAULT ? (hipStream_t) nullptr : (s ? (hipStream_t)s : ctx->own_stream);
  return 0;
}
void* tbk_get_stream(tbk_ctx* ctx) { return ctx ? (void*)ctx->stream : nullptr; }

int tbk_set_profiling(tbk_ctx* ctx, int enabled) {
  if (!ctx) return TBK_EINVAL;
  ctx->profiling = enabled != 0;
  return 0;
}

int tbk_kernel_times(tbk_ctx* ctx, tbk_kernel_time* out, int cap) {
  if (!ctx) return TBK_EINVAL;
  int n = (int)ctx->last_times.size();
  for (int i = 0; i < n && i < cap; ++i) out[i] = ctx->last_times[i];
  return n;
}

namespace {
struct PinnedBlk {
  void* raw;
  size_t raw_bytes;
};
std::mutex g_pin_m;
std::vector<std::pair<void*, PinnedBlk>> g_pin;
constexpr size_t PIN_HUGE = (size_t)2 << 20;
}

int tbk_host_alloc(size_t bytes, void** out) {
// ... 376 lines not shown
```

### tiebrush_amd/csrc/tbk_internal.h

```cpp
#pragma once
#include <hip/hip_runtime.h>
#include <stdint.h>
#include <stdio.h>
#include <string.h>

#include <string>
#include <condition_variable>
#include <functional>
#include <mutex>
#include <thread>
#include <utility>
#include <vector>

#include "../../include/tbk.h"

enum : uint32_t {
  TBK_DERR_UNSORTED = 1u << 0,
  TBK_DERR_COLLISION = 1u << 1,
  TBK_DERR_FATALOP = 1u << 2,
  TBK_DERR_SPAN = 1u << 3,
  TBK_DERR_NCIGAR = 1u << 4,
  TBK_DERR_FRACTIONAL = 1u << 5,
  TBK_DERR_OVERFLOW = 1u << 6,
  TBK_DERR_INTERNAL = 1u << 7,
  TBK_DERR_BIGBUCKET = 1u << 8,
  TBK_DERR_RAWORDER = 1u << 9
};

struct KTime {
  const char* name;
  hipEvent_t a, b;
};

struct TbkWorker {
  std::thread th;
  std::mutex m;
  std::condition_variable cv;
  std::function<void()> job;
  bool busy = false, quit = false, started = false;
  void post(std::function<void()> j) {
    {
      std::lock_guard<std::mutex> lk(m);
      if (!started) {
        started = true;
        th = std::thread([this]() {
          std::unique_lock<std::mutex> lk2(m);
          for (;;) {
            cv.wait(lk2, [&] { return quit || (bool)job; });
            if (quit) return;
            std::function<void()> run = std::move(job);
            job = nullptr;
            lk2.unlock();
            run();
            lk2.lock();
            busy = false;
            cv.notify_all();
          }
        });
      }
      job = std::move(j);
      busy = true;
    }
    cv.notify_all();
  }
  void wait() {
    std::unique_lock<std::mutex> lk(m);
    cv.wait(lk, [&] { return !busy; });
  }
  ~TbkWorker() {
    {
      std::lock_guard<std::mutex> lk(m);
      quit = true;
    }
    cv.notify_all();
    if (th.joinable()) th.join();
  }
};

struct TbkDebug {
  int path = 0;
  int raw = -1;
  int sort = 0;
  int scan = 0;
  uint32_t hash_mask = 0xFFFFFFFFu;
  uint64_t qhash_mask = ~0ull;
  uint32_t yd_wave_min = 0;
  uint32_t yd_bgrid = 0;
  bool yd_radix = false;
  bool yd_literal = false;
  bool yd_front_split = false;
  bool yd_own_arena = false;
  uint32_t wg_og = 0;
  bool wg_stats = false;
  bool wg_dense_verify = false, wg_rank_merge = false;
  bool wg_back_split = false;
  bool cov_legacy = false, cov_bundle_scan = false, cov_prep = false, junc_radix = false, no_junc_agg = false;
  uint64_t cov_tile_cap = 0;
  uint32_t jh_cap = 0;
  bool index_chain = false;
  bool no_register = false;
  bool no_bounce = false;
  bool phases = false;
  uint64_t fmt_slice = 0;
};
void tbk_debug_parse(const char* spec, TbkDebug* out);

struct tbk_ctx {
  int device = 0;
  TbkDebug dbg;
  hipStream_t own_stream = nullptr;
  hipStream_t stream = nullptr;
  hipStream_t aux = nullptr;
  hipEvent_t aux_done = nullptr;
  char* ws = nullptr;
  size_t ws_cap = 0, ws_off = 0;
  size_t ws_top = 0;
  bool ws_top_mode = false;
  bool ws_borrowed = false;
  std::vector<std::pair<char*, size_t>> ws_overflow;
  size_t ws_over_used = 0;
  uint32_t* d_err = nullptr;
  uint64_t* d_scalars = nullptr;
  uint64_t* h_scalars = nullptr;
  hipEvent_t stage_ev = nullptr;
  char* d_view = nullptr;
  size_t d_view_cap = 0;
  struct ViewPrep {
    bool valid = false;
    const void* cig = nullptr;
    uint32_t n = 0;
    int32_t *start = nullptr, *end = nullptr, *yi = nullptr;
    uint32_t *jcnt = nullptr, *ridx = nullptr;
    const void* agg = nullptr;
    uint32_t agg_tiles = 0;
    uint64_t n_bases = 0, sum_abs = 0, n_junc = 0;
    uint32_t err = 0;
  } view_prep;
  bool profiling = false;
  std::vector<KTime> ktimes;
  std::vector<hipEvent_t> ev_pool;
  size_t ev_used = 0;
  std::vector<tbk_kernel_time> last_times;
  std::string last_error;
  tbk_collapse_route route{};
  int num_cu = 256;
  void* yd_job = nullptr;
  tbk_ctx* yd_ctx = nullptr;
  TbkWorker* yd_worker = nullptr;
  bool yd_pending = false;
  int yd_rc = 0;
  size_t ws_base_off = 0;
  tbk_ctx* side_ctx = nullptr;
  TbkWorker* side_worker = nullptr;
  bool side_times_pending = false;
  std::vector<void*> registered;
  char* d_unpack = nullptr;
  size_t d_unpack_cap = 0;
  std::vector<uint8_t> unpack_tbm;
  void* bam_dev = nullptr;
  void* enc = nullptr;
  void* ix = nullptr;
  void* stager = nullptr;
  char* bounce = nullptr;
  char* kept = nullptr;
  size_t kept_cap = 0;
  uint32_t kept_n = 0;
  uint32_t* kept_rep = nullptr;
  double* kept_yc = nullptr;
  int64_t* kept_yx = nullptr;
  int32_t* kept_yd = nullptr;
  char* d_names = nullptr;
  uint64_t* d_name_off = nullptr;
  uint32_t n_names = 0;
  void* fmt_pin[2] = {nullptr, nullptr};
  size_t fmt_pin_cap = 0;
};
void tbk_stager_free(tbk_ctx* ctx);
void tbk_enc_free(tbk_ctx* ctx);
void tbk_ix_free(tbk_ctx* ctx);
struct TbkIxIn {
  uint32_t n;
  const uint8_t* pay;
  const uint64_t* ooff;
  uint32_t nmem;
  const uint64_t* cut;
  const uint64_t* moff;
  uint64_t ztotal;
};
int tbk_ix_check_opts(tbk_ctx* ctx, const tbk_ix_opts* ix);
int tbk_ix_build(tbk_ctx* ctx, const TbkIxIn& in, const tbk_ix_opts* ix, tbk_ix_part* part);
bool tbk_bam_dev_records(tbk_ctx* ctx, const uint8_t** inf, const uint64_t** rec, uint32_t* n);
bool tbk_bam_dev_is_tile(tbk_ctx* ctx, const tbk_soa_in* tile);
void* tbk_bam_dev_alloc(tbk_ctx* ctx, size_t bytes);
void tbk_bam_dev_compacted(tbk_ctx* ctx, uint64_t* rec, uint32_t n, const int32_t* tid);

hipStream_t tbk_aux_stream(tbk_ctx* ctx);
tbk_ctx* tbk_side_ctx(tbk_ctx* ctx);
int tbk_side_begin(tbk_ctx* side, size_t arena_hint);
void tbk_side_end(tbk_ctx* side);

#define TBK_HIP(call)                                                                            \
  do {                                                                                           \
    hipError_t _e = (call);                                                                      \
    if (_e != hipSuccess) {                                                                      \
      char _b[512];                                                                              \
      snprintf(_b, sizeof(_b), "%s:%d %s -> %s", __FILE__, __LINE__, #call, hipGetErrorString(_e)); \
      ctx->last_error = _b;                                                                      \
      return TBK_EHIP;                                                                           \
    }                                                                                            \
  } while (0)

#define TBK_TRY(expr)        \
  do {                       \
    int _rc = (expr);        \
    if (_rc != 0) return _rc; \
  } while (0)

int tbk_ws_reserve(tbk_ctx* ctx, size_t bytes);
int tbk_ws_presize(tbk_ctx* ctx, size_t bytes);
void* tbk_ws_alloc_raw(tbk_ctx* ctx, size_t bytes);
template <class T>
static inline T* ws_alloc(tbk_ctx* ctx, size_t n) {
  return (T*)tbk_ws_alloc_raw(ctx, n * sizeof(T));
}

hipEvent_t tbk_event(tbk_ctx* ctx);
static inline void tbk_prof_begin(tbk_ctx* ctx, const char* name) {
  if (!ctx->profiling) return;
  KTime k{name, tbk_event(ctx), tbk_event(ctx)};
  (void)hipEventRecord(k.a, ctx->stream);
  ctx->ktimes.push_back(k);
}
static inline void tbk_prof_end(tbk_ctx* ctx) {
  if (!ctx->profiling) return;
  (void)hipEventRecord(ctx->ktimes.back().b, ctx->stream);
}

#define TBK_LAUNCH(ctx, name, kern, grid, block, shmem, ...)                          \
  do {                                                                                \
    tbk_prof_begin(ctx, name);                                                        \
    hipLaunchKernelGGL(kern, dim3(grid), dim3(block), shmem, (ctx)->stream, __VA_ARGS__); \
    tbk_prof_end(ctx);                                                                \
  } while (0)

void tbk_prof_begin_call(tbk_ctx* ctx);
void tbk_prof_end_call(tbk_ctx* ctx);
int tbk_check_launch(tbk_ctx* ctx, const char* what);
extern "C" void tbk_bam_release(tbk_ctx* ctx);
void* tbk_stage_acquire(tbk_ctx* ctx);
void tbk_stage_release(tbk_ctx* ctx);
int tbk_sync_err(tbk_ctx* ctx, uint32_t* err_bits);
int tbk_derr_to_status(tbk_ctx* ctx, uint32_t bits);

static inline uint32_t cdiv(uint64_t a, uint64_t b) { return (uint32_t)((a + b - 1) / b); }

int tbk_exscan_u32(tbk_ctx* ctx, const uint32_t* in, uint32_t* out, uint32_t n, uint64_t* d_total);
int tbk_exscan_u32_u64(tbk_ctx* ctx, const uint32_t* in, uint64_t* out, uint32_t n, uint64_t* d_total);

struct SortBufs {
  uint64_t *hi, *lo;
  uint32_t* val;
  uint64_t *hi2, *lo2;
  uint32_t* val2;
};
int tbk_radix_sort128(tbk_ctx* ctx, SortBufs* b, uint32_t n, uint64_t only_hi = ~0ull, uint64_t only_lo = ~0ull,
                      bool masks_are_exact = false);
size_t tbk_radix_ws_bytes(uint32_t n);
int tbk_radix_sort_w64(tbk_ctx* ctx, uint64_t** w, uint64_t** w2, uint32_t n, uint64_t mask, bool mask_is_exact);
int tbk_sort_runs(tbk_ctx* ctx, SortBufs* b, uint32_t n_hi, const uint32_t* d_run_off, uint32_t nruns, uint32_t* err,
                  uint32_t* nbig_zeroed);

int tbk_collapse_device(tbk_ctx* ctx, const tbk_collapse_opts* o, const tbk_soa_in* in, tbk_groups_out* out);
int tbk_collapse_warm(tbk_ctx* ctx);
int tbk_collapse_yd_run(tbk_ctx* run_on, void* job);
int tbk_coverage_device(tbk_ctx* ctx, const tbk_cov_in* in, tbk_cov_out* out);
int tbk_cov_view_build(tbk_ctx* ctx, const int32_t* r_tid, const int32_t* r_pos, const uint8_t* r_strand, const uint32_t* r_cig_off,
                       const uint32_t* r_cig, const uint32_t* g_rep, const double* g_yc, const int64_t* g_yx, uint32_t ng, tbk_cov_in* view,
                       const uint64_t* g_key = nullptr);
int tbk_sample_device(tbk_ctx* ctx, const tbk_cov_in* in, int32_t num_samples, tbk_sample_out* out);
int tbk_format_device(tbk_ctx* ctx, const tbk_track_rows* rows, tbk_track_sink sink, void* user, uint64_t* out_bytes);
int tbk_names_upload(tbk_ctx* ctx, uint32_t n_names, const uint64_t* off, const char* bytes);
```

Before: 21.63 billion records/s.

## Fuse coverage head counting into groups-to-view gather and skip cl_heads pass

The count kernel now records per-wave bundle aggregates and per-wave cigar prefix offsets. The gather kernel uses them to compute per-tile head counts and gap sums inline, with no in-kernel block scan. Coverage then runs a single-block scan over the precomputed tables in place of the cl_heads_k<false> pass over all records. This removes one full pass over the view data and a shared-memory scan from gather. The cost is extra workspace, per-lane shuffle scans in gather, and a serial single-block scan over many tiles.

```diff
diff --git a/include/tbk.h b/include/tbk.h
--- a/include/tbk.h
+++ b/include/tbk.h
@@ -183,6 +183,7 @@
 int tbk_last_route(const tbk_ctx* ctx, tbk_collapse_route* out);
 int tbk_coverage_tile(tbk_ctx* ctx, const tbk_cov_in* in, tbk_cov_out* out);
 int tbk_sample_tile(tbk_ctx* ctx, const tbk_cov_in* in, int32_t num_samples, tbk_sample_out* out);
+int tbk_cov_heads_probe(tbk_ctx* ctx, uint32_t* hcnt, int64_t* xsum, uint32_t cap, uint32_t* n_tiles, uint32_t* from_view);
 
 int tbk_groups_to_cov_in(tbk_ctx* ctx, const tbk_soa_in* in, const tbk_groups_out* groups, tbk_cov_in* view);
 
diff --git a/tiebrush_amd/_lib.py b/tiebrush_amd/_lib.py
--- a/tiebrush_amd/_lib.py
+++ b/tiebrush_amd/_lib.py
@@ -23,7 +23,7 @@
            "tbk_shard_pack", "tbk_shard_unpack", "tbk_partial_keys", "tbk_partial_pack", "tbk_partial_unpack", "tbk_partial_reduce", "tbk_unpack_tile", "tbk_tile_join", "tbk_reserve_tile", "tbk_bgzf_deflate", "tbk_bam_encode", "tbk_kept_results", "tbk_warmup", "tbk_partial_stage_keys", "tbk_partial_stage_cands", "tbk_partial_stage_pack",
            "tbk_partial_pack_md", "tbk_partial_unpack_md", "tbk_partial_reduce_md", "tbk_track_names", "tbk_format_track", "tbk_bam_encode_indexed",
            "tbk_bam_decode_spans", "tbk_region_view", "tbk_cov_clip", "tbk_sample_clip", "tbk_bam_decode_file_spans", "tbk_tile_region", "tbk_last_route",
-           "tbk_regions_view", "tbk_cov_clip_regions", "tbk_sample_clip_regions", "tbk_tile_regions"]
+           "tbk_regions_view", "tbk_cov_clip_regions", "tbk_sample_clip_regions", "tbk_tile_regions", "tbk_cov_heads_probe"]
 
 
 class CollapseOpts(C.Structure):
@@ -159,6 +159,8 @@
     L.tbk_collapse_finish_yd.argtypes = [_P]
     L.tbk_coverage_tile.argtypes = [_P, C.POINTER(CovIn), C.POINTER(CovOut)]
     L.tbk_sample_tile.argtypes = [_P, C.POINTER(CovIn), C.c_int32, C.POINTER(SampleOut)]
+    L.tbk_cov_heads_probe.argtypes = [_P, _P, _P, C.c_uint32, C.POINTER(C.c_uint32), C.POINTER(C.c_uint32)]
+    L.tbk_cov_heads_probe.restype = C.c_int
     L.tbk_groups_to_cov_in.argtypes = [_P, C.POINTER(SoaIn), C.POINTER(GroupsOut), C.POINTER(CovIn)]
     L.tbk_bgzf_inflate.argtypes = [_P, _P, C.c_uint64, _P, C.c_uint64, C.POINTER(C.c_uint64), C.c_int]
     L.tbk_bam_decode.argtypes = [_P, C.c_uint32, _P, _P, _P, C.c_int, C.c_int, C.POINTER(SoaIn), _P]
diff --git a/tiebrush_amd/api.py b/tiebrush_amd/api.py
--- a/tiebrush_amd/api.py
+++ b/tiebrush_amd/api.py
@@ -171,6 +171,13 @@
         arr = (_lib.KernelTime * 128)()
         n = self.L.tbk_kernel_times(self.h, arr, 128)
         return {arr[i].name.decode(): (float(arr[i].ms), int(arr[i].launches)) for i in range(min(n, 128))}
+
+    def cov_heads_probe(self):
+        n, fv = C.c_uint32(0), C.c_uint32(0)
+        cap = 1 << 16
+        hcnt, xsum = np.zeros(cap, np.uint32), np.zeros(cap, np.int64)
+        self._check(self.L.tbk_cov_heads_probe(self.h, hcnt.ctypes.data, xsum.ctypes.data, cap, C.byref(n), C.byref(fv)), "tbk_cov_heads_probe")
+        return (hcnt[:n.value].copy(), xsum[:n.value].copy(), bool(fv.value)) if n.value else None
 
     def _alloc(self, device_mode, n, dtype):
         n = max(int(n), 1)
diff --git a/tiebrush_amd/csrc/cb_tiles.hpp b/tiebrush_amd/csrc/cb_tiles.hpp
--- a/tiebrush_amd/csrc/cb_tiles.hpp
+++ b/tiebrush_amd/csrc/cb_tiles.hpp
@@ -29,6 +29,56 @@
     if ((int)lane_id() >= d) v = op(o, v);
   }
   return v;
+}
+__device__ __forceinline__ bool cb_head_step(const CbAgg& before, int32_t tid, int32_t start, long long* x) {
+  const bool first = before.last_tid == INT32_MIN;
+  const bool head = first || tid != before.last_tid || start > before.mx;
+  *x = head ? (long long)start - 1ll - (first ? 0ll : (long long)before.mx) : 0ll;
+  return head;
+}
+struct CbLanes {
+  uint64_t runs;
+  uint32_t nvalid;
+  int32_t prev_tid;
+};
+__device__ __forceinline__ CbLanes cb_lanes(bool valid, int32_t tid) {
+  CbLanes w;
+  w.prev_tid = __shfl_up(tid, 1, 64);
+  w.runs = __ballot(valid && lane_id() > 0u && tid != w.prev_tid);
+  w.nvalid = (uint32_t)__popcll(__ballot(valid));
+  return w;
+}
+__device__ __forceinline__ CbAgg cb_wave_agg(const CbLanes& w, int32_t tid, int32_t end) {
+  if (w.nvalid == 0u) return CbAgg{0, INT32_MIN, INT32_MIN, 1u};
+  const uint32_t last_run = w.runs ? 63u - (uint32_t)__clzll((long long)w.runs) : 0u;
+  int32_t mx = lane_id() >= last_run && lane_id() < w.nvalid ? end : INT32_MIN;
+#pragma unroll
+  for (int d = 32; d >= 1; d >>= 1) {
+    const int32_t o = __shfl_xor(mx, d, 64);
+    mx = o > mx ? o : mx;
+  }
+  return CbAgg{__shfl(tid, 0, 64), __shfl(tid, (int)w.nvalid - 1, 64), mx, w.runs ? 0u : 1u};
+}
+__device__ __forceinline__ CbAgg cb_lane_before(const CbLanes& w, const CbAgg& carry, int32_t tid, int32_t end) {
+  const uint32_t ln = lane_id();
+  const uint64_t upto = w.runs & (~0ull >> (63u - ln));
+  const int run0 = upto ? 63 - __clzll((long long)upto) : 0;
+  int32_t inc = end;
+#pragma unroll
+  for (int d = 1; d < 64; d <<= 1) {
+    const int32_t o = __shfl_up(inc, d, 64);
+    if ((int)ln - d >= run0) inc = o > inc ? o : inc;
+  }
+  const int32_t mx_before = __shfl_up(inc, 1, 64);
+  if (ln == 0u) return carry;
+  CbAgg b;
+  b.first_tid = carry.first_tid;
+  b.last_tid = w.prev_tid;
+  const bool from_lane0 = (w.runs & (~0ull >> (64u - ln))) == 0ull;
+  const bool joins = from_lane0 && carry.last_tid != INT32_MIN && carry.last_tid == b.last_tid;
+  b.mx = joins && carry.mx > mx_before ? carry.mx : mx_before;
+  b.whole = 0u;
+  return b;
 }
 __device__ __forceinline__ void cb_put(uint64_t* p, uint64_t v) { __hip_atomic_store(p, v, __ATOMIC_RELAXED, __HIP_MEMORY_SCOPE_AGENT); }
 __device__ __forceinline__ uint64_t cb_get(const uint64_t* p) { return __hip_atomic_load(p, __ATOMIC_RELAXED, __HIP_MEMORY_SCOPE_AGENT); }
diff --git a/tiebrush_amd/csrc/collapse.hip b/tiebrush_amd/csrc/collapse.hip
--- a/tiebrush_amd/csrc/collapse.hip
+++ b/tiebrush_amd/csrc/collapse.hip
@@ -2477,25 +2477,34 @@
 __global__ __launch_bounds__(CB_NT) void g2c_count_key_k(uint32_t ng, const uint64_t* __restrict__ key, const uint32_t* __restrict__ rep,
                                                          const uint32_t* __restrict__ cig_off, const uint32_t* __restrict__ cig,
                                                          uint32_t* __restrict__ cnt, uint32_t* __restrict__ cfirst, uint4* __restrict__ part,
+                                                         uint4* __restrict__ wagg, uint32_t* __restrict__ wcig,
                                                          unsigned long long* __restrict__ tsum, uint32_t* __restrict__ done,
                                                          unsigned long long* __restrict__ total) {
-  constexpr uint32_t NWV = CB_NT / 64;
-  __shared__ CbAgg wl[CB_ROWS * NWV];
-  __shared__ unsigned long long wsum[CB_ROWS * NWV];
+  constexpr uint32_t NROW = CB_TILE / CB_NT, NWV = CB_NT / 64, NQ = NROW * NWV;
+  static_assert(NQ == 64, "one wave folds the tile's (row, wave) entries");
+  __shared__ CbAgg wl[NQ];
+  __shared__ uint32_t wn[NQ];
+  __shared__ unsigned long long wsum[8];
   const CbOp op{};
   const CbAgg none{0, INT32_MIN, INT32_MIN, 1u};
-  for (uint32_t r = 0; r < CB_ROWS; ++r) {
-    const uint64_t i = (uint64_t)blockIdx.x * CB_TILE + ((uint64_t)r * CB_NT + threadIdx.x) * 4u;
-    CbAgg a = none;
-    uint32_t n4[4] = {0u, 0u, 0u, 0u};
+  const uint32_t o0 = blockIdx.x * CB_TILE, wv = threadIdx.x >> 6;
+  for (uint32_t j0 = 0; j0 < NROW; j0 += 4u) {
+    uint64_t k0[4], k1[4];
 #pragma unroll
-    for (int e = 0; e < 4; ++e) {
-      if (i + e < ng) {
-        const uint32_t o = (uint32_t)(i + e);
-        const uint64_t k0 = key[2 * (size_t)o], k1 = key[2 * (size_t)o + 1];
-        const int32_t tidv = (int32_t)(uint32_t)(k0 >> 33) - 1, posv = (int32_t)(uint32_t)((k0 >> 2) & 0x7FFFFFFFull) - 1;
-        uint32_t n = g2c_key_ops(k1);
-        int l = (int)(uint32_t)(k1 >> 32);
+    for (uint32_t u = 0; u < 4u; ++u) {
+      const uint32_t o = o0 + (j0 + u) * CB_NT + threadIdx.x;
+      k0[u] = o < ng ? key[2 * (size_t)o] : 0ull;
+      k1[u] = o < ng ? key[2 * (size_t)o + 1] : 0ull;
+    }
+#pragma unroll
+    for (uint32_t u = 0; u < 4u; ++u) {
+      const uint32_t o = o0 + (j0 + u) * CB_NT + threadIdx.x;
+      const bool valid = o < ng;
+      const int32_t tidv = (int32_t)(uint32_t)(k0[u] >> 33) - 1, posv = (int32_t)(uint32_t)((k0[u] >> 2) & 0x7FFFFFFFull) - 1;
+      uint32_t n = 0;
+      int l = (int)(uint32_t)(k1[u] >> 32);
+      if (valid) {
+        n = g2c_key_ops(k1[u]);
         if (n == 0) {
           const uint32_t rp = rep[o];
           const uint32_t c0 = cig_off[rp];
@@ -2504,37 +2513,30 @@
           int nex = 0;
           l = walk_exons(posv, cig + c0, n, [](int, int) {}, &nex);
         }
-        n4[e] = n;
-        a = op(a, CbAgg{tidv, tidv, posv + l, 1u});
-      }
-    }
-    if (i + 3 < ng) {
-      *reinterpret_cast<uint4*>(cnt + i) = make_uint4(n4[0], n4[1], n4[2], n4[3]);
-    } else {
-#pragma unroll
-      for (int e = 0; e < 4; ++e)
-        if (i + e < ng) cnt[i + e] = n4[e];
-    }
-    a = wave_incl_scan_op(a, op);
-    const unsigned long long sum = wave_sum((unsigned long long)n4[0] + n4[1] + n4[2] + n4[3]);
-    if (lane_id() == 63) {
-      wl[r * NWV + (threadIdx.x >> 6)] = a;
-      wsum[r * NWV + (threadIdx.x >> 6)] = sum;
+        cnt[o] = n;
+      }
+      const CbAgg a = cb_wave_agg(cb_lanes(valid, tidv), tidv, posv + l);
+      const uint32_t sum = wave_sum(n);
+      if (lane_id() == 0) {
+        wl[(j0 + u) * NWV + wv] = a;
+        wn[(j0 + u) * NWV + wv] = sum;
+      }
     }
   }
   __syncthreads();
-  if (threadIdx.x == 0) {
-    CbAgg run = none;
-    unsigned long long sum = 0;
-#pragma unroll
-    for (uint32_t q = 0; q < CB_ROWS * NWV; ++q) {
-      run = op(run, wl[q]);
-      sum += wsum[q];
-    }
-    uint64_t* o = reinterpret_cast<uint64_t*>(part + blockIdx.x);
-    cb_put(o, (uint64_t)(uint32_t)run.first_tid | ((uint64_t)(uint32_t)run.last_tid << 32));
-    cb_put(o + 1, (uint64_t)(uint32_t)run.mx | ((uint64_t)run.whole << 32));
-    cb_put(reinterpret_cast<uint64_t*>(tsum + blockIdx.x), sum);
+  if (wv == 0) {
+    const CbAgg inc = wave_incl_scan_op(wl[threadIdx.x], op);
+    CbAgg ex = shfl_up_t(inc, 1);
+    if (threadIdx.x == 0) ex = none;
+    const uint32_t sn = wn[threadIdx.x], sinc = wave_incl_sum(sn);
+    wagg[(size_t)blockIdx.x * NQ + threadIdx.x] = make_uint4((uint32_t)ex.first_tid, (uint32_t)ex.last_tid, (uint32_t)ex.mx, ex.whole);
+    wcig[(size_t)blockIdx.x * NQ + threadIdx.x] = sinc - sn;
+    if (threadIdx.x == 63) {
+      uint64_t* o = reinterpret_cast<uint64_t*>(part + blockIdx.x);
+      cb_put(o, (uint64_t)(uint32_t)inc.first_tid | ((uint64_t)(uint32_t)inc.last_tid << 32));
+      cb_put(o + 1, (uint64_t)(uint32_t)inc.mx | ((uint64_t)inc.whole << 32));
+      cb_put(reinterpret_cast<uint64_t*>(tsum + blockIdx.x), (uint64_t)sinc);
+    }
   }
   if (!cb_last_block(done)) return;
   const uint32_t ntiles = gridDim.x;
@@ -2557,38 +2559,36 @@
   uint32_t *jcnt, *ridx;
   unsigned long long* sums;
 };
+template <bool HEADS>
 __global__ __launch_bounds__(256) void g2c_gather_key_k(uint32_t ng, const uint64_t* __restrict__ key, const double* __restrict__ yc,
                                                         const int64_t* __restrict__ yx, const uint32_t* __restrict__ cfirst,
                                                         const uint32_t* __restrict__ cnt, const uint32_t* __restrict__ cig,
                                                         const unsigned long long* __restrict__ tbase, const uint4* __restrict__ part,
+                                                        const uint4* __restrict__ wagg, const uint32_t* __restrict__ wcig,
+                                                        uint32_t* __restrict__ hcnt, long long* __restrict__ xsum,
                                                         uint32_t ntiles, uint32_t total, int32_t* __restrict__ o_tid,
                                                         int32_t* __restrict__ o_pos, uint8_t* __restrict__ o_strand, double* __restrict__ o_yc,
                                                         int64_t* __restrict__ o_yx, uint32_t* __restrict__ o_cig_off, uint32_t* __restrict__ o_cig,
                                                         uint4* __restrict__ o_part, G2cPrep P) {
   constexpr uint32_t NROW = CB_TILE / 256u;
-  __shared__ uint32_t s_w[NROW * 4u];
   for (uint32_t q = blockIdx.x * 256u + threadIdx.x; q < ntiles; q += gridDim.x * 256u) o_part[q] = part[q];
   unsigned long long mb = 0, ay = 0, nji = 0;
   uint32_t eb = 0;
   for (uint32_t tile = blockIdx.x; tile < ntiles; tile += gridDim.x) {
   const uint32_t o0 = tile * CB_TILE;
+  const uint32_t base = (uint32_t)tbase[tile];
+  const uint4 pv = part[tile];
+  const CbAgg before_tile{(int32_t)pv.x, (int32_t)pv.y, (int32_t)pv.z, pv.w};
+  uint32_t nh = 0;
+  long long xs = 0;
   for (uint32_t j = 0; j < NROW; ++j) {
     const uint32_t o = o0 + j * 256u + threadIdx.x;
-    const uint32_t s = wave_sum(o < ng ? cnt[o] : 0u);
-    if (lane_id() == 0) s_w[j * 4u + (threadIdx.x >> 6)] = s;
-  }
-  __syncthreads();
-  if (threadIdx.x < 64u) {
-    const uint32_t v = s_w[threadIdx.x];
-    s_w[threadIdx.x] = wave_incl_sum(v) - v;
-  }
-  __syncthreads();
-  const uint32_t base = (uint32_t)tbase[tile];
-  for (uint32_t j = 0; j < NROW; ++j) {
-    const uint32_t o = o0 + j * 256u + threadIdx.x;
-    const uint32_t cn = o < ng ? cnt[o] : 0u;
-    const uint32_t d = base + s_w[j * 4u + (threadIdx.x >> 6)] + wave_incl_sum(cn) - cn;
-    if (o >= ng) continue;
+    const uint32_t q = tile * (NROW * 4u) + j * 4u + (threadIdx.x >> 6);
+    const bool valid = o < ng;
+    const uint32_t cn = valid ? cnt[o] : 0u;
+    const uint32_t d = base + wcig[q] + wave_incl_sum(cn) - cn;
+    int32_t h_tid = 0, h_start = 0, h_end = 0;
+    if (valid) {
     const uint64_t k0 = key[2 * (size_t)o], k1 = key[2 * (size_t)o + 1];
     const int32_t tidv = (int32_t)(uint32_t)(k0 >> 33) - 1, posv = (int32_t)(uint32_t)((k0 >> 2) & 0x7FFFFFFFull) - 1;
     o_tid[o] = tidv;
@@ -2642,8 +2642,37 @@
     P.end[o] = posv + l;
     P.jcnt[o] = (uint32_t)(nex - 1);
     nji += (unsigned long long)(nex - 1);
-  }
-  __syncthreads();
+    h_tid = tidv;
+    h_start = posv + 1;
+    h_end = posv + l;
+    }
+    if (HEADS) {
+      const uint4 wa = wagg[q];
+      const CbAgg carry = CbOp{}(before_tile, CbAgg{(int32_t)wa.x, (int32_t)wa.y, (int32_t)wa.z, wa.w});
+      const CbAgg before = cb_lane_before(cb_lanes(valid, h_tid), carry, h_tid, h_end);
+      long long x = 0;
+      if (valid && cb_head_step(before, h_tid, h_start, &x)) {
+        ++nh;
+        xs += x;
+      }
+    }
+  }
+  if (HEADS) {
+    __shared__ uint32_t red_h[4];
+    __shared__ long long red_x[4];
+    nh = wave_sum(nh);
+    xs = (long long)wave_sum((unsigned long long)xs);
+    if (lane_id() == 0) {
+      red_h[threadIdx.x >> 6] = nh;
+      red_x[threadIdx.x >> 6] = xs;
+    }
+    __syncthreads();
+    if (threadIdx.x == 0) {
+      hcnt[tile] = red_h[0] + red_h[1] + red_h[2] + red_h[3];
+      xsum[tile] = red_x[0] + red_x[1] + red_x[2] + red_x[3];
+    }
+    __syncthreads();
+  }
   }
   __shared__ unsigned long long red_mb[4], red_ay[4], red_nj[4];
   __shared__ uint32_t red_e[4];
@@ -2727,13 +2756,17 @@
   uint32_t* ooff = nullptr;
   uint4* part = nullptr;
   unsigned long long* tbase = nullptr;
+  uint4* wagg = nullptr;
+  uint32_t* wcig = nullptr;
   if (g_key) {
     part = ws_alloc<uint4>(ctx, ntiles);
     tbase = ws_alloc<unsigned long long>(ctx, ntiles);
-    if (!part || !tbase) return TBK_ENOMEM;
+    wagg = ws_alloc<uint4>(ctx, (size_t)ntiles * 64);
+    wcig = ws_alloc<uint32_t>(ctx, (size_t)ntiles * 64);
+    if (!part || !tbase || !wagg || !wcig) return TBK_ENOMEM;
     uint32_t* done = (uint32_t*)(ctx->d_scalars + 21);
     TBK_HIP(hipMemsetAsync(done, 0, sizeof(uint64_t), ctx->stream));
-    TBK_LAUNCH(ctx, "g2c_count", g2c_count_key_k, ntiles, CB_NT, 0, ng, g_key, g_rep, r_cig_off, r_cig, cnt, cfirst, part, tbase, done,
+    TBK_LAUNCH(ctx, "g2c_count", g2c_count_key_k, ntiles, CB_NT, 0, ng, g_key, g_rep, r_cig_off, r_cig, cnt, cfirst, part, wagg, wcig, tbase, done,
                (unsigned long long*)(ctx->d_scalars + 20));
   } else {
     ooff = ws_alloc<uint32_t>(ctx, ng);
@@ -2747,7 +2780,7 @@
   if (total >= (1ull << 32)) return TBK_E2BIG;
   auto al = [](size_t x) { return (x + 255) & ~(size_t)255; };
   size_t need = al((size_t)ng * 4) * 2 + al(ng) + al((size_t)ng * 8) * 2 + al((size_t)(ng + 1) * 4) + al((size_t)total * 4 + 4) +
-                (g_key ? al((size_t)ng * 4) * 5 + al((size_t)ntiles * sizeof(uint4)) : 0);
+                (g_key ? al((size_t)ng * 4) * 5 + al((size_t)ntiles * sizeof(uint4)) + al((size_t)ntiles * 4) + al((size_t)ntiles * 8) : 0);
   if (need > ctx->d_view_cap) {
     if (ctx->d_view) (void)hipFree(ctx->d_view);
     ctx->d_view = nullptr;
@@ -2771,6 +2804,9 @@
   uint32_t* o_cig = (uint32_t*)take((size_t)total * 4 + 4);
   G2cPrep P{};
   uint4* o_part = nullptr;
+  uint32_t* o_hcnt = nullptr;
+  long long* o_xsum = nullptr;
+  const bool heads = !ctx->dbg.view_heads_split;
   if (g_key) {
     P.start = (int32_t*)take((size_t)ng * 4);
     P.end = (int32_t*)take((size_t)ng * 4);
@@ -2778,10 +2814,18 @@
     P.jcnt = (uint32_t*)take((size_t)ng * 4);
     P.ridx = (uint32_t*)take((size_t)ng * 4);
     o_part = (uint4*)take((size_t)ntiles * sizeof(uint4));
+    o_hcnt = (uint32_t*)take((size_t)ntiles * 4);
+    o_xsum = (long long*)take((size_t)ntiles * 8);
     P.sums = (unsigned long long*)(ctx->d_scalars + 24);
     TBK_HIP(hipMemsetAsync(P.sums, 0, 4 * sizeof(uint64_t), ctx->stream));
-    TBK_LAUNCH(ctx, "g2c_gather", g2c_gather_key_k, ntiles, B, 0, ng, g_key, g_yc, g_yx, cfirst, cnt, r_cig, tbase, part, ntiles, (uint32_t)total,
-               o_tid, o_pos, o_strand, o_yc, o_yx, o_cig_off, o_cig, o_part, P);
+#define G2C_GATHER(HEADS)                                                                                                                   \
+  TBK_LAUNCH(ctx, "g2c_gather", g2c_gather_key_k<HEADS>, ntiles, B, 0, ng, g_key, g_yc, g_yx, cfirst, cnt, r_cig, tbase, part, wagg, wcig, o_hcnt, \
+             o_xsum, ntiles, (uint32_t)total, o_tid, o_pos, o_strand, o_yc, o_yx, o_cig_off, o_cig, o_part, P)
+    if (heads)
+      G2C_GATHER(true);
+    else
+      G2C_GATHER(false);
+#undef G2C_GATHER
     TBK_HIP(hipMemcpyAsync(ctx->h_scalars + 24, ctx->d_scalars + 24, 4 * sizeof(uint64_t), hipMemcpyDeviceToHost, ctx->stream));
   } else
     TBK_LAUNCH(ctx, "g2c_gather", g2c_gather_k, cdiv(ng, B), B, 0, ng, g_rep, g_yc, g_yx, r_tid, r_pos, r_strand, cfirst, cnt, r_cig, ooff,
@@ -2809,6 +2853,8 @@
     V.ridx = P.ridx;
     V.agg = o_part;
     V.agg_tiles = ntiles;
+    V.hcnt = heads ? o_hcnt : nullptr;
+    V.xsum = heads ? o_xsum : nullptr;
     V.n_bases = ctx->h_scalars[24];
     V.sum_abs = ctx->h_scalars[25];
     V.err = (uint32_t)ctx->h_scalars[26];
diff --git a/tiebrush_amd/csrc/cov.hip b/tiebrush_amd/csrc/cov.hip
--- a/tiebrush_amd/csrc/cov.hip
+++ b/tiebrush_amd/csrc/cov.hip
@@ -725,6 +725,13 @@
   }
 }
 
+__global__ __launch_bounds__(CB_NT) void cl_scan_k(uint32_t nt, const uint32_t* __restrict__ hcnt, const long long* __restrict__ xsum,
+                                                   uint32_t* __restrict__ hbase, long long* __restrict__ xbase) {
+  __shared__ uint32_t smu[CB_NT / 64];
+  __shared__ long long smx[CB_NT / 64];
+  cl_scan_block<CB_NT>(nt, hcnt, xsum, hbase, xbase, smu, smx);
+}
+
 template <bool EMIT>
 __global__ __launch_bounds__(CB_NT) void cl_heads_k(uint32_t m, CovArrays A, const uint4* __restrict__ part ,
                                                     uint32_t* __restrict__ hcnt, long long* __restrict__ xsum, const uint32_t* __restrict__ hbase,
@@ -796,10 +803,9 @@
 #pragma unroll
     for (int e = 0; e < 4; ++e) {
       if (i + e < m) {
-        const bool first = w.last_tid == INT32_MIN;
-        const bool head = first || t4[r][e] != w.last_tid || s4[r][e] > w.mx;
-        if (head) {
-          xs[r] += (long long)s4[r][e] - 1ll - (first ? 0ll : (long long)w.mx);
+        long long x;
+        if (cb_head_step(w, t4[r][e], s4[r][e], &x)) {
+          xs[r] += x;
           hd |= 1u << e;
           ++nh;
         }
@@ -1702,7 +1708,7 @@
 };
 
 static int cov_intervals_lean(tbk_ctx* ctx, const tbk_cov_in* in, tbk_cov_out* out, CovArrays A, uint32_t m, bool all_valid, uint64_t sum_abs,
-                              const uint4* pre_part) {
+                              const uint4* pre_part, const uint32_t* pre_hcnt, const long long* pre_xsum) {
   const uint32_t B = 256;
   uint64_t* sc = ctx->d_scalars;
   const uint32_t cbt = cdiv(m, CB_TILE);
@@ -1730,8 +1736,15 @@
   uint32_t* done = (uint32_t*)(sc + 16);
   TBK_HIP(hipMemsetAsync(done, 0, sizeof(uint64_t), ctx->stream));
   if (!pre_part) TBK_LAUNCH(ctx, "cov_bundles", cb_agg_k, cbt, CB_NT, 0, m, A.tid, A.end, own_part, done);
-  TBK_LAUNCH(ctx, "cov_bundles", cl_heads_k<false>, cbt, CB_NT, 0, m, A, cpart, hcnt, xsum, (const uint32_t*)nullptr, (const long long*)nullptr, in->cig_off,
-             in->cig, T, L, sc, ctx->d_err, done + 1, hbase, xbase);
+  if (pre_part && pre_hcnt && pre_xsum)
+    TBK_LAUNCH(ctx, "cov_bundles", cl_scan_k, 1, CB_NT, 0, cbt, pre_hcnt, pre_xsum, hbase, xbase);
+  else
+    TBK_LAUNCH(ctx, "cov_bundles", cl_heads_k<false>, cbt, CB_NT, 0, m, A, cpart, hcnt, xsum, (const uint32_t*)nullptr, (const long long*)nullptr, in->cig_off,
+               in->cig, T, L, sc, ctx->d_err, done + 1, hbase, xbase);
+  ctx->cl_tables.hcnt = pre_part && pre_hcnt && pre_xsum ? pre_hcnt : hcnt;
+  ctx->cl_tables.xsum = pre_part && pre_hcnt && pre_xsum ? pre_xsum : xsum;
+  ctx->cl_tables.tiles = cbt;
+  ctx->cl_tables.from_view = pre_part && pre_hcnt && pre_xsum;
   TBK_LAUNCH(ctx, "cov_place", cl_heads_k<true>, cbt, CB_NT, 0, m, A, cpart, hcnt, xsum, hbase, xbase, in->cig_off, in->cig, T, L, sc, ctx->d_err,
              (uint32_t*)nullptr, (uint32_t*)nullptr, (long long*)nullptr);
   uint32_t eb = 0;
@@ -1791,8 +1804,23 @@
   return 0;
 }
 
+extern "C" int tbk_cov_heads_probe(tbk_ctx* ctx, uint32_t* hcnt, int64_t* xsum, uint32_t cap, uint32_t* n_tiles, uint32_t* from_view) {
+  if (!ctx || !n_tiles || !from_view) return TBK_EINVAL;
+  const auto& t = ctx->cl_tables;
+  *n_tiles = t.tiles;
+  *from_view = t.from_view ? 1u : 0u;
+  if (!t.tiles) return 0;
+  if (cap < t.tiles || !hcnt || !xsum) return TBK_E2BIG;
+  TBK_HIP(hipSetDevice(ctx->device));
+  TBK_HIP(hipStreamSynchronize(ctx->stream));
+  TBK_HIP(hipMemcpy(hcnt, t.hcnt, (size_t)t.tiles * sizeof(uint32_t), hipMemcpyDeviceToHost));
+  TBK_HIP(hipMemcpy(xsum, t.xsum, (size_t)t.tiles * sizeof(int64_t), hipMemcpyDeviceToHost));
+  return 0;
+}
+
 static int cov_run(tbk_ctx* ctx, const tbk_cov_in* in, tbk_cov_out* out, bool sample_mode) {
   const uint32_t n = in->n_records;
+  ctx->cl_tables = {};
   const bool want_cov = out->cap_intervals > 0, want_j = out->cap_junctions > 0;
   out->n_intervals = out->n_junctions = 0;
   out->n_bases = 0;
@@ -1878,7 +1906,7 @@
   if (want_cov && !fractional && !sample_mode && !ctx->dbg.cov_legacy && !ctx->dbg.cov_bundle_scan) {
     const size_t ws_mark = ctx->ws_off;
     const uint4* pre_part = (prepared && V.agg && V.agg_tiles == cdiv(m, CB_TILE)) ? (const uint4*)V.agg : nullptr;
-    const int lrc = cov_intervals_lean(ctx, in, out, A, m, all_valid, sum_abs, pre_part);
+    const int lrc = cov_intervals_lean(ctx, in, out, A, m, all_valid, sum_abs, pre_part, pre_part ? V.hcnt : nullptr, pre_part ? V.xsum : nullptr);
     if (lrc < 0) return lrc;
     lean_done = lrc == 0;
     if (!lean_done) {
diff --git a/tiebrush_amd/csrc/tbk_api.hip b/tiebrush_amd/csrc/tbk_api.hip
--- a/tiebrush_amd/csrc/tbk_api.hip
+++ b/tiebrush_amd/csrc/tbk_api.hip
@@ -478,6 +478,7 @@
     else if (k == "wg_dense_verify") out->wg_dense_verify = on;
     else if (k == "wg_rank_merge") out->wg_rank_merge = on;
     else if (k == "wg_back") out->wg_back_split = v == "split";
+    else if (k == "view_heads") out->view_heads_split = v == "split";
     else if (k == "cov_legacy") out->cov_legacy = on;
     else if (k == "cov_bundle_scan") out->cov_bundle_scan = on;
     else if (k == "cov_prep") out->cov_prep = on;
diff --git a/tiebrush_amd/csrc/tbk_internal.h b/tiebrush_amd/csrc/tbk_internal.h
--- a/tiebrush_amd/csrc/tbk_internal.h
+++ b/tiebrush_amd/csrc/tbk_internal.h
@@ -94,6 +94,7 @@
   bool wg_stats = false;
   bool wg_dense_verify = false, wg_rank_merge = false;
   bool wg_back_split = false;
+  bool view_heads_split = false;
   bool cov_legacy = false, cov_bundle_scan = false, cov_prep = false, junc_radix = false, no_junc_agg = false;
   uint64_t cov_tile_cap = 0;
   uint32_t jh_cap = 0;
@@ -133,9 +134,17 @@
     uint32_t *jcnt = nullptr, *ridx = nullptr;
     const void* agg = nullptr;
     uint32_t agg_tiles = 0;
+    const uint32_t* hcnt = nullptr;
+    const long long* xsum = nullptr;
     uint64_t n_bases = 0, sum_abs = 0, n_junc = 0;
     uint32_t err = 0;
   } view_prep;
+  struct ClTables {
+    const uint32_t* hcnt = nullptr;
+    const long long* xsum = nullptr;
+    uint32_t tiles = 0;
+    bool from_view = false;
+  } cl_tables;
   bool profiling = false;
   std::vector<KTime> ktimes;
   std::vector<hipEvent_t> ev_pool;
```

After: 21.75 billion records/s (median of 6 runs). No clear change (+0.6%).
